# TGAC/KAT

Hardware: AMD Instinct MI355X
Metric: k-mers/sec (whole node) for kat comp reads-vs-assembly k=27 (higher is better)
Workload: dtype u64

## Files before the change

### kat_amd/csrc/kg_count.hip

```cpp
#include "kg_host.hpp"
#include "kg_ingest.hpp"
#include "kg_kernels.hpp"
#include "kg_partition.hpp"
#include "kg_partition_wide.hpp"

#include <condition_variable>
#include <deque>
#include <mutex>
#include <thread>


static const uint64_t g_test_sweep_thr = hook("KATGPU_TEST_SWEEP_THR") ? strtoull(hook("KATGPU_TEST_SWEEP_THR"), nullptr, 10) : 0;
static const uint64_t g_test_max_starts = hook("KATGPU_TEST_MAX_STARTS") ? strtoull(hook("KATGPU_TEST_MAX_STARTS"), nullptr, 10) : 0;

namespace kg {
static __global__ void __launch_bounds__(256)
k_sweep(DevTable t, uint32_t thr, unsigned long long* scratch) {
    uint32_t mx = 0;
    const uint64_t stride = (uint64_t)gridDim.x * blockDim.x;
    for (uint64_t i = (uint64_t)blockIdx.x * blockDim.x + threadIdx.x; i < t.cap; i += stride) {
        uint32_t c = t.counts[i];
        if (c >= thr) {
            uint64_t key = t.keys[i];
            uint32_t take = (c / thr) * thr;
            c -= take;
            t.counts[i] = c;
            ovf_add(t, key, take);
        }
        mx = c > mx ? c : mx;
    }
    for (int off = 32; off > 0; off >>= 1) { uint32_t o = __shfl_down(mx, off, 64); mx = o > mx ? o : mx; }
    if ((threadIdx.x & 63) == 0) atomicMax(scratch, (unsigned long long)mx);
}
}

static int maybe_sweep(katgpu_table* t, uint64_t next_starts) {
    katgpu_ctx* c = t->ctx;
    if (t->dev().cbits) return KATGPU_OK;
    const uint64_t limit = g_test_sweep_thr ? 2 * g_test_sweep_thr - 1 : 0xFFFFFFFFULL;
    if (t->count_bound + t->unchecked_adds + next_starts <= limit) return KATGPU_OK;
    const uint32_t thr = g_test_sweep_thr ? (uint32_t)g_test_sweep_thr : 0x80000000u;
    unsigned long long* scratch = (unsigned long long*)&t->dev().ctrs[CTR_SCRATCH];
    HIPCHK(c, hipMemsetAsync(scratch, 0, sizeof(uint64_t), c->stream));
    {
        ScopedTimer tm(c, KATGPU_K_REGROW, t->dev().cap);
        hipLaunchKernelGGL(k_sweep, dim3(grid_for(c, t->dev().cap, 256, 8)), dim3(256), 0, c->stream, t->dev(), thr, scratch);
    }
    uint64_t mx = 0;
    HIPCHK(c, hipMemcpyAsync(&mx, scratch, sizeof mx, hipMemcpyDeviceToHost, c->stream));
    HIPCHK(c, hipStreamSynchronize(c->stream));
    t->count_bound = mx;
    t->unchecked_adds = 0;
    return KATGPU_OK;
}

static int launch_count(katgpu_table* t, const uint8_t* dev_bases, size_t n) {
    katgpu_ctx* c = t->ctx;
    if (n < t->dev().k) return KATGPU_OK;
    if (t->dev().keys_b) {
        const uint64_t n_chunks = (n + WIDE_CHUNK_STARTS - 1) / WIDE_CHUNK_STARTS;
        const int grid = (int)std::min<uint64_t>(n_chunks, (uint64_t)c->n_cu * 4);
        ScopedTimer tm(c, KATGPU_K_COUNT, n);
        if ((reinterpret_cast<uintptr_t>(dev_bases) & 15) == 0)
            hipLaunchKernelGGL((k_count<true, true>), dim3(grid), dim3(COUNT_BLOCK), 0, c->stream, t->dev(), dev_bases, (uint64_t)n, n_chunks);
        else
            hipLaunchKernelGGL((k_count<false, true>), dim3(grid), dim3(COUNT_BLOCK), 0, c->stream, t->dev(), dev_bases, (uint64_t)n, n_chunks);
        HIPCHK(c, hipGetLastError());
        return KATGPU_OK;
    }
    int src = maybe_sweep(t, n);
    if (src) return src;
    t->unchecked_adds += n;
    const uint64_t n_chunks = (n + CHUNK_STARTS - 1) / CHUNK_STARTS;
    const int grid = (int)std::min<uint64_t>(n_chunks, (uint64_t)c->n_cu * c->count_blocks_per_cu);
    ScopedTimer tm(c, KATGPU_K_COUNT, n);
    if ((reinterpret_cast<uintptr_t>(dev_bases) & 15) == 0)
        hipLaunchKernelGGL(k_count<true>, dim3(grid), dim3(COUNT_BLOCK), 0, c->stream, t->dev(), dev_bases, (uint64_t)n, n_chunks);
    else
        hipLaunchKernelGGL(k_count<false>, dim3(grid), dim3(COUNT_BLOCK), 0, c->stream, t->dev(), dev_bases, (uint64_t)n, n_chunks);
    HIPCHK(c, hipGetLastError());
    return KATGPU_OK;
}



static const uint64_t g_part_min_starts = getenv("KATGPU_PART_MIN_STARTS") ? strtoull(getenv("KATGPU_PART_MIN_STARTS"), nullptr, 10) : (32ULL << 20);
static const uint64_t g_test_round_items = hook("KATGPU_TEST_ROUND_ITEMS") ? strtoull(hook("KATGPU_TEST_ROUND_ITEMS"), nullptr, 10) : 0;
static const double g_arena_fraction = getenv("KATGPU_ARENA_FRACTION") ? std::min(0.95, std::max(0.05, atof(getenv("KATGPU_ARENA_FRACTION")))) : 0.85;
static const uint32_t g_p1_wgs = hook("KATGPU_P1_WGS") ? std::max<uint32_t>(1, (uint32_t)strtoul(hook("KATGPU_P1_WGS"), nullptr, 10)) : 3;
static const bool g_l1_lean = hook_u64("KATGPU_L1_LEAN", 1) != 0;
static const uint32_t g_l1_fast = hook("KATGPU_L1_FAST") ? (uint32_t)strtoul(hook("KATGPU_L1_FAST"), nullptr, 10) : 1;
static const uint32_t g_test_l1_cpb = hook("KATGPU_TEST_L1_CPB") ? (uint32_t)strtoul(hook("KATGPU_TEST_L1_CPB"), nullptr, 10) : 0;
static const uint32_t g_p2_fast = hook("KATGPU_P2_FAST") ? (uint32_t)strtoul(hook("KATGPU_P2_FAST"), nullptr, 10) : 1;
static const uint64_t g_test_p2_ovf_cap = hook("KATGPU_TEST_P2_OVF_CAP") ? strtoull(hook("KATGPU_TEST_P2_OVF_CAP"), nullptr, 10) : 0;
static const uint32_t g_test_spill_mod = hook("KATGPU_TEST_SPILL_MOD") ? (uint32_t)strtoul(hook("KATGPU_TEST_SPILL_MOD"), nullptr, 10) : 0;
static const uint64_t g_test_ap_seg = hook_u64("KATGPU_TEST_AP_SEG", 0) & ~3ULL;
static const uint32_t g_apply_per_cu = (uint32_t)hook_u64("KATGPU_APPLY_PER_CU", 0);
static const uint64_t g_fresh_max_pct = hook_u64("KATGPU_FRESH_MAX_PCT", 100);
static const bool g_l1b_stamp = hook_u64("KATGPU_L1B_STAMP", 0) != 0;
static const bool g_p2x_stamp = hook_u64("KATGPU_P2X_STAMP", 0) != 0;
static const bool g_p2_stamp = hook_u64("KATGPU_P2_STAMP", 0) != 0;
static const bool g_apply_stamp = hook_u64("KATGPU_APPLY_STAMP", 0) != 0;

static bool part_geometry(const DevTable& d, PartGeom* g) {
    g->R = d.n_regions; g->S = d.region_slots; g->P1 = d.p1; g->P2 = d.p2; g->l2 = d.l2;
    g->b_lo = 0; g->b_hi = d.p1;
    g->pl = place_make(d.k, d.p1, d.n1, d.l2);
    g->hb = l2_hi_bytes(g->pl.rb);
    g->hb1 = l2_hi_bytes(g->pl.n1);
    g->cbits = d.cbits;
    if (d.cbits && g->hb > 2) g->hb = 2;
    return d.k <= 32 && g->pl.rb <= 63  && g->P1 <= MAX_PARTS && g->P2 <= MAX_PARTS && g->S % 4 == 0 && g->S >= 64 && g->S <= AP2_MAX_SLOTS;
}
static double l2_items_per_l1_item(uint32_t hb) { return 1 + 1.0 / 16 + 2.0 * MAX_PARTS / l2_tile_items(hb); }
static const uint32_t g_test_pass_buckets = hook("KATGPU_TEST_PASS_BUCKETS") ? (uint32_t)strtoul(hook("KATGPU_TEST_PASS_BUCKETS"), nullptr, 10) : 0;
static uint32_t pass_buckets(uint32_t p1, uint32_t n_cu) {
    if (g_test_pass_buckets) return std::max<uint32_t>(1, std::min(p1, g_test_pass_buckets));
    return n_cu && p1 > n_cu && p1 % n_cu == 0 ? n_cu : p1;
}
static double arena_bytes_per_item(uint32_t hb, uint32_t passes) { return 8.0 * (1 + 1.0 / 24) + l2_bytes_per_item(hb) * (1 + 1.0 / 24) * l2_items_per_l1_item(hb) / passes + 0.25 + 0.02; }

static const bool g_test_grow_nomem = hook("KATGPU_TEST_GROW_NOMEM") != nullptr;

static void insert_keys(katgpu_table* t, const void* keys, uint64_t n, size_t key_bytes) {
    katgpu_ctx* c = t->ctx;
    ScopedTimer tm(c, KATGPU_K_COUNT, n);
    if (key_bytes == 16) hipLaunchKernelGGL(k_insert_keys_w, dim3(grid_for(c, n, 256, 6)), dim3(256), 0, c->stream, t->dev(), (const u64x2*)keys, n);
    else hipLaunchKernelGGL(k_insert_keys, dim3(grid_for(c, n, 256, 6)), dim3(256), 0, c->stream, t->dev(), (const uint64_t*)keys, n);
}
typedef std::vector<std::pair<const void*, uint64_t>> KeyLists;
static int grow_beside_arena(katgpu_table* t, uint64_t incoming, uint64_t min_cap, const KeyLists& stash, size_t key_bytes, bool* arena_lost) {
    uint64_t n_stash = 0;
    for (auto& l : stash) n_stash += l.second;
    katgpu_ctx* c = t->ctx;
    auto grow = [&]() -> int {
        if (min_cap > t->dev().cap) {
            if (t->disable_grow) return fail(c, KATGPU_ERR_TABLE_FULL, "Hash full");
            uint64_t nc = t->dev().cap; while (nc < min_cap) nc *= 2;
            return regrow(t, nc);
        }
        return ensure_room(t, incoming);
    };
    *arena_lost = false;
    int rc = g_test_grow_nomem ? KATGPU_ERR_NOMEM : grow();
    if (rc != KATGPU_ERR_NOMEM) return rc;
    (void)hipGetLastError();
    std::vector<uint8_t> host;
    if (n_stash) {
        try { host.resize(n_stash * key_bytes); } catch (...) { return fail(c, KATGPU_ERR_NOMEM, "no host memory to park %llu spilled k-mers", (unsigned long long)n_stash); }
        uint64_t at = 0;
        for (auto& l : stash) { HIPCHK(c, hipMemcpy(host.data() + at * key_bytes, l.first, l.second * key_bytes, hipMemcpyDeviceToHost)); at += l.second; }
    }
    HIPCHK(c, hipStreamSynchronize(c->stream));
    release_arena(c);
    *arena_lost = true;
    if (g_trace) fprintf(stderr, "[katgpu] growth beside the partition arena failed: arena released, %llu keys parked on the host\n", (unsigned long long)n_stash);
    rc = grow();
    if (rc) return rc;
    if (n_stash) {
        const size_t chunk = std::min<size_t>(n_stash, ((size_t)256 << 20) / key_bytes);
        uint8_t* d = nullptr;
        HIPCHK(c, pool_alloc(c, (void**)&d, chunk * key_bytes));
        for (size_t i = 0; i < n_stash && rc == KATGPU_OK; i += chunk) {
            const size_t m = std::min(chunk, (size_t)n_stash - i);
            if (hipMemcpyAsync(d, host.data() + i * key_bytes, m * key_bytes, hipMemcpyHostToDevice, c->stream) != hipSuccess) { rc = fail(c, KATGPU_ERR_DEVICE, "spill upload"); break; }
            insert_keys(t, d, m, key_bytes);
            if (hipStreamSynchronize(c->stream) != hipSuccess) rc = fail(c, KATGPU_ERR_DEVICE, "spill insert");
        }
        pool_release(c, d);
    }
    return rc;
}

static int ensure_arena(katgpu_ctx* c, size_t small_bytes, size_t item_bytes, size_t want_items, size_t want_bytes, const char* note, bool* usable) {
    *usable = false;
    if (c->arena_limit) want_bytes = std::min(want_bytes, std::max(c->arena_limit, small_bytes + item_bytes * ((size_t)64 << 20)));
    if (c->arena_bytes < want_bytes) {
        size_t free_b = 0, total_b = 0;
        HIPCHK(c, hipMemGetInfo(&free_b, &total_b));
        free_b += c->arena_bytes;
        const size_t bytes = std::min<size_t>(want_bytes, (size_t)(g_arena_fraction * (double)free_b));
        if (bytes > c->arena_bytes + c->arena_bytes / 2 || c->arena_bytes < small_bytes + item_bytes * std::min<size_t>(want_items, (size_t)64 << 20)) {
            if (c->arena) { HIPCHK(c, hipFree(c->arena)); c->arena = nullptr; c->arena_bytes = 0; }
            if (!g_test_round_items && bytes < small_bytes + item_bytes * ((size_t)1 << 20)) return KATGPU_OK;
            const double t_ar = now_ms();
            if (hipMalloc((void**)&c->arena, bytes) != hipSuccess) { (void)hipGetLastError(); c->arena = nullptr; return KATGPU_OK; }
            c->arena_bytes = bytes;
            if (g_trace) fprintf(stderr, "[katgpu +%.0f ms] partition arena of %.1f GB%s: %.0f ms\n", since_load(), bytes / 1e9, note, now_ms() - t_ar);
        }
    }
    *usable = true;
    return KATGPU_OK;
}
struct ArenaBusy { katgpu_ctx* c; explicit ArenaBusy(katgpu_ctx* c_) : c(c_) { c->arena_busy = true; } ~ArenaBusy() { c->arena_busy = false; } };
template <typename T> static T* carve(uint8_t*& a, size_t bytes) { T* p = (T*)a; a += align_up(bytes, 256); return p; }

constexpr size_t LDS_BYTES = 160 * 1024, LDS_GRANULE = 1280;
template <typename K, typename... Args>
static int launch_lds(katgpu_ctx* c, K kern, dim3 grid, dim3 block, size_t lds, size_t ceiling, Args... args) {
    if (!c->lds_attr.count(reinterpret_cast<const void*>(kern))) {
        HIPCHK(c, hipFuncSetAttribute(reinterpret_cast<const void*>(kern), hipFuncAttributeMaxDynamicSharedMemorySize, (int)ceiling));
        c->lds_attr.insert(reinterpret_cast<const void*>(kern));
    }
    hipLaunchKernelGGL(kern, grid, block, lds, c->stream, args...);
    return KATGPU_OK;
}

struct StampLine { const char* head; int n_shown, n_sum; const char* phase[9];  int digits; };
static const StampLine STAMPS_L1B = {"[katgpu] level-1 (blocks) stamps (wave 0 of every workgroup, cycles summed):", 9, 9,
    {" codes %.*f %%", "  blocks out %.*f %%", " (+ barrier %.*f %%)", "  sweep %.*f %%", " (+ %.*f %%)", "  per bucket %.*f %%", " (+ %.*f %%)", "  placing %.*f %%", " (+ %.*f %%)"}, 1};
static const StampLine STAMPS_P2X = {"[katgpu] level-2 (blocks in, blocks out) stamps (wave 0 of every workgroup, cycles summed):", 7, 9,
    {" wait for the tile %.*f %%", " (+ barrier %.*f %%)", "  ranking + blocks out %.*f %%", " (+ %.*f %%)", "  per sub-bucket %.*f %%", " (+ %.*f %%)", "  placing %.*f %%"}, 1};
static const StampLine STAMPS_P2 = {"[katgpu] level-2 stamps (lane 0 of every workgroup, cycles summed):", 5, 5,
    {" wait for the tile %.*f %%", "  digit + rank %.*f %%", "  scan %.*f %%", "  staging %.*f %%", "  copy-out %.*f %%"}, 0};
constexpr int STAMP_AT_APPLY = 8, STAMP_AT = 18;
constexpr int STAMP_AREA = 256 / 8;
static_assert(2 <= STAMP_AT_APPLY && STAMP_AT_APPLY + 9 <= STAMP_AT && STAMP_AT + 10 <= STAMP_AREA, "the stamp counters lie behind spill_n and ovf_n, apart, inside spill_n's carve");
template <typename Launch>
static int with_stamps(katgpu_ctx* c, unsigned long long* dev, int n, const StampLine* line, Launch launch) {
    unsigned long long st[10];
    HIPCHK(c, hipMemsetAsync(dev, 0, n * sizeof(unsigned long long), c->stream));
    int rc = launch(dev);
    if (rc) return rc;
    HIPCHK(c, hipMemcpyAsync(st, dev, n * sizeof(unsigned long long), hipMemcpyDeviceToHost, c->stream));
    HIPCHK(c, hipStreamSynchronize(c->stream));
    double tot = line ? 0 : (double)(st[0] + st[1] + st[3] + st[4]);
    if (!line && st[5])
        fprintf(stderr, "[katgpu] apply stamps (wave 0 of every workgroup, cycles summed): fill %.3g (%.0f %%)  walk %.3g (%.0f %%; drains %.0f %% of the walk, %.2f iterations per pass)  barrier + sweep %.3g (%.0f %%)  write-back %.3g (%.0f %%); %llu regions, %.1f chunks per wave and region, %.0f cycles per region\n",
                (double)st[0], 100 * st[0] / tot, (double)st[1], 100 * st[1] / tot, 100.0 * st[2] / std::max(1.0, (double)st[1]), (double)st[8] / std::max(1.0, (double)st[7]), (double)st[3], 100 * st[3] / tot, (double)st[4], 100 * st[4] / tot, st[5], (double)st[6] / st[5], tot / st[5]);
    if (!line || !st[n - 1]) return KATGPU_OK;
    for (int i = 0; i < line->n_sum; ++i) tot += (double)st[i];
    char buf[768];
    int at = snprintf(buf, sizeof buf, "%s", line->head);
    for (int i = 0; i < line->n_shown; ++i) at += snprintf(buf + at, sizeof buf - at, line->phase[i], line->digits, 100 * st[i] / tot);
    fprintf(stderr, "%s; %llu tiles, %.0f cycles per tile\n", buf, st[n - 1], tot / st[n - 1]);
    return KATGPU_OK;
}

struct ApplyForm { bool packed; int block, kp; bool fresh , hooked; };
struct ApplyLaunch {
    katgpu_table* t; const PartGeom& g; const uint64_t* off2; const uint8_t* l2_buf; uint64_t* spill_buf; unsigned long long* spill_n; const uint32_t* run_len; const uint64_t* bucket_end;
    dim3 grid; size_t lds; uint32_t qcap; uint64_t seg_len; uint32_t zero_fill; ApplyForm* form;
};
template <int B, int KP, int HB, bool INL, bool HK, bool LATE , int NR, bool STAMP = false>
static int apply_pk(const ApplyLaunch& a) {
    if (a.form) *a.form = ApplyForm{true, B, KP, INL, HK};
    return launch_lds(a.t->ctx, k_p3_apply_pk<B, KP, HB, INL, HK, LATE, NR, STAMP>, a.grid, dim3(B), a.lds, LDS_BYTES - 256, a.t->dv, a.g, a.off2, a.l2_buf, a.spill_buf, a.spill_n, a.run_len, a.bucket_end,
                      a.qcap, a.seg_len, g_test_spill_mod, a.zero_fill);
}
template <int HB>
static int apply_pk_shape(const ApplyLaunch& a, uint32_t blk, bool fresh, bool hooked) {
    if (hooked) return apply_pk<1024, 5, HB, false, true, true, 3>(a);
    if (blk == 1024) return fresh ? apply_pk<1024, 5, HB, true, false, true, 3>(a) : apply_pk<1024, 5, HB, false, false, true, 2>(a);
    if (a.g.S <= 4096) {
        if (HB == 1 && g_apply_stamp && fresh)
            return with_stamps(a.t->ctx, a.spill_n + STAMP_AT_APPLY, 9, nullptr, [&](unsigned long long*) { return apply_pk<512, 4, 1, true, false, true, 3, true>(a); });
        return fresh ? apply_pk<512, 4, HB, true, false, true, 3>(a) : apply_pk<512, 4, HB, false, false, true, 2>(a);
    }
    if (HB == 1 && g_apply_stamp && !fresh)
        return with_stamps(a.t->ctx, a.spill_n + STAMP_AT_APPLY, 9, nullptr, [&](unsigned long long*) { return apply_pk<512, 10, 1, false, false, false, 2, true>(a); });
    return fresh ? apply_pk<512, 10, HB, true, false, false, 3>(a) : apply_pk<512, 10, HB, false, false, false, 2>(a);
}
template <int B, int KP, int HB, bool INL, int QC, bool HK>
static int apply_kv12(const ApplyLaunch& a) {
    if (a.form) *a.form = ApplyForm{false, B, KP, INL, HK};
    return launch_lds(a.t->ctx, k_p3_apply2<B, KP, 4, 3, HB, false, INL, true, QC, HK>, a.grid, dim3(B), a.lds, LDS_BYTES - 256, a.t->dev(), a.g, a.off2, a.l2_buf, a.spill_buf, a.spill_n, a.run_len, a.bucket_end,
                      (unsigned long long*)nullptr, g_test_spill_mod, a.seg_len);
}
template <int HB>
static int apply_kv12_shape(const ApplyLaunch& a, uint32_t blk, bool big, bool fresh, bool hooked) {
    if (hooked) return apply_kv12<1024, 5, HB, false, AP2_QCAP_BIG, true>(a);
    if (blk == 512 && a.g.S <= 2048) return fresh ? apply_kv12<512, 2, HB, true, AP2_QCAP, false>(a) : apply_kv12<512, 2, HB, false, AP2_QCAP, false>(a);
    if (blk == 512) return fresh ? apply_kv12<512, 4, HB, true, AP2_QCAP, false>(a) : apply_kv12<512, 4, HB, false, AP2_QCAP, false>(a);
    if (big) return fresh ? apply_kv12<1024, 5, HB, true, AP2_QCAP_BIG, false>(a) : apply_kv12<1024, 5, HB, false, AP2_QCAP_BIG, false>(a);
    return fresh ? apply_kv12<1024, 4, HB, true, AP2_QCAP, false>(a) : apply_kv12<1024, 4, HB, false, AP2_QCAP, false>(a);
}
static int launch_apply(katgpu_table* t, const PartGeom& g, const uint64_t* off2, const uint8_t* l2_buf, uint64_t* spill_buf, unsigned long long* spill_n,
                        const uint32_t* run_len, const uint64_t* bucket_end, uint64_t round_items, ApplyForm* form = nullptr) {
    katgpu_ctx* c = t->ctx;
    const uint32_t n_cu = (uint32_t)c->n_cu, regions = (g.b_hi - g.b_lo) * g.P2;
    bool fresh = t->distinct == 0;
    const bool hooked = g_test_spill_mod != 0;
    ApplyLaunch a{t, g, off2, l2_buf, spill_buf, spill_n, run_len, bucket_end, dim3(1), 0, 0, 0, 0, form};
    int rc = KATGPU_OK;
    if (g.cbits) {
        const size_t region_b = (size_t)g.S * 8;
        auto room = [&](uint32_t wgs) -> long { return (long)(LDS_BYTES / wgs / LDS_GRANULE * LDS_GRANULE) - 64 - (long)region_b; };
        uint32_t per_cu = 4;
        auto min_q = [&](uint32_t wgs) -> long { return 8L * 8 * (wgs == 2 ? 72 : 96); };
        while (per_cu > 1 && room(per_cu) < min_q(per_cu)) --per_cu;
        if (g_apply_per_cu) per_cu = std::min(per_cu, g_apply_per_cu);
        uint32_t blk = per_cu == 1 ? 1024 : 512;
        if (hooked) { blk = 1024; per_cu = 1; }
        per_cu = std::min<uint32_t>(per_cu, 2048 / blk);
        const uint32_t nw = blk / 64;
        while (per_cu > 1 && room(per_cu) < (long)(nw * 72 * 8)) --per_cu;
        a.qcap = (uint32_t)std::min<long>(256, room(per_cu) / (long)(nw * 8));
        if (a.qcap < 72) return fail(c, KATGPU_ERR_DEVICE, "a region of %u packed slots leaves no room for the apply kernel's queues", g.S);
        a.lds = region_b + (size_t)nw * a.qcap * 8;
        if (fresh && a.qcap >= 96 && (double)round_items * 100.0 >= (double)g_fresh_max_pct * (double)t->dv.cap) fresh = false;
        const uint64_t seg_cap = (pk_half(g.cbits) - 1) & ~3ULL;
        a.seg_len = g_test_ap_seg ? std::min<uint64_t>(g_test_ap_seg, seg_cap) : std::min<uint64_t>(AP2_SEGMENT, seg_cap);
        a.grid = dim3(std::min<uint32_t>(regions, n_cu * per_cu));
        const uint64_t r_lo = (uint64_t)g.b_lo * g.P2, r_hi = (uint64_t)g.b_hi * g.P2;
        if (t->zero_from != ~0ULL) { if (t->zero_from == r_lo) a.zero_fill = 1; else t->zero_rest(); }
        switch (g.hb) {
        case 0: rc = apply_pk_shape<0>(a, blk, fresh, hooked); break;
        case 1: rc = apply_pk_shape<1>(a, blk, fresh, hooked); break;
        case 2: rc = apply_pk_shape<2>(a, blk, fresh, hooked); break;
        default: return fail(c, KATGPU_ERR_DEVICE, "packed apply: item width %u", g.hb);
        }
        if (rc) return rc;
        HIPCHK(c, hipGetLastError());
        if (a.zero_fill) t->zero_from = r_hi >= t->dv.n_regions ? ~0ULL : r_hi;
        return KATGPU_OK;
    }
    const uint32_t blk = hooked ? 1024 : (g.S <= 4096 ? 512 : 1024);
    const bool big = g.S > 8192 || hooked;
    a.lds = (size_t)g.S * 12 + (size_t)(blk / 64) * (big ? AP2_QCAP_BIG : AP2_QCAP) * 12;
    const uint32_t per_cu = (uint32_t)std::max<size_t>(1, std::min<size_t>(LDS_BYTES / (a.lds + 512), 2048 / blk));
    a.grid = dim3(std::min<uint32_t>(regions, n_cu * per_cu));
    a.seg_len = g_test_ap_seg ? std::min<uint64_t>(g_test_ap_seg, AP2_SEGMENT) : AP2_SEGMENT;
    switch (g.hb) {
    case 0: rc = apply_kv12_shape<0>(a, blk, big, fresh, hooked); break;
    case 1: rc = apply_kv12_shape<1>(a, blk, big, fresh, hooked); break;
    case 2: rc = apply_kv12_shape<2>(a, blk, big, fresh, hooked); break;
    case 4: rc = apply_kv12_shape<4>(a, blk, big, fresh, hooked); break;
    }
    if (rc) return rc;
    HIPCHK(c, hipGetLastError());
    return KATGPU_OK;
}

constexpr size_t SEG_PAD = 64;
struct PartArena {
    uint32_t hb, passes; double per_item; size_t fixed_l1, small_bytes;
    uint32_t* hist1; uint64_t* offs; uint64_t* l1_off; uint64_t* off2; uint32_t* cnt2; uint64_t* bend; unsigned long long* spill_n; unsigned long long* ovf_n;
    uint8_t* l1_buf;
    uint8_t* l2_buf;
    uint64_t* ovf_buf; uint64_t ovf_cap;
    size_t round_items, l1_items, l2_items;
    PartArena(const PartGeom& g0, uint32_t W, uint32_t n_cu) : hb(g0.hb), passes(std::max<uint32_t>(1, g0.P1 / pass_buckets(g0.P1, n_cu))), per_item(arena_bytes_per_item(hb, passes)) {
        fixed_l1 = (size_t)W * MAX_PARTS * SEG_PAD;
        const size_t fixed_l2 = (size_t)((double)fixed_l1 * l2_items_per_l1_item(hb) / passes) + (size_t)MAX_PARTS * MAX_PARTS * P2_RUN_SLACK + 8192;
        small_bytes = align_up((size_t)W * MAX_PARTS * 4, 256) + align_up((size_t)W * MAX_PARTS * 8, 256) +
                      align_up((MAX_PARTS + 1) * 8, 256) + align_up(((size_t)MAX_PARTS * MAX_PARTS + 1) * 8, 256) +
                      align_up((size_t)MAX_PARTS * MAX_PARTS * 4, 256) + align_up((size_t)MAX_PARTS * 8, 256) + align_up((size_t)MAX_PARTS * 4, 256) + 256 +
                      (fixed_l1 + fixed_l2 + 4096) * 8 + 4096;
    }
    void carve_from(uint8_t* a, size_t arena_bytes, uint32_t W, size_t want_items) {
        hist1 = carve<uint32_t>(a, (size_t)W * MAX_PARTS * 4);
        offs = carve<uint64_t>(a, (size_t)W * MAX_PARTS * 8);
        l1_off = carve<uint64_t>(a, (MAX_PARTS + 1) * 8);
        off2 = carve<uint64_t>(a, ((size_t)MAX_PARTS * MAX_PARTS + 1) * 8);
        cnt2 = carve<uint32_t>(a, (size_t)MAX_PARTS * MAX_PARTS * 4);
        bend = carve<uint64_t>(a, (size_t)MAX_PARTS * 8);
        carve<uint32_t>(a, (size_t)MAX_PARTS * 4);
        spill_n = carve<unsigned long long>(a, STAMP_AREA * 8);
        ovf_n = spill_n + 1;
        round_items = std::min<size_t>(want_items, (size_t)((double)(arena_bytes - small_bytes) / per_item));
        l1_items = (round_items + round_items / 24 + fixed_l1 + 15) & ~(size_t)15;
        l2_items = ((size_t)((double)l1_items * l2_items_per_l1_item(hb) / passes) + (size_t)MAX_PARTS * MAX_PARTS * P2_RUN_SLACK + 4096 + 11) / 12 * 12;
        l1_buf = a;
        l2_buf = l1_buf + l1_items * 8;
        ovf_buf = (uint64_t*)(l2_buf + align_up(l2_buffer_bytes(hb, l2_items), 16));
        ovf_cap = g_test_p2_ovf_cap ? g_test_p2_ovf_cap : round_items / 32 + 1024;
    }
};
static int restore_ones(katgpu_table* t) { katgpu_ctx* c = t->ctx; HIPCHK(c, hipMemcpyAsync(&t->dv.ctrs[CTR_ONES], &t->ones, sizeof(uint64_t), hipMemcpyHostToDevice, c->stream)); return KATGPU_OK; }
static int probe_items_per_start(katgpu_table* t, const PartGeom& g, const PartArena& A, uint32_t W, const uint8_t* p, size_t left, double* items_per_start) {
    katgpu_ctx* c = t->ctx;
    const size_t probe_m = std::min<size_t>(left, (size_t)64 << 20) / P1_TILE_STARTS * P1_TILE_STARTS;
    const uint64_t pt = probe_m / P1_TILE_STARTS, ptw = (pt + W - 1) / W;
    hipLaunchKernelGGL(k_p1v2_count, dim3(W), dim3(P1_BLOCK), 0, c->stream, t->dv, g, p, (uint64_t)(probe_m + t->dv.k - 1), pt, ptw, A.hist1);
    hipLaunchKernelGGL(k_p1_scan, dim3(1), dim3(PART_BLOCK), 0, c->stream, g, W, A.hist1, A.offs, A.l1_off);
    uint64_t probe_items = 0;
    HIPCHK(c, hipMemcpyAsync(&probe_items, &A.l1_off[g.P1], sizeof probe_items, hipMemcpyDeviceToHost, c->stream));
    HIPCHK(c, hipStreamSynchronize(c->stream));
    *items_per_start = std::max(0.05, (double)probe_items / (double)probe_m);
    return t->dv.k == 32 && !t->dv.canonical ? restore_ones(t) : KATGPU_OK;
}
static size_t round_starts(size_t left, size_t round_items, double items_per_start) {
    size_t m = left;
    if (m > round_items) m = std::min(m, (size_t)((double)round_items / items_per_start * 0.98));
    if (m < left) {
        const size_t rounds_left = (left + m - 1) / m;
        m = (left + rounds_left - 1) / rounds_left;
        m += P1_TILE_STARTS - m % P1_TILE_STARTS;
        m = std::min(m, left);
    }
    return m;
}

enum class L1Edition { Blocks, SegLean512, SegLean1024, SegPlain512, SegPlain1024, ExactLean, ExactPlain };
static const char* const L1_EDITION_NAME[] = {"Blocks", "SegLean512", "SegLean1024", "SegPlain512", "SegPlain1024", "ExactLean", "ExactPlain"};
struct L1Plan {
    L1Edition edition; bool seg ; uint32_t wgs ; uint64_t n_tiles, tiles_per_wg;
    uint64_t seg_cap, cap_plain, stride64;
};
static L1Plan plan_level1(const PartGeom& g, uint32_t k, size_t m, uint64_t est_items, uint32_t W, uint32_t n_cu, size_t l1_items, bool seg_wanted) {
    const bool lean = g_l1_lean && lean_applies(k, g.pl.n1);
    const bool pb512 = g.P1 <= 512;
    const bool l1b = lean && pb512 && g.hb1 == 2;
    const uint64_t n_tiles = (m + P1_TILE_STARTS - 1) / P1_TILE_STARTS;
    L1Plan pl;
    pl.wgs = l1b ? n_cu : W;
    pl.n_tiles = l1b ? (m + L1B_TILE_STARTS - 1) / L1B_TILE_STARTS : n_tiles;
    uint64_t seg_cap = est_items / ((uint64_t)pl.wgs * g.P1);
    seg_cap += seg_cap / 24 + SEG_PAD;
    if (g_test_l1_cpb) seg_cap = std::min<uint64_t>(seg_cap, g_test_l1_cpb);
    if (l1b) seg_cap = (seg_cap + L1B_ITEMS - 1) / L1B_ITEMS * L1B_ITEMS;
    pl.cap_plain = seg_cap;
    if (!l1b && g.hb1 != 4 && !g_test_l1_cpb) seg_cap += std::min<uint64_t>(3 * seg_cap, 2 * ((pl.n_tiles + pl.wgs - 1) / pl.wgs));
    if (!l1b) seg_cap = (seg_cap + 3) & ~3ULL;
    pl.seg_cap = seg_cap;
    pl.stride64 = l1b ? align_up(8 * (uint64_t)pl.wgs * pl.cap_plain + 32, 64)
                      : std::max<uint64_t>(8 * (uint64_t)pl.wgs * pl.cap_plain, (uint64_t)(4 + g.hb1) * pl.wgs * seg_cap) + 32;
    pl.seg = seg_wanted && pl.stride64 * g.P1 <= (uint64_t)l1_items * 8 &&
             seg_cap < (1u << 24) && pl.stride64 <= 0xFFFFFFFFULL ;
    if (pl.seg) pl.edition = l1b ? L1Edition::Blocks : lean ? (pb512 ? L1Edition::SegLean512 : L1Edition::SegLean1024) : (pb512 ? L1Edition::SegPlain512 : L1Edition::SegPlain1024);
    else { pl.edition = lean ? L1Edition::ExactLean : L1Edition::ExactPlain; pl.wgs = W; pl.n_tiles = n_tiles; }
    pl.tiles_per_wg = (pl.n_tiles + pl.wgs - 1) / pl.wgs;
    return pl;
}
static int launch_l1_scatter(katgpu_table* t, const PartGeom& g, const L1Plan& l1, const PartArena& A, const uint8_t* p, uint64_t nb) {
    katgpu_ctx* c = t->ctx;
    auto blocks = [&](auto kern, unsigned long long* stamps) {
        return launch_lds(c, kern, dim3(l1.wgs), dim3(L1B_THREADS), sizeof(P1BLds), sizeof(P1BLds), t->dv, g, p, nb, l1.n_tiles, l1.tiles_per_wg,
                          A.l1_buf, (uint32_t)(l1.seg_cap / L1B_ITEMS), (uint32_t)l1.stride64, A.ovf_buf, A.ovf_n, A.ovf_cap, stamps);
    };
    auto segmented = [&](auto kern) {
        hipLaunchKernelGGL(kern, dim3(l1.wgs), dim3(P1_BLOCK), 0, c->stream, t->dv, g, p, nb, l1.n_tiles, l1.tiles_per_wg, (const uint64_t*)nullptr, (const uint64_t*)nullptr, A.l1_buf,
                           (uint32_t)l1.seg_cap, (uint32_t)l1.stride64, (uint32_t)l1.cap_plain, A.ovf_buf, A.ovf_n, A.ovf_cap);
        return KATGPU_OK;
    };
    auto exact = [&](auto kern) {
        hipLaunchKernelGGL(kern, dim3(l1.wgs), dim3(P1_BLOCK), 0, c->stream, t->dv, g, p, nb, l1.n_tiles, l1.tiles_per_wg, (const uint64_t*)A.offs, (const uint64_t*)A.l1_off, A.l1_buf,
                           0u, 0u, 0u, (uint64_t*)nullptr, (unsigned long long*)nullptr, (uint64_t)0);
        return KATGPU_OK;
    };
    switch (l1.edition) {
    case L1Edition::Blocks:
        if (!g_l1b_stamp) return blocks(k_p1b_scatter<false>, nullptr);
        return with_stamps(c, A.spill_n + STAMP_AT, 10, &STAMPS_L1B, [&](unsigned long long* st) { return blocks(k_p1b_scatter<true>, st); });
    case L1Edition::SegLean512:   return segmented(k_p1v2_scatter<true, true, 512>);
    case L1Edition::SegLean1024:  return segmented(k_p1v2_scatter<true, true, MAX_PARTS>);
    case L1Edition::SegPlain512:  return segmented(k_p1v2_scatter<true, false, 512>);
    case L1Edition::SegPlain1024: return segmented(k_p1v2_scatter<true, false, MAX_PARTS>);
    case L1Edition::ExactLean:    return exact(k_p1v2_scatter<false, true, MAX_PARTS>);
    case L1Edition::ExactPlain:   return exact(k_p1v2_scatter<false, false, MAX_PARTS>);
    }
    return KATGPU_OK;
}
static int level1(katgpu_table* t, const PartGeom& g, const L1Plan& l1, const PartArena& A, const uint8_t* p, size_t m, double items_per_start, uint64_t* items) {
    katgpu_ctx* c = t->ctx;
    const uint64_t nb = m + t->dv.k - 1;
    if (l1.seg) {
        int rc;
        { ScopedTimer tm(c, KATGPU_K_PART_L1S, *items); rc = launch_l1_scatter(t, g, l1, A, p, nb); }
        if (!rc && g_trace) fprintf(stderr, "[katgpu] partition round (segmented level 1%s): %zu starts, ~%llu items, %llu k-mers per segment (arena %.1f GB)\n", l1.edition == L1Edition::Blocks ? ", blocks of ten" : "", m,
                                    (unsigned long long)*items, (unsigned long long)l1.seg_cap, c->arena_bytes / 1e9);
        return rc;
    }
    {
        ScopedTimer tm(c, KATGPU_K_PART_L1, m);
        hipLaunchKernelGGL(k_p1v2_count, dim3(l1.wgs), dim3(P1_BLOCK), 0, c->stream, t->dv, g, p, nb, l1.n_tiles, l1.tiles_per_wg, A.hist1);
        hipLaunchKernelGGL(k_p1_scan, dim3(1), dim3(PART_BLOCK), 0, c->stream, g, l1.wgs, A.hist1, A.offs, A.l1_off);
    }
    HIPCHK(c, hipMemcpyAsync(items, &A.l1_off[g.P1], sizeof *items, hipMemcpyDeviceToHost, c->stream));
    HIPCHK(c, hipStreamSynchronize(c->stream));
    if (g_trace) fprintf(stderr, "[katgpu] partition round: %zu starts -> %llu items (buffer %zu items, arena %.1f GB, ratio %.3f)\n", m, (unsigned long long)*items, A.round_items, c->arena_bytes / 1e9, items_per_start);
    if (*items > A.round_items) return t->dv.k == 32 && !t->dv.canonical ? restore_ones(t) : KATGPU_OK;
    if (!*items) return KATGPU_OK;
    ScopedTimer tm(c, KATGPU_K_PART_L1S, *items);
    return launch_l1_scatter(t, g, l1, A, p, nb);
}

enum class L1Items { Groups , WideGroups , Blocks  };
static const char* const L1_ITEMS_NAME[] = {"Groups", "WideGroups", "Blocks"};
enum L2Family : uint32_t { L2_BLOCKS = 1 , L2_ONE_PASS = 2 , L2_EXACT = 4  };
struct L2Pass { katgpu_ctx* c; const PartGeom& g; const PartArena& A; uint32_t grid; L1Items src; uint64_t seg_slots; uint32_t* families ; };
template <typename K>
static int p2_one_pass(const L2Pass& x, K kern, size_t lds, unsigned long long* stamps = nullptr) {
    return launch_lds(x.c, kern, dim3(x.grid), dim3(PART_BLOCK), lds, lds, x.g, x.A.l1_off, x.A.l1_buf, x.A.l2_buf, x.A.off2, x.A.cnt2, x.A.ovf_buf, x.A.ovf_n, x.A.ovf_cap, x.seg_slots, stamps);
}
template <typename K>
static int p2_exact(const L2Pass& x, K kern, size_t lds) {
    return launch_lds(x.c, kern, dim3(x.grid), dim3(PART_BLOCK), lds, lds, x.g, x.A.l1_off, x.A.l1_buf, x.A.l2_buf, x.A.off2, x.seg_slots, x.A.bend);
}
template <int HB>
static int launch_l2_hb(const L2Pass& x, bool one_pass) {
    constexpr size_t lds_e = sizeof(P2Lds<HB>), lds_f = sizeof(typename P2FastLds<HB>::type);
    unsigned long long* const stamps = x.A.spill_n + STAMP_AT;
    if (x.families) *x.families |= !one_pass ? L2_EXACT : x.src == L1Items::Blocks && HB == 1 ? L2_BLOCKS : L2_ONE_PASS;
    switch (x.src) {
    case L1Items::Blocks:
        if constexpr (HB == 4) break;
        else if (!one_pass) return p2_exact(x, k_p2<HB, false, true>, lds_e);
        else if constexpr (HB != 1) return p2_one_pass(x, k_p2_fast<HB, false, false, true>, lds_f);
        else if (!g_p2x_stamp) return p2_one_pass(x, k_p2x_fast<false>, sizeof(P2XLds));
        else return with_stamps(x.c, stamps, 10, &STAMPS_P2X, [&](unsigned long long* st) { return p2_one_pass(x, k_p2x_fast<true>, sizeof(P2XLds), st); });
    case L1Items::WideGroups: return one_pass ? p2_one_pass(x, k_p2_fast<HB, true>, lds_f) : p2_exact(x, k_p2<HB, true>, lds_e);
    case L1Items::Groups:
        if constexpr (HB == 1) if (one_pass && g_p2_stamp) return with_stamps(x.c, stamps, 6, &STAMPS_P2, [&](unsigned long long* st) { return p2_one_pass(x, k_p2_fast<1, false, true>, lds_f, st); });
        return one_pass ? p2_one_pass(x, k_p2_fast<HB, false>, lds_f) : p2_exact(x, k_p2<HB, false>, lds_e);
    }
    return fail(x.c, KATGPU_ERR_DEVICE, "level 2 from blocked level-1 items: item width %u", x.g.hb);
}
static int launch_l2(const L2Pass& x, bool one_pass) {
    switch (x.g.hb) {
    case 0: return launch_l2_hb<0>(x, one_pass);
    case 1: return launch_l2_hb<1>(x, one_pass);
    case 2: return launch_l2_hb<2>(x, one_pass);
    case 4: return launch_l2_hb<4>(x, one_pass);
    }
    return fail(x.c, KATGPU_ERR_DEVICE, "level 2: item width %u", x.g.hb);
}
enum class L2Next { UseCnt2 , Exact , FallBackExact ,
                    RedoRound  };
static int read_overflow(katgpu_table* t, const PartArena& A, bool seg, bool tried_fast, unsigned long long ovf_l1, const unsigned long long* ovf_before, unsigned long long* overflowed, L2Next* next) {
    katgpu_ctx* c = t->ctx;
    HIPCHK(c, hipMemcpyAsync(overflowed, A.ovf_n, sizeof *overflowed, hipMemcpyDeviceToHost, c->stream));
    HIPCHK(c, hipStreamSynchronize(c->stream));
    if (seg && ovf_l1 > A.ovf_cap) {
        if (g_trace) fprintf(stderr, "[katgpu] segmented level 1: %llu k-mers beyond their segments (list holds %llu): exact level 1 from here on\n", ovf_l1, (unsigned long long)A.ovf_cap);
        *next = L2Next::RedoRound;
        return restore_ones(t);
    }
    *next = !tried_fast ? L2Next::Exact : *overflowed <= A.ovf_cap ? L2Next::UseCnt2 : L2Next::FallBackExact;
    if (*next == L2Next::FallBackExact) {
        if (g_trace) fprintf(stderr, "[katgpu] k_p2_fast: %llu k-mers beyond their runs (list holds %llu): exact level 2 from here on\n", *overflowed, (unsigned long long)A.ovf_cap);
        *overflowed = *ovf_before;
        HIPCHK(c, hipMemcpyAsync(A.ovf_n, ovf_before, sizeof *ovf_before, hipMemcpyHostToDevice, c->stream));
    }
    return KATGPU_OK;
}

enum class RoundEnd { Done, RedoExactL1 , DirectPath  };
static int level2_and_apply(katgpu_table* t, PartGeom& g, const L1Plan& l1, const PartArena& A, uint64_t items, bool* p2_fast_ok, KeyLists* lists, RoundEnd* end) {
    katgpu_ctx* c = t->ctx;
    const bool seg = l1.seg;
    const uint64_t seg_slots = seg ? (uint64_t)l1.wgs * l1.seg_cap : 0;
    const L1Items src = seg && l1.edition == L1Edition::Blocks ? L1Items::Blocks : g.hb1 == 4 ? L1Items::WideGroups : L1Items::Groups;
    *end = RoundEnd::Done;
    std::vector<uint64_t> h_l1_off;
    unsigned long long ovf_l1 = 0;
    if (!seg) {
        h_l1_off.resize(g.P1 + 1);
        HIPCHK(c, hipMemcpyAsync(h_l1_off.data(), A.l1_off, (g.P1 + 1) * sizeof(uint64_t), hipMemcpyDeviceToHost, c->stream));
    } else HIPCHK(c, hipMemcpyAsync(&ovf_l1, A.ovf_n, sizeof ovf_l1, hipMemcpyDeviceToHost, c->stream));
    HIPCHK(c, hipStreamSynchronize(c->stream));
    auto lbeg = [&](uint32_t b) -> uint64_t { return seg ? (uint64_t)b * g.l1_real : h_l1_off[b]; };
    const uint32_t tile2 = l2_tile_items(g.hb);
    auto pass_extent = [&](uint32_t b_lo, uint32_t b_hi) -> uint64_t {
        const uint64_t nn = lbeg(b_hi) - lbeg(b_lo);
        return nn + nn / 16 + 2ULL * g.P2 * (nn / tile2 + 1) + (uint64_t)(b_hi - b_lo) * g.P2 * P2_RUN_SLACK + 64;
    };
    uint32_t step = pass_buckets(g.P1, (uint32_t)c->n_cu);
    auto fits = [&](uint32_t st) { for (uint32_t b = 0; b < g.P1; b += st) if (pass_extent(b, std::min(g.P1, b + st)) > A.l2_items) return false; return true; };
    while (step > 1 && !fits(step)) step = (step + 1) / 2;
    if (!fits(step)) {
        *end = RoundEnd::DirectPath;
        return seg || (t->dv.k == 32 && !t->dv.canonical) ? restore_ones(t) : KATGPU_OK;
    }
    const bool try_fast0 = *p2_fast_ok && (g_p2_fast == 2 || items / g.R >= 1024);
    unsigned long long ovf_total = ovf_l1;
    uint32_t l2_families = 0;
    ApplyForm ap{};
    if (g_trace && g.P1 > step) fprintf(stderr, "[katgpu]   level 2 + apply in %u passes of %u buckets (level-2 buffer: %zu items)\n", (g.P1 + step - 1) / step, step, A.l2_items);
    for (uint32_t b_lo = 0; b_lo < g.P1; b_lo += step) {
        g.b_lo = b_lo; g.b_hi = std::min(g.P1, b_lo + step);
        const uint64_t pass_items = std::max<uint64_t>(1, (uint64_t)((double)items * (g.b_hi - g.b_lo) / g.P1));
        auto l1_at = [&](uint32_t b) -> uint64_t { return seg ? (uint64_t)b * g.l1_stride : l1_bucket_base(lbeg(b), b); };
        uint64_t* spill_buf = (uint64_t*)(A.l1_buf + l1_at(b_lo));
        g.spill_cap = (l1_at(g.b_hi) - l1_at(b_lo)) / 8;
        const bool try_fast = try_fast0 && *p2_fast_ok;
        const L2Pass x{c, g, A, std::min<uint32_t>(g.b_hi - g.b_lo, (uint32_t)c->n_cu), src, seg_slots, &l2_families};
        HIPCHK(c, hipMemsetAsync(A.spill_n, 0, sizeof(unsigned long long), c->stream));
        int rc = KATGPU_OK;
        if (try_fast) { ScopedTimer tm(c, KATGPU_K_PART_L2, pass_items); rc = launch_l2(x, true); }
        if (rc) return rc;
        L2Next next = L2Next::Exact;
        unsigned long long overflowed = ovf_total;
        if (try_fast || (seg && b_lo == 0)) {
            rc = read_overflow(t, A, seg, try_fast, ovf_l1, &ovf_total, &overflowed, &next);
            if (rc) return rc;
            if (next == L2Next::RedoRound) { *end = RoundEnd::RedoExactL1; return KATGPU_OK; }
            if (next == L2Next::FallBackExact) *p2_fast_ok = false;
        }
        const bool runs = next == L2Next::UseCnt2;
        if (!runs) { ScopedTimer tm(c, KATGPU_K_PART_L2, pass_items); rc = launch_l2(x, false); }
        if (rc) return rc;
        ovf_total = overflowed;
        {
            ScopedTimer tm(c, KATGPU_K_PART_APPLY, pass_items);
            rc = launch_apply(t, g, A.off2, A.l2_buf, spill_buf, A.spill_n, runs ? A.cnt2 : nullptr, runs ? nullptr : A.bend, items, &ap);
        }
        if (rc) return rc;
        HIPCHK(c, hipGetLastError());
        unsigned long long spilled = 0;
        HIPCHK(c, hipMemcpyAsync(&spilled, A.spill_n, sizeof spilled, hipMemcpyDeviceToHost, c->stream));
        HIPCHK(c, hipStreamSynchronize(c->stream));
        if (spilled > g.spill_cap)
            return fail(c, KATGPU_ERR_TABLE_FULL, "Hash full: %llu k-mers of a partition pass found no slot (the list holds %llu); raise the size hint", spilled, (unsigned long long)g.spill_cap);
        if (spilled) lists->push_back({spill_buf, spilled});
    }
    if (ovf_total) lists->push_back({A.ovf_buf, ovf_total});
    if (g_trace) {
        char l2[32];
        snprintf(l2, sizeof l2, "%s%s%s", l2_families & L2_BLOCKS ? "+blocks" : "", l2_families & L2_ONE_PASS ? "+one-pass" : "", l2_families & L2_EXACT ? "+exact" : "");
        fprintf(stderr, "[katgpu] partition forms: l1=%s items=%s hb1=%u hb=%u l2=%s apply=%s B=%d KP=%d fresh=%d%s\n", L1_EDITION_NAME[(int)l1.edition], L1_ITEMS_NAME[(int)src], g.hb1, g.hb,
                l2[0] ? l2 + 1 : "none", ap.packed ? "packed" : "KV12", ap.block, ap.kp, (int)ap.fresh, ap.hooked ? " hooked" : "");
    }
    return KATGPU_OK;
}
static int insert_spilled(katgpu_table* t, const KeyLists& lists, bool* arena_lost) {
    *arena_lost = false;
    if (lists.empty()) return KATGPU_OK;
    uint64_t total = 0;
    for (auto& l : lists) total += l.second;
    int rc = grow_beside_arena(t, total, 0, lists, 8, arena_lost);
    if (rc || *arena_lost) return rc;
    for (auto& l : lists) insert_keys(t, l.first, l.second, 8);
    return KATGPU_OK;
}

static int count_partitioned(katgpu_table* t, const uint8_t* dev_bases, size_t n, size_t* done) {
    katgpu_ctx* c = t->ctx;
    const uint32_t k = t->dv.k, n_cu = (uint32_t)c->n_cu;
    const size_t n_starts = n - k + 1;
    *done = 0;
    c->arena_borrowed = false;
    if (n < 64) return KATGPU_OK;
    if (!g_test_round_items && !t->disable_grow && t->dv.cap < n_starts / 16) {
        uint64_t nc = t->dv.cap; while (nc < n_starts / 16) nc *= 2;
        int grc = regrow(t, nc);
        if (grc) return grc;
    }
    const uint32_t W = n_cu * std::min<uint32_t>(g_p1_wgs, 4);
    PartGeom g0;
    if (!part_geometry(t->dv, &g0)) return KATGPU_OK;
    PartArena A(g0, W, n_cu);
    size_t want_items = n_starts;
    if (g_test_round_items) want_items = std::min<size_t>(want_items, g_test_round_items);
    bool usable = false;
    int rc = ensure_arena(c, A.small_bytes, 18, want_items, A.small_bytes + (size_t)((A.per_item + 0.5) * (double)want_items), "", &usable);
    if (rc || !usable) return rc;
    ArenaBusy busy(c);
    A.carve_from(c->arena, c->arena_bytes, W, want_items);
    if (!g_test_round_items && A.round_items < ((size_t)1 << 20) && A.round_items < n_starts) return KATGPU_OK;
    bool p2_fast_ok = g_p2_fast != 0, l1_fast_ok = g_l1_fast != 0;
    double items_per_start = 1.0;
    size_t pos = 0;
    bool ratio_known = false;
    while (pos < n_starts) {
        rc = refresh_counters(t);
        if (rc) return rc;
        if ((double)t->distinct > 0.6 * (double)t->dv.cap) {
            bool lost = false;
            rc = grow_beside_arena(t, 0, t->dv.cap * 2, KeyLists(), 8, &lost);
            if (rc) return rc;
            if (lost) break;
        }
        PartGeom g;
        if (!part_geometry(t->dv, &g)) break;
        if (g.hb > A.hb) break;
        const size_t left = n_starts - pos;
        const uint8_t* p = dev_bases + pos;
        if (!ratio_known && !g_test_round_items && (left > A.round_items || (l1_fast_ok && left >= ((size_t)64 << 20)))) {
            rc = probe_items_per_start(t, g, A, W, p, left, &items_per_start);
            if (rc) return rc;
            ratio_known = true;
        }
        const size_t m = round_starts(left, A.round_items, items_per_start);
        t->count_bound = 0xFFFFFFFFULL;
        const uint64_t est_items = (uint64_t)((double)m * items_per_start);
        const bool seg_wanted = l1_fast_ok && (g_l1_fast == 2 || (ratio_known && est_items >= ((uint64_t)64 << 20)));
        const L1Plan l1 = plan_level1(g, k, m, est_items, W, n_cu, A.l1_items, seg_wanted);
        g.l1_stride = l1.seg ? l1.stride64 : 0;
        g.l1_real = l1.seg ? (uint64_t)l1.wgs * l1.cap_plain : 0;
        HIPCHK(c, hipMemsetAsync(A.spill_n, 0, 2 * sizeof(unsigned long long), c->stream));
        uint64_t items = est_items;
        rc = level1(t, g, l1, A, p, m, items_per_start, &items);
        if (rc) return rc;
        if (!l1.seg && items > A.round_items) {
            items_per_start = std::min(1.0, (double)items / (double)m * 1.02);
            continue;
        }
        if (items) {
            KeyLists lists;
            RoundEnd end;
            rc = level2_and_apply(t, g, l1, A, items, &p2_fast_ok, &lists, &end);
            if (rc) return rc;
            if (end == RoundEnd::RedoExactL1) { l1_fast_ok = false; continue; }
            if (end == RoundEnd::DirectPath) break;
            bool lost = false;
            rc = insert_spilled(t, lists, &lost);
            if (rc) return rc;
            if (lost) { pos += m; break; }
        }
        pos += m;
    }
    *done = pos;
    return refresh_counters(t);
}

static bool wide_part_geometry(const DevTable& d) {
    return d.keys_b && d.p1 <= (uint32_t)MAX_PARTS && d.p2 <= (uint32_t)MAX_PARTS && d.region_slots % 4 == 0 && d.region_slots >= 64 && d.region_slots <= WIDE_AP_MAX_SLOTS &&
           (uint64_t)d.p1 * d.p2 == d.n_regions;
}
static int count_partitioned_w(katgpu_table* t, const uint8_t* dev_bases, size_t n, size_t* done) {
    katgpu_ctx* c = t->ctx;
    const uint32_t k = t->dev().k;
    const size_t n_starts = n - k + 1;
    *done = 0;
    c->arena_borrowed = false;
    if (n < 4096 || !wide_part_geometry(t->dev())) return KATGPU_OK;
    if (!g_test_round_items && !t->disable_grow && t->dev().cap < n_starts / 16) {
        uint64_t nc = t->dev().cap; while (nc < n_starts / 16) nc *= 2;
        int grc = regrow(t, nc);
        if (grc) return grc;
        if (!wide_part_geometry(t->dev())) return KATGPU_OK;
    }
    const uint32_t W = (uint32_t)c->n_cu * 3;
    const size_t tile_starts = W1_TILE_STARTS;
    const size_t small_bytes = align_up((size_t)W * MAX_PARTS * 4, 256) + align_up((size_t)W * MAX_PARTS * 8, 256) + align_up((MAX_PARTS + 1) * 8, 256) +
                               align_up(((size_t)MAX_PARTS * MAX_PARTS + 1) * 8, 256) + 256 + 4096;
    size_t want_items = n_starts;
    if (g_test_round_items) want_items = std::min<size_t>(want_items, g_test_round_items);
    bool usable = false;
    int rc = ensure_arena(c, small_bytes, 32, want_items + 64, small_bytes + 32 * (want_items + 64), " (wide k-mers)", &usable);
    if (rc || !usable) return rc;
    ArenaBusy busy(c);
    uint8_t* a = c->arena;
    uint32_t* hist1 = carve<uint32_t>(a, (size_t)W * MAX_PARTS * 4);
    uint64_t* offs = carve<uint64_t>(a, (size_t)W * MAX_PARTS * 8);
    uint64_t* l1_off = carve<uint64_t>(a, (MAX_PARTS + 1) * 8);
    uint64_t* off2 = carve<uint64_t>(a, ((size_t)MAX_PARTS * MAX_PARTS + 1) * 8);
    unsigned long long* spill_n = carve<unsigned long long>(a, 256);
    const size_t round_items = std::min<size_t>(want_items, (c->arena_bytes - small_bytes) / 32);
    u64x2* l1_buf = (u64x2*)a;
    u64x2* l2_buf = l1_buf + round_items;
    if (!g_test_round_items && round_items < ((size_t)1 << 20) && round_items < n_starts) return KATGPU_OK;
    if (round_items < tile_starts && round_items < n_starts) return KATGPU_OK;

    size_t pos = 0;
    while (pos < n_starts) {
        rc = refresh_counters(t);
        if (rc) return rc;
        if ((double)t->distinct > 0.6 * (double)t->dev().cap) {
            bool lost = false;
            rc = grow_beside_arena(t, 0, t->dev().cap * 2, KeyLists(), 16, &lost);
            if (rc) return rc;
            if (lost) break;
        }
        if (!wide_part_geometry(t->dev())) break;
        const DevTable d = t->dev();
        size_t m = std::min(n_starts - pos, round_items);
        if (m < n_starts - pos) {
            const size_t rounds_left = (n_starts - pos + m - 1) / m;
            m = std::min(m, (n_starts - pos + rounds_left - 1) / rounds_left + tile_starts);
            m -= m % tile_starts;
            if (!m) break;
        }
        const size_t nb = m + k - 1;
        const uint8_t* p = dev_bases + pos;
        const uint64_t n_tiles = (m + tile_starts - 1) / tile_starts;
        const uint64_t tiles_per_wg = (n_tiles + W - 1) / W;
        PartGeom g{};
        g.P1 = d.p1;
        HIPCHK(c, hipMemsetAsync(spill_n, 0, sizeof(unsigned long long), c->stream));
        {
            ScopedTimer tm(c, KATGPU_K_PART_L1, m);
            hipLaunchKernelGGL(k_w1<false>, dim3(W), dim3(W1_BLOCK), 0, c->stream, d, d.p1, p, (uint64_t)nb, n_tiles, tiles_per_wg, hist1, (const uint64_t*)nullptr, (u64x2*)nullptr);
            hipLaunchKernelGGL(k_p1_scan, dim3(1), dim3(PART_BLOCK), 0, c->stream, g, W, hist1, offs, l1_off);
        }
        uint64_t items = 0;
        HIPCHK(c, hipMemcpyAsync(&items, &l1_off[d.p1], sizeof items, hipMemcpyDeviceToHost, c->stream));
        HIPCHK(c, hipStreamSynchronize(c->stream));
        if (g_trace) fprintf(stderr, "[katgpu] partition round (wide k-mers): %zu starts -> %llu items (buffer %zu items, arena %.1f GB)\n", m, (unsigned long long)items, round_items, c->arena_bytes / 1e9);
        if (items > round_items) return fail(c, KATGPU_ERR_DEVICE, "wide partition round: %llu items from %zu starts", (unsigned long long)items, m);
        if (items) {
            {
                ScopedTimer tm(c, KATGPU_K_PART_L1S, items);
                hipLaunchKernelGGL(k_w1<true>, dim3(W), dim3(W1_BLOCK), 0, c->stream, d, d.p1, p, (uint64_t)nb, n_tiles, tiles_per_wg, (uint32_t*)nullptr, (const uint64_t*)offs, l1_buf);
            }
            {
                ScopedTimer tm(c, KATGPU_K_PART_L2, items);
                hipLaunchKernelGGL(k_w2, dim3(std::min<uint32_t>(d.p1, (uint32_t)c->n_cu)), dim3(PART_BLOCK), 0, c->stream, d.p1, d.p2, (const uint64_t*)l1_off, (const u64x2*)l1_buf, l2_buf, off2);
            }
            {
                ScopedTimer tm(c, KATGPU_K_PART_APPLY, items);
                rc = launch_lds(c, k_w3_apply, dim3(std::min<uint32_t>(d.n_regions, (uint32_t)c->n_cu)), dim3(W3_BLOCK), (size_t)d.region_slots * 20, LDS_BYTES - 256, d, (const uint64_t*)off2, (const u64x2*)l2_buf,
                                l1_buf , spill_n, g_test_spill_mod);
                if (rc) return rc;
            }
            HIPCHK(c, hipGetLastError());
            unsigned long long spilled = 0;
            HIPCHK(c, hipMemcpyAsync(&spilled, spill_n, sizeof spilled, hipMemcpyDeviceToHost, c->stream));
            HIPCHK(c, hipStreamSynchronize(c->stream));
            if (spilled) {
                if (g_trace) fprintf(stderr, "[katgpu]   %llu k-mers spilled by full regions\n", spilled);
                bool lost = false;
                rc = grow_beside_arena(t, spilled, 0, KeyLists(1, {l1_buf, spilled}), 16, &lost);
                if (rc) return rc;
                if (lost) { pos += m; break; }
                insert_keys(t, l1_buf, spilled, 16);
                HIPCHK(c, hipStreamSynchronize(c->stream));
            }
        }
        pos += m;
    }
    *done = pos;
    return refresh_counters(t);
}

int count_resident(katgpu_table* t, const uint8_t* dev_bases, size_t n) {
    const uint32_t k = t->dv.k;
    if (n < k) return KATGPU_OK;
    size_t pos = 0;
    const size_t n_starts = n - k + 1;
    while (!t->dv.keys_b && n_starts - pos >= std::max<uint64_t>(g_part_min_starts, 1) && (reinterpret_cast<uintptr_t>(dev_bases + pos) & 15) == 0) {
        size_t done = 0;
        int prc = count_partitioned(t, dev_bases + pos, n - pos, &done);
        if (prc) return prc;
        if (!done) break;
        pos += done;
    }
    while (t->dv.keys_b && n_starts - pos >= std::max<uint64_t>(g_part_min_starts, 1) && (reinterpret_cast<uintptr_t>(dev_bases + pos) & 15) == 0) {
        size_t done = 0;
        int prc = count_partitioned_w(t, dev_bases + pos, n - pos, &done);
        if (prc) return prc;
        if (!done) break;
        pos += done;
    }
    while (pos < n_starts) {
        int rc = refresh_counters(t);
        if (rc) return rc;
        uint64_t room = (uint64_t)(load_limit(t->dev()) * (double)t->dev().cap) > t->distinct ? (uint64_t)(load_limit(t->dev()) * (double)t->dev().cap) - t->distinct : 0;
        uint64_t want = std::min<uint64_t>(n_starts - pos, (uint64_t)CHUNK_STARTS * 65536);
        if (g_test_max_starts) want = std::min<uint64_t>(want, g_test_max_starts);
        if (room < std::min<uint64_t>(want, std::max<uint64_t>(t->dev().cap / 64, CHUNK_STARTS))) {
            rc = ensure_room(t, std::min<uint64_t>(want, std::max<uint64_t>(t->dev().cap / 2, CHUNK_STARTS)));
            if (rc) return rc;
            continue;
        }
        uint64_t starts = std::min(want, room);
        if (starts < n_starts - pos) starts -= starts % 16;
        if (starts == 0) starts = std::min<uint64_t>(16, n_starts - pos);
        rc = launch_count(t, dev_bases + pos, (size_t)(starts + k - 1));
        if (rc) return rc;
        pos += starts;
    }
    return refresh_counters(t);
}

extern "C" int katgpu_count_bases_device(katgpu_table* t, const uint8_t* dev_bases, size_t n) {
    if (!t || (!dev_bases && n)) return KATGPU_ERR_INVALID_ARG;
    HIPCHK(t->ctx, hipSetDevice(t->ctx->device));
    return count_resident(t, dev_bases, n);
}

static const size_t g_ring_bytes = (getenv("KATGPU_RING_MB") ? std::max<size_t>(1, strtoull(getenv("KATGPU_RING_MB"), nullptr, 10)) : 1024) << 20;

static int ensure_staging(katgpu_ctx* c, size_t want = 0) {
    int rc = ensure_pinned(c); if (rc) return rc;
    size_t ring_want = g_ring_bytes;
    if (want) ring_want = std::min(g_ring_bytes, std::max<size_t>((size_t)16 << 20, align_up(want + 4096, (size_t)16 << 20)));
    if (c->ring_bytes && c->ring_bytes < ring_want) {
        for (int i = 0; i < 2; ++i) { hipFree(c->ring[i]); c->ring[i] = nullptr; }
        c->ring_bytes = 0;
    }
    for (; !c->ring_bytes; ring_want /= 2) {
        if (ring_want < ((size_t)1 << 20)) return fail(c, KATGPU_ERR_NOMEM, "no device memory for the staging rings");
        bool ok = true;
        for (int i = 0; i < 2 && ok; ++i) {
            hipError_t e = hipMalloc((void**)&c->ring[i], ring_want);
            if (e != hipSuccess && c->arena && !c->arena_borrowed && !c->arena_busy) {
                (void)hipGetLastError();
                hipFree(c->arena); c->arena = nullptr; c->arena_bytes = 0;
                e = hipMalloc((void**)&c->ring[i], ring_want);
            }
            if (e != hipSuccess) { (void)hipGetLastError(); for (int j = 0; j < i; ++j) { hipFree(c->ring[j]); c->ring[j] = nullptr; } ok = false; }
        }
        if (ok) c->ring_bytes = ring_want;
    }
    return KATGPU_OK;
}

struct HostFeeder {
    katgpu_table* t; katgpu_ctx* c;
    int cur = 0; size_t fill = 0; bool pin_used[2] = {false, false};
    int ring_cur = 0; size_t ring_fill = 0;
    uint8_t tail[64]; uint32_t tail_n = 0;
    static constexpr size_t HEAD = 64;
    std::thread worker;
    std::mutex mu; std::condition_variable cv;
    struct Job { int ring; size_t n; };
    std::deque<Job> jobs;
    bool ring_busy[2] = {false, false};
    bool stop = false;
    int worker_rc = KATGPU_OK; std::string worker_err;

    explicit HostFeeder(katgpu_table* t_) : t(t_), c(t_->ctx) {}
    ~HostFeeder() { shutdown(); }

    void run() {
        hipSetDevice(c->device);
        for (;;) {
            Job j;
            {
                std::unique_lock<std::mutex> lk(mu);
                cv.wait(lk, [&] { return stop || !jobs.empty(); });
                if (jobs.empty()) return;
                j = jobs.front(); jobs.pop_front();
            }
            int rc = worker_rc ? worker_rc : count_resident(t, c->ring[j.ring], j.n);
            {
                std::lock_guard<std::mutex> lk(mu);
                if (rc && !worker_rc) { worker_rc = rc; worker_err = c->err; }
                ring_busy[j.ring] = false;
            }
            cv.notify_all();
        }
    }
    void shutdown() {
        if (!worker.joinable()) return;
        { std::lock_guard<std::mutex> lk(mu); stop = true; }
        cv.notify_all();
        worker.join();
    }
    int begin(size_t want = 0) {
        int rc = ensure_staging(c, want); if (rc) return rc;
        tail_n = 0;
        worker = std::thread([this] { run(); });
        return open_ring();
    }
    int open_ring() {
        uint8_t head[HEAD];
        memset(head, 'N', HEAD);
        memcpy(head + HEAD - tail_n, tail, tail_n);
        HIPCHK(c, hipMemcpyAsync(c->ring[ring_cur], head, HEAD, hipMemcpyHostToDevice, c->copy_stream));
        HIPCHK(c, hipStreamSynchronize(c->copy_stream));
        ring_fill = HEAD;
        return KATGPU_OK;
    }
    int submit_ring() {
        HIPCHK(c, hipStreamSynchronize(c->copy_stream));
        const int other = ring_cur ^ 1;
        {
            std::unique_lock<std::mutex> lk(mu);
            if (ring_fill > HEAD) { ring_busy[ring_cur] = true; jobs.push_back({ring_cur, ring_fill}); }
            cv.notify_all();
            cv.wait(lk, [&] { return !ring_busy[other]; });
            if (worker_rc) return fail(c, worker_rc, "%s", worker_err.c_str());
        }
        if (ring_fill > HEAD) ring_cur = other;
        return open_ring();
    }
    int push(const uint8_t* p, size_t n) {
        while (n) {
            if (fill == 0 && pin_used[cur]) { hipError_t e = hipEventSynchronize(c->pin_free[cur]); if (e != hipSuccess) return fail(c, KATGPU_ERR_DEVICE, "%s", hipGetErrorString(e)); }
            const size_t room = c->stage_bytes - fill, take = std::min(room, n);
            memcpy(c->pinned[cur] + fill, p, take);
            fill += take; p += take; n -= take;
            if (fill == c->stage_bytes) { int rc = flush(); if (rc) return rc; }
        }
        return KATGPU_OK;
    }
    int flush() {
        if (!fill) return KATGPU_OK;
        const uint32_t want = t->dv.k - 1;
        size_t off = 0;
        while (off < fill) {
            if (ring_fill == c->ring_bytes) { int rc = submit_ring(); if (rc) return rc; }
            const size_t take = std::min(fill - off, c->ring_bytes - ring_fill);
            const uint8_t* src = c->pinned[cur] + off;
            HIPCHK(c, hipMemcpyAsync(c->ring[ring_cur] + ring_fill, src, take, hipMemcpyHostToDevice, c->copy_stream));
            ring_fill += take; off += take;
            if (take >= want) { memcpy(tail, src + take - want, want); tail_n = want; }
            else {
                uint8_t tmp[128]; const uint32_t keep = (uint32_t)std::min<size_t>(tail_n, want - take);
                memcpy(tmp, tail + tail_n - keep, keep); memcpy(tmp + keep, src, take);
                tail_n = keep + (uint32_t)take; memcpy(tail, tmp, tail_n);
            }
        }
        HIPCHK(c, hipEventRecord(c->pin_free[cur], c->copy_stream));
        pin_used[cur] = true;
        cur ^= 1; fill = 0;
        return KATGPU_OK;
    }
    int end_of_file() {
        static const uint8_t sep = 'N';
        return push(&sep, 1);
    }
    int finish() {
        int rc = flush(); if (rc) { shutdown(); return rc; }
        HIPCHK(c, hipStreamSynchronize(c->copy_stream));
        {
            std::unique_lock<std::mutex> lk(mu);
            if (ring_fill > HEAD) { ring_busy[ring_cur] = true; jobs.push_back({ring_cur, ring_fill}); }
            cv.notify_all();
// ... 108 lines not shown
```

### kat_amd/csrc/kg_l2_blocks.hpp

```cpp
#pragma once

namespace kg {

constexpr int L2X_N = 14;
constexpr uint32_t L2X_TILE = L2X_N * PART_BLOCK;
constexpr uint32_t L2X_POOL = 1252;

struct P2XLds {
    uint32_t hist[MAX_PARTS + 64];
    uint2 gb[MAX_PARTS];
    uint32_t where[L2X_POOL];
    uint32_t wave_tot[32];
    __attribute__((aligned(64))) uint32_t img[(MAX_PARTS + L2X_POOL) * 16];
};
static_assert(sizeof(P2XLds) <= 160 * 1024 - 256 && offsetof(P2XLds, img) % 64 == 0, "LDS");
static_assert(PART_BLOCK == MAX_PARTS, "thread b is sub-bucket b");

template <bool STAMP = false >
__global__ void __launch_bounds__(PART_BLOCK)
k_p2x_fast(PartGeom g, const uint64_t* __restrict__ l1_off, const uint8_t* __restrict__ l1_buf, uint8_t* __restrict__ l2_buf,
           uint64_t* __restrict__ off2, uint32_t* __restrict__ cnt2, uint64_t* __restrict__ ovf_buf, unsigned long long* __restrict__ ovf_n,
           uint64_t ovf_cap, uint64_t seg_slots, unsigned long long* __restrict__ stamps) {
    constexpr int N = L2X_N;
    constexpr uint32_t PB = MAX_PARTS, TILE_CAP = L2Fmt<1>::TILE ;
    extern __shared__ __attribute__((aligned(64))) unsigned char lds_raw[];
    P2XLds& L = *reinterpret_cast<P2XLds*>(lds_raw);
    unsigned char* const img8 = reinterpret_cast<unsigned char*>(L.img);
    const uint32_t tid = threadIdx.x, P = g.P2;
    unsigned long long st[10] = {0, 0, 0, 0, 0, 0, 0, 0, 0, 0}, tq = 0;
    auto stamp = [&](int i) { if (STAMP) { const unsigned long long x = (unsigned long long)clock64(); st[i] += x - tq; tq = x; } };
    uint64_t beg0, n0, nr0;
    l1_bucket_range(g, l1_off, seg_slots, g.b_lo, beg0, n0, nr0);
    uint32_t tid_o = tid;
    for (uint32_t b1 = g.b_lo + blockIdx.x; b1 < g.b_hi; b1 += gridDim.x) {
        uint64_t beg, n_items, n_real;
        const uint8_t* bucket = l1_buf + l1_bucket_range(g, l1_off, seg_slots, b1, beg, n_items, n_real);
        const uint64_t cap = p2_region_cap(n_real, P, TILE_CAP, L2_BLOCK_ITEMS);
        const uint64_t obase = p2_out_base(beg, b1, P, TILE_CAP, L2_BLOCK_ITEMS) - p2_out_base(beg0, g.b_lo, P, TILE_CAP, L2_BLOCK_ITEMS);
        uint8_t* const runs = l2_buf + l2_lo_at<1>(obase >> 2);
        const uint32_t capb = (uint32_t)(cap / L2_BLOCK_ITEMS);
        lds_barrier();
        asm volatile("" : "+v"(tid_o));
        L.hist[tid_o] = 0; L.gb[tid_o] = uint2{0u, 0u};
        if (tid < 64) L.hist[PB + tid_o] = 0;
        L.img[tid_o * 16 + 15] = 0;
        if (tid < P) off2[(uint64_t)b1 * P + tid_o] = obase + (uint64_t)tid * cap;
        uint32_t n_out = 0;
        constexpr int OUT_STEPS = (L2X_POOL + PART_BLOCK / 4 - 1) / (PART_BLOCK / 4);
        static_assert(OUT_STEPS <= N / 2, "a step per pair of the ranking's items");
        struct OutStep { u32x4 v; uint32_t where; };
        auto out_read = [&](int it, OutStep& o) {
            asm volatile("" : "+v"(tid_o));
            const uint32_t s = min((tid_o >> 2) + (uint32_t)it * (PART_BLOCK / 4), L2X_POOL - 1);
            o.where = L.where[s];
            o.v = *reinterpret_cast<const u32x4*>(&L.img[(PB + s) * 16 + (tid_o & 3) * 4]);
        };
        auto out_store = [&](int it, const OutStep& o) {
            asm volatile("" : "+v"(tid_o));
            if ((tid_o >> 2) + (uint32_t)it * (PART_BLOCK / 4) < n_out)
                *reinterpret_cast<u32x4*>(runs + (((uint64_t)o.where << 6) | ((tid_o & 3) * 16))) = o.v;
        };
        RawTileB<N> raw;
        p2_tile_issue_l1b<N>(bucket, 0, raw);
        for (uint64_t tbeg = 0; tbeg < n_items; tbeg += L2X_TILE) {
            if (STAMP) tq = (unsigned long long)clock64();
            TileItems<N, false> key;
            const uint32_t valid = p2_tile_decode_l1b<N>(tbeg, n_items, raw, key);
            {
#pragma unroll
                for (int j = 0; j < N; ++j) asm volatile("" : "+v"(key.lo[j]));
#pragma unroll
                for (int j = 0; j < N / 2; ++j) asm volatile("" : "+v"(key.hi[j]));
            }
            p2_tile_issue_l1b<N>(bucket, tbeg + L2X_TILE, raw);
            stamp(0);
            lds_barrier();
            stamp(1);
            uint32_t br[N];
            {
                uint32_t rk[N];
                const uint32_t dump = PB + (tid & 63);
                OutStep o;
#pragma unroll
                for (int j = 0; j < N; ++j) {
                    if (j % 2 == 0 && j / 2 < OUT_STEPS) out_read(j / 2, o);
                    const uint32_t b = place_digit2_of(key.r1(j), g.pl) & (PB - 1);
                    rk[j] = atomicAdd(&L.hist[(valid >> j & 1) ? b : dump], 1u);
                    br[j] = b << 16;
                    if (j >= 2) br[j - 2] |= rk[j - 2];
                    if (j % 2 == 1 && j / 2 < OUT_STEPS) out_store(j / 2, o);
                }
#pragma unroll
                for (int j = N - 2; j < N; ++j) br[j] |= rk[j];
            }
            stamp(2);
            lds_barrier();
            stamp(3);
            asm volatile("" : "+v"(tid_o));
            {
                uint32_t want = 0, avail = 0, nblk = 0, cur = 0, cn_old = 0;
                if (tid < P) {
                    avail = L.hist[tid_o];
                    const uint32_t w15 = L.img[tid_o * 16 + 15];
                    cur = w15 & 0x0FFFFFFFu; cn_old = w15 >> 28;
                    nblk = __umulhi(avail, 0xAAAAAAABu) >> 3;
                    want = min(nblk, capb > cur ? capb - cur : 0u);
                }
                const uint32_t lane = tid_o & 63, wave = tid_o >> 6;
                const uint32_t inc = wave_inclusive_scan(want);
                if (lane == 63) L.wave_tot[wave] = inc;
                lds_barrier();
                const uint32_t sc = wave_inclusive_scan(lane < PART_BLOCK / 64 ? L.wave_tot[lane] : 0u);
                const uint32_t wv = (uint32_t)__builtin_amdgcn_readfirstlane((int)wave);
                const uint32_t excl = (wv ? lane_value(sc, (int)wv - 1) : 0u) + inc - want;
                { const uint32_t tot = lane_value(sc, PART_BLOCK / 64 - 1); n_out = tot < L2X_POOL ? tot : L2X_POOL; }
                if (tid < P) {
                    const uint32_t nst = excl < L2X_POOL ? min(want, L2X_POOL - excl) : 0u;
                    const bool stuck = nblk != 0 && nst == 0;
                    L.gb[tid_o] = uint2{(L2_BLOCK_ITEMS * nst) | ((stuck ? 0xFFFFu : L2_BLOCK_ITEMS * nblk) << 16), PB + excl};
                    if (nst) {
                        const uint32_t first = tid_o * capb + cur;
                        for (uint32_t q = 0; q < nst; ++q) L.where[excl + q] = first + q;
                    }
                    const uint32_t cn = stuck ? cn_old : avail - L2_BLOCK_ITEMS * nblk;
                    L.img[tid_o * 16 + 15] = (cur + nst) | (cn << 28);
                    L.hist[tid_o] = cn;
                } else L.hist[tid_o] = 0;
                if (tid < 64) L.hist[PB + tid_o] = 0;
                blk_move_waiting(L, tid_o);
            }
            stamp(4);
            lds_barrier();
            stamp(5);
            {
                uint32_t lostm = 0;
                constexpr int SB = 2;
#pragma unroll
                for (int j0 = 0; j0 < N; j0 += SB) {
                    uint2 G[SB];
#pragma unroll
                    for (int u = 0; u < SB; ++u) G[u] = L.gb[br[j0 + u] >> 16];
#pragma unroll
                    for (int u = 0; u < SB; ++u) asm volatile("" : "+v"(G[u].x), "+v"(G[u].y));
#pragma unroll
                    for (int u = 0; u < SB; ++u) {
                        const int j = j0 + u;
                        const bool ok = (valid >> j & 1) != 0;
                        const uint32_t v = br[j] & 0xFFFFu, lf = G[u].x >> 16;
                        const uint32_t q = __umulhi(v, 0xAAAAAAABu) >> 3;
                        uint32_t s = v - L2_BLOCK_ITEMS * q, B_p = G[u].y + q;
                        asm volatile("" : "+v"(s), "+v"(B_p));
                        const bool placed = v < (G[u].x & 0xFFFFu), later = v >= lf;
                        const uint32_t B = later ? br[j] >> 16 : B_p;
                        const uint64_t rem = key.r1(j) & g.pl.mr;
                        if (ok && (placed || later)) { L.img[B * 16 + s] = (uint32_t)rem; img8[B * 64 + 48 + s] = (uint8_t)(rem >> 32); }
                        lostm |= (ok && !placed && !later) ? 1u << j : 0u;
                    }
                }
                if (__any(lostm != 0)) {
#pragma unroll
                    for (int j = 0; j < N; ++j)
                        if (lostm >> j & 1) {
                            const unsigned long long at = atomicAdd(ovf_n, 1ULL);
                            if (at < ovf_cap) ovf_buf[at] = place_key_d(b1, br[j] >> 16, key.r1(j) & g.pl.mr, g.pl);
                        }
                }
            }
            stamp(6);
            if (STAMP) st[9] += 1;
        }
        lds_barrier();
#pragma unroll
        for (int it = 0; it < OUT_STEPS; ++it) { OutStep o; out_read(it, o); out_store(it, o); }
        lds_barrier();
        asm volatile("" : "+v"(tid_o));
        uint32_t blocks = 0;
        {
            const uint32_t w15 = L.img[tid_o * 16 + 15], cur = w15 & 0x0FFFFFFFu, cn = tid < P ? w15 >> 28 : 0u;
            const bool room = cur < capb;
            if (cn && room) for (uint32_t q = cn; q < L2_BLOCK_ITEMS; ++q) { L.img[tid_o * 16 + q] = 0xFFFFFFFFu; img8[tid_o * 64 + 48 + q] = 0xFF; }
            if (cn && !room)
                for (uint32_t q = 0; q < cn; ++q) {
                    const unsigned long long at = atomicAdd(ovf_n, 1ULL);
                    if (at < ovf_cap) ovf_buf[at] = place_key_d(b1, tid, ((uint64_t)img8[tid_o * 64 + 48 + q] << 32) | L.img[tid_o * 16 + q], g.pl);
                }
            L.gb[tid_o].x = cn && room ? 1u : 0u;
            blocks = cur + (cn && room ? 1u : 0u);
        }
        lds_barrier();
        for (uint32_t qi = tid_o; qi < 4 * P; qi += PART_BLOCK) {
            const uint32_t b = qi >> 2, w = qi & 3;
            const uint32_t cur = L.img[b * 16 + 15] & 0x0FFFFFFFu;
            const u32x4 v = *reinterpret_cast<const u32x4*>(&L.img[b * 16 + 4 * w]);
            if (L.gb[b].x) *reinterpret_cast<u32x4*>(runs + (((uint64_t)b * capb + cur) << 6) + 16 * w) = v;
        }
        asm volatile("" : "+v"(tid_o));
        if (tid < P) cnt2[(uint64_t)b1 * P + tid_o] = blocks * L2_BLOCK_ITEMS;
    }
    if (STAMP && tid == 0 && stamps) for (int i = 0; i < 10; ++i) atomicAdd(&stamps[i], st[i]);
}

}
```

### kat_amd/csrc/kg_partition.hpp

```cpp
#pragma once
#include "kg_kernels.hpp"
#include "kg_l1_lean.hpp"
#include "kg_apply_lean.hpp"

#include <cstddef>
#include <type_traits>

namespace kg {

constexpr int PART_BLOCK = 1024;
constexpr int PART_ITEMS = BASES_PER_LANE;
constexpr int TILE_ITEMS = PART_BLOCK * PART_ITEMS;
constexpr int L1_TILE_BYTES = TILE_ITEMS;
constexpr int L1_TILE_STARTS = L1_TILE_BYTES - CHUNK_OVERLAP;
constexpr int L1_LANES_WITH_STARTS = L1_TILE_STARTS / PART_ITEMS;

__device__ __forceinline__ void lds_barrier() { asm volatile("s_waitcnt lgkmcnt(0)\n\ts_barrier" ::: "memory"); }
__device__ __forceinline__ void spill_put(uint64_t* __restrict__ spill, unsigned long long* __restrict__ spill_n, uint64_t cap, uint64_t key) {
    const unsigned long long at = atomicAdd(spill_n, 1ULL);
    if (at < cap) spill[at] = key;
}

struct PartGeom {
    uint32_t R, S;
    uint32_t P1, P2;
    uint32_t b_lo, b_hi;
    uint32_t l2;
    uint32_t hb;
    uint32_t hb1;
    uint64_t l1_stride;
    uint64_t l1_real;
    uint64_t spill_cap;
    uint32_t cbits;
    Place pl;
};
__device__ __host__ __forceinline__ uint32_t l2_hi_bytes(uint32_t rb) { return rb <= 31 ? 0u : rb <= 39 ? 1u : rb <= 47 ? 2u : 4u; }
template <int HB> struct L2Fmt {
    static constexpr int N = HB == 4 ? 12 : 16;
    static constexpr int TILE = N * 1024;
    static constexpr int NS = TILE + 3 * 1024;
    static constexpr uint32_t GS = 16 + 4 * HB;
    static constexpr uint64_t NONE = HB == 4 ? ~0ULL : (1ULL << (32 + 8 * HB)) - 1;
};
__device__ __host__ __forceinline__ uint32_t l2_tile_items(uint32_t hb) { return hb == 4 ? 12 * 1024 : 16 * 1024; }
__device__ __host__ __forceinline__ constexpr bool l2_blocked(uint32_t hb) { return hb == 1; }
constexpr uint32_t L2_BLOCK_ITEMS = 12, L2_BLOCK_BYTES = 64;
template <int HB> __device__ __host__ __forceinline__ uint64_t l2_lo_at(uint64_t grp) {
    if (l2_blocked(HB)) { const uint64_t b = grp / 3; return b * L2_BLOCK_BYTES + (grp - 3 * b) * 16; }
    return grp * L2Fmt<HB>::GS;
}
template <int HB> __device__ __host__ __forceinline__ uint64_t l2_hi_at(uint64_t grp) {
    if (l2_blocked(HB)) { const uint64_t b = grp / 3; return b * L2_BLOCK_BYTES + 48 + (grp - 3 * b) * 4; }
    return grp * L2Fmt<HB>::GS + 16;
}
__device__ __host__ __forceinline__ uint64_t l2_buffer_bytes(uint32_t hb, uint64_t items) { return l2_blocked(hb) ? (items / L2_BLOCK_ITEMS + 2) * L2_BLOCK_BYTES : items / 4 * (16 + 4 * hb); }
__device__ __host__ __forceinline__ double l2_bytes_per_item(uint32_t hb) { return l2_blocked(hb) ? (double)L2_BLOCK_BYTES / L2_BLOCK_ITEMS : 4.0 + hb; }
__device__ __host__ __forceinline__ uint32_t l2_run_align(uint32_t hb) { return l2_blocked(hb) ? L2_BLOCK_ITEMS : 4u; }
template <int HB> struct HiWord { typedef uint32_t type; };
template <> struct HiWord<1> { typedef uint8_t type; };
template <> struct HiWord<2> { typedef uint16_t type; };
template <int HB>
__device__ __forceinline__ void l2_put(uint8_t* __restrict__ buf, uint64_t i, uint64_t rem) {
    reinterpret_cast<uint32_t*>(buf + l2_lo_at<HB>(i >> 2))[i & 3] = (uint32_t)rem;
    if (HB) reinterpret_cast<typename HiWord<HB>::type*>(buf + l2_hi_at<HB>(i >> 2))[i & 3] = (typename HiWord<HB>::type)(rem >> 32);
}
template <int HB>
__device__ __forceinline__ uint64_t l2_get(const uint8_t* __restrict__ buf, uint64_t i) {
    const uint32_t l = reinterpret_cast<const uint32_t*>(buf + l2_lo_at<HB>(i >> 2))[i & 3];
    const uint32_t h = HB ? (uint32_t)reinterpret_cast<const typename HiWord<HB>::type*>(buf + l2_hi_at<HB>(i >> 2))[i & 3] : 0u;
    return ((uint64_t)h << 32) | l;
}
typedef uint32_t u32x4 __attribute__((ext_vector_type(4)));
typedef uint32_t u32x2 __attribute__((ext_vector_type(2)));
typedef u32x4 u32x4_a4 __attribute__((aligned(4)));
typedef u32x2 u32x2_a4 __attribute__((aligned(4)));
template <int HB> struct HiGroup { typedef uint32_t type; typedef uint32_t mem; };
template <> struct HiGroup<2> { typedef u32x2 type; typedef u32x2_a4 mem; };
template <> struct HiGroup<4> { typedef u32x4 type; typedef u32x4_a4 mem; };
template <int HB>
__device__ __forceinline__ uint32_t hi_of_group(const typename HiGroup<HB>::type& h, int q);
template <> __device__ __forceinline__ uint32_t hi_of_group<0>(const uint32_t&, int) { return 0; }
template <> __device__ __forceinline__ uint32_t hi_of_group<1>(const uint32_t& h, int q) { return (h >> (8 * q)) & 0xFF; }
template <> __device__ __forceinline__ uint32_t hi_of_group<2>(const u32x2& h, int q) { return ((q < 2 ? h.x : h.y) >> (16 * (q & 1))) & 0xFFFF; }
template <> __device__ __forceinline__ uint32_t hi_of_group<4>(const u32x4& h, int q) { return q == 0 ? h.x : q == 1 ? h.y : q == 2 ? h.z : h.w; }
template <int HB>
__device__ __forceinline__ void l2_store_group(uint8_t* __restrict__ buf, uint64_t grp, const u32x4& lo, const typename HiGroup<HB>::type& hi) {
    uint8_t* p = buf + grp * L2Fmt<HB>::GS;
    *reinterpret_cast<u32x4_a4*>(p) = lo;
    if (HB) *reinterpret_cast<typename HiGroup<HB>::mem*>(p + 16) = hi;
}
template <int HB>
struct L2Run {
    const uint8_t* p;
    uint32_t r0;
    __device__ __forceinline__ L2Run(const uint8_t* __restrict__ buf, uint64_t g0) {
        if constexpr (l2_blocked(HB)) { const uint64_t q0 = g0 / 3; r0 = (uint32_t)(g0 - 3 * q0); p = buf + q0 * L2_BLOCK_BYTES; }
        else { r0 = 0; p = buf + g0 * L2Fmt<HB>::GS; }
    }
    __device__ __forceinline__ void load(uint32_t gi, u32x4& lo, typename HiGroup<HB>::type& hi) const {
        if constexpr (l2_blocked(HB)) {
            const uint32_t x = r0 + gi, blk = __umulhi(x, 0xAAAAAAABu) >> 1, part = x - 3 * blk;
            const uint8_t* q = p + ((uint64_t)blk << 6);
            lo = *reinterpret_cast<const u32x4*>(q + 16 * part);
            hi = *reinterpret_cast<const uint32_t*>(q + 48 + 4 * part);
        } else {
            const uint8_t* q = p + (uint64_t)gi * L2Fmt<HB>::GS;
            lo = *reinterpret_cast<const u32x4_a4*>(q);
            if (HB) hi = *reinterpret_cast<const typename HiGroup<HB>::mem*>(q + 16);
        }
    }
};

template <int HB>
struct P2Lds {
    uint64_t cursor[MAX_PARTS];
    uint32_t hist[MAX_PARTS];
    uint32_t goff[MAX_PARTS];
    uint32_t wave_tot[32];
    uint32_t pad_[32];
    uint32_t st_lo[L2Fmt<HB>::TILE];
    typename HiWord<HB>::type st_hi[HB ? L2Fmt<HB>::TILE : 4];
};
static_assert(sizeof(P2Lds<0>) <= 160 * 1024 && sizeof(P2Lds<1>) <= 160 * 1024 && sizeof(P2Lds<2>) <= 160 * 1024 && sizeof(P2Lds<4>) <= 160 * 1024, "LDS");

__device__ __forceinline__ uint32_t block_exclusive_scan(uint32_t v, uint32_t* wave_tot, uint32_t* total) {
    const uint32_t lane = threadIdx.x & 63, wave = threadIdx.x >> 6;
    const uint32_t inc = wave_inclusive_scan(v);
    if (lane == 63) wave_tot[wave] = inc;
    lds_barrier();
    const uint32_t sc = wave_inclusive_scan(lane < PART_BLOCK / 64 ? wave_tot[lane] : 0u);
    const uint32_t wv = (uint32_t)__builtin_amdgcn_readfirstlane((int)wave);
    *total = lane_value(sc, PART_BLOCK / 64 - 1);
    const uint32_t prefix = wv ? lane_value(sc, (int)wv - 1) : 0u;
    lds_barrier();
    return prefix + inc - v;
}

__device__ __forceinline__ uint64_t block_exclusive_scan64(uint64_t v, uint64_t* wave_tot) {
    const uint32_t lane = threadIdx.x & 63, wave = threadIdx.x >> 6;
    uint64_t inc = v;
#pragma unroll
    for (int d = 1; d < 64; d <<= 1) { uint64_t o = __shfl_up(inc, d, 64); if (lane >= (uint32_t)d) inc += o; }
    lds_barrier();
    if (lane == 63) wave_tot[wave] = inc;
    lds_barrier();
    uint64_t prefix = 0;
#pragma unroll
    for (int w = 0; w < PART_BLOCK / 64; ++w) { uint64_t x = wave_tot[w]; if ((uint32_t)w < wave) prefix += x; }
    lds_barrier();
    return prefix + inc - v;
}

static __global__ void __launch_bounds__(PART_BLOCK)
k_p1_scan(PartGeom g, uint32_t n_wg, const uint32_t* __restrict__ hist1, uint64_t* __restrict__ offs, uint64_t* __restrict__ l1_off) {
    __shared__ uint64_t s_base[MAX_PARTS + 1];
    const uint32_t b = threadIdx.x;
    uint64_t tot = 0;
    if (b < g.P1) for (uint32_t w = 0; w < n_wg; ++w) tot += hist1[(uint64_t)w * g.P1 + b];
    if (b < g.P1) s_base[b] = tot;
    lds_barrier();
    if (b == 0) {
        uint64_t run = 0;
        for (uint32_t i = 0; i < g.P1; ++i) { uint64_t v = s_base[i]; s_base[i] = run; run += v; }
        s_base[g.P1] = run;
    }
    lds_barrier();
    if (b < g.P1) l1_off[b] = s_base[b];
    if (b == 0) l1_off[g.P1] = s_base[g.P1];
    if (b < g.P1) {
        uint64_t run = s_base[b];
        for (uint32_t w = 0; w < n_wg; ++w) { offs[(uint64_t)w * g.P1 + b] = run; run += hist1[(uint64_t)w * g.P1 + b]; }
    }
}

constexpr int P1_BLOCK = 512;
constexpr int P1_TILE_BYTES = P1_BLOCK * PART_ITEMS;
constexpr int P1_TILE_STARTS = P1_TILE_BYTES - CHUNK_OVERLAP;
constexpr int P1_LANES_WITH_STARTS = P1_TILE_STARTS / PART_ITEMS;

__device__ __host__ __forceinline__ uint64_t l1_bucket_base(uint64_t first_item, uint32_t b) { return 8 * first_item + 32ULL * b; }
template <uint32_t HB1>
__device__ __forceinline__ void l1_put(uint8_t* __restrict__ bucket, uint64_t group_byte, uint32_t q, uint32_t lo, uint32_t hi) {
    uint8_t* grp = bucket + group_byte;
    if (HB1 == 4) { reinterpret_cast<uint64_t*>(grp)[q] = ((uint64_t)hi << 32) | lo; return; }
    reinterpret_cast<uint32_t*>(grp)[q] = lo;
    if (HB1 == 1) grp[16 + q] = (uint8_t)hi;
    else if (HB1 == 2) reinterpret_cast<uint16_t*>(grp + 16)[q] = (uint16_t)hi;
}
__device__ __forceinline__ void l1_put_any(uint8_t* __restrict__ bucket, uint64_t group_byte, uint32_t q, uint32_t hb1, uint32_t lo, uint32_t hi) {
    if (hb1 == 0) l1_put<0>(bucket, group_byte, q, lo, hi);
    else if (hb1 == 1) l1_put<1>(bucket, group_byte, q, lo, hi);
    else if (hb1 == 2) l1_put<2>(bucket, group_byte, q, lo, hi);
    else l1_put<4>(bucket, group_byte, q, lo, hi);
}

template <bool LEAN = false, bool SEG = false, int PB = MAX_PARTS>
struct P1LdsT {
    typedef typename std::conditional<SEG, uint32_t, uint64_t>::type cursor_t;
    cursor_t cursor[PB];
    uint32_t hist[PB + (LEAN ? 64 : 0)];
    uint32_t real[SEG ? PB : 1];
    uint32_t off[PB + (LEAN ? 64 : 0)];
    uint32_t wave_tot[16];
    uint32_t code[P1_BLOCK + 2];
    uint16_t bad[P1_BLOCK + 2];
    uint32_t rcode[LEAN ? P1_BLOCK + 2 : 1];
    uint32_t pad_[2];
    uint32_t pos[P1_TILE_BYTES + (SEG ? 3 * PB : 0) + (LEAN ? 128 : 0)];
};
static_assert(P1_BLOCK == (int)LEAN_BLOCK, "kg_l1_lean.hpp: the staged entries' arithmetic is written for this tile");
constexpr uint32_t P1_RCW = LEAN_RCW;
constexpr uint32_t P1_PAD = 0xFFFF0000u;

__device__ __forceinline__ uint64_t kmer_at(const uint32_t* code, uint32_t p, uint32_t k, bool canonical) {
    const uint32_t w = p >> 4, o = p & 15;
    const uint32_t c0 = code[w], c1 = code[w + 1], c2 = code[w + 2];
    const uint32_t sh = (32 - 2 * o) & 31;
    const uint32_t h1 = o ? __builtin_amdgcn_alignbit(c0, c1, sh) : c0, h0 = o ? __builtin_amdgcn_alignbit(c1, c2, sh) : c1;
    const uint64_t hi = ((uint64_t)h1 << 32) | h0;
    return canon_if(hi >> (64 - 2 * k), k, canonical);
}

__device__ __forceinline__ u32x4 p1_tile_issue(const uint8_t* __restrict__ bases, uint64_t n, uint64_t tile_off) {
    const uint64_t off = tile_off + (uint64_t)threadIdx.x * PART_ITEMS;
    return *reinterpret_cast<const u32x4*>(bases + (off + PART_ITEMS <= n ? off : 0));
}
__device__ __forceinline__ void p1_tile_fix(const uint8_t* __restrict__ bases, uint64_t n, uint64_t tile_off, const u32x4& v, uint32_t (&w)[4]) {
    const uint64_t off = tile_off + (uint64_t)threadIdx.x * PART_ITEMS;
    w[0] = v.x; w[1] = v.y; w[2] = v.z; w[3] = v.w;
    if (off + PART_ITEMS > n) {
#pragma unroll
        for (int q = 0; q < 4; ++q) {
            uint32_t x = 0;
#pragma unroll
            for (int b = 0; b < 4; ++b) { uint64_t i = off + q * 4 + b; x |= (i < n ? (uint32_t)bases[i] : (uint32_t)'N') << (8 * b); }
            w[q] = x;
        }
    }
}

__device__ __forceinline__ void p1_tile_load(const uint8_t* __restrict__ bases, uint64_t n, uint64_t tile_off, uint32_t (&w)[4]) {
    load16<true>(bases, n, tile_off + (uint64_t)threadIdx.x * PART_ITEMS, w);
}

template <bool LEAN, bool SEG, int PB>
__device__ __forceinline__ void p1_tile_stage(P1LdsT<LEAN, SEG, PB>& L, const uint32_t (&w)[4]) {
    const uint32_t tid = threadIdx.x;
    uint32_t code, bad;
    encode16(w, code, bad);
    L.code[tid] = code;
    L.bad[tid] = (uint16_t)bad;
    if (LEAN) L.rcode[P1_BLOCK - 1 - tid] = lean_revcomp16(code);
    if (tid < 2) { L.code[P1_BLOCK + tid] = 0; L.bad[P1_BLOCK + tid] = 0xFFFF; if (LEAN) L.rcode[P1_BLOCK + tid] = 0; }
    lds_barrier();
}

__device__ __forceinline__ void p1_scan_pair(uint32_t v0, uint32_t v1, uint32_t* wave_tot, uint32_t& e0, uint32_t& e1) {
    const uint32_t lane = threadIdx.x & 63, wave = threadIdx.x >> 6;
    const uint32_t i0 = wave_inclusive_scan(v0), i1 = wave_inclusive_scan(v1);
    lds_barrier();
    if (lane == 63) { wave_tot[wave] = i0; wave_tot[8 + wave] = i1; }
    lds_barrier();
    const uint32_t sc = wave_inclusive_scan(lane < 16 ? wave_tot[lane] : 0u);
    const uint32_t wv = (uint32_t)__builtin_amdgcn_readfirstlane((int)wave);
    const uint32_t p0 = wv ? lane_value(sc, (int)wv - 1) : 0u;
    const uint32_t p1 = lane_value(sc, 7 + (int)wv);
    e0 = p0 + i0 - v0;
    e1 = p1 + i1 - v1;
}

static __global__ void __launch_bounds__(P1_BLOCK)
k_p1v2_count(DevTable t, PartGeom g, const uint8_t* __restrict__ bases, uint64_t n, uint64_t n_tiles, uint64_t tiles_per_wg,
             uint32_t* __restrict__ hist1) {
    __shared__ uint32_t s_hist[MAX_PARTS];
    __shared__ StagedTile<P1_BLOCK, 2> s;
    const uint32_t tid = threadIdx.x;
    const bool canonical = t.canonical != 0;
    for (uint32_t b = tid; b < MAX_PARTS; b += P1_BLOCK) s_hist[b] = 0;
    uint32_t ones = 0;
    const uint64_t t0 = (uint64_t)blockIdx.x * tiles_per_wg, t1 = min(t0 + tiles_per_wg, n_tiles);
    u32x4 raw = p1_tile_issue(bases, n, (t0 < t1 ? t0 : 0) * P1_TILE_STARTS);
    for (uint64_t tile = t0; tile < t1; ++tile) {
        uint32_t w[4];
        p1_tile_fix(bases, n, tile * P1_TILE_STARTS, raw, w);
        raw = p1_tile_issue(bases, n, (tile + 1 < t1 ? tile + 1 : tile) * P1_TILE_STARTS);
        lds_barrier();
        uint32_t code, bad;
        encode16(w, code, bad);
        s.stage(code, bad); s.pad();
        lds_barrier();
        if (tid < P1_LANES_WITH_STARTS) {
            LaneWindow lw;
            lw.init(s.code, s.bad, tid, t.k);
#pragma unroll 4
            for (int j = 0; j < PART_ITEMS; ++j, lw.step()) {
                if (!lw.valid()) continue;
                const uint64_t key = canon_if(lw.fwd(), t.k, canonical);
                if (key == EMPTY) { ++ones; continue; }
                atomicAdd(&s_hist[place_digit1_of(key, g.pl)], 1u);
            }
        }
    }
    lds_barrier();
    for (uint32_t b = tid; b < g.P1; b += P1_BLOCK) hist1[(uint64_t)blockIdx.x * g.P1 + b] = s_hist[b];
    for (int off = 32; off > 0; off >>= 1) ones += __shfl_down(ones, off, 64);
    if ((tid & 63) == 0 && ones) atomicAdd((unsigned long long*)&t.ctrs[CTR_ONES], (unsigned long long)ones);
}

template <bool SEG, bool LEAN = false, int PB = MAX_PARTS>
__global__ void __launch_bounds__(P1_BLOCK, SEG && PB == 512 ? 6 : 4)
k_p1v2_scatter(DevTable t, PartGeom g, const uint8_t* __restrict__ bases, uint64_t n, uint64_t n_tiles, uint64_t tiles_per_wg,
               const uint64_t* __restrict__ offs, const uint64_t* __restrict__ l1_off, uint8_t* __restrict__ l1_buf, uint32_t seg_cap ,
               uint32_t bucket_stride ,
               uint32_t seg_real ,
               uint64_t* __restrict__ ovf_buf, unsigned long long* __restrict__ ovf_n, uint64_t ovf_cap) {
    __shared__ __attribute__((aligned(16))) P1LdsT<LEAN, SEG, PB> L;
    typedef typename P1LdsT<LEAN, SEG, PB>::cursor_t cursor_t;
    typedef P1LdsT<LEAN, SEG, PB> P1Lds_t;
    static_assert(!LEAN || offsetof(P1Lds_t, rcode) - offsetof(P1Lds_t, code) == 4 * P1_RCW, "the copy-out reads code | bad | rcode as one array");
    const uint32_t tid = threadIdx.x, P = g.P1, k = t.k;
    const bool canonical = t.canonical != 0;
    const uint32_t hb1 = g.hb1, gs1 = 16 + 4 * hb1;
    const bool grouped = SEG && hb1 != 4;
    uint32_t ones = 0;
    const uint64_t seg_off = SEG ? (uint64_t)blockIdx.x * (seg_cap >> 2) * gs1 : 0;
    for (uint32_t b = tid; b < P; b += P1_BLOCK) { L.cursor[b] = SEG ? (cursor_t)0 : (cursor_t)(offs[(uint64_t)blockIdx.x * P + b] - l1_off[b]); if (SEG) L.real[b] = 0; }
    constexpr uint32_t DUMP0 = LEAN ? sizeof(L.pos) / 4 - 128 : 0;
    static_assert(DUMP0 % 4 == 0, "dump slots");
    if (LEAN && tid < 64) L.off[PB + tid] = grouped ? DUMP0 / 4 : DUMP0;
    const uint64_t t0 = (uint64_t)blockIdx.x * tiles_per_wg, t1 = min(t0 + tiles_per_wg, n_tiles);
    u32x4 raw = p1_tile_issue(bases, n, (t0 < t1 ? t0 : 0) * P1_TILE_STARTS);
    for (uint64_t tile = t0; tile < t1; ++tile) {
        uint32_t w[4];
        p1_tile_fix(bases, n, tile * P1_TILE_STARTS, raw, w);
        lds_barrier();
        for (uint32_t b = tid; b < PB + (LEAN ? 64 : 0); b += P1_BLOCK) L.hist[b] = 0;
        p1_tile_stage(L, w);
        uint32_t br[PART_ITEMS];
        uint32_t valid = 0;
        if (LEAN) {
            const LeanGeom lg = lean_geom(k, canonical, g.pl.n1);
            const uint32_t v16 = tid < P1_LANES_WITH_STARTS ? lean_valid16(L.bad[tid], L.bad[tid + 1], L.bad[tid + 2], k) : 0u;
            LeanWin w{L.code[tid], L.code[tid + 1], L.code[tid + 2], 0, 0};
            uint32_t f_hi, f_lo;
            lean_fwd(w, lg, f_hi, f_lo);
            { const uint64_t rc0 = kmer_revcomp(((uint64_t)f_hi << 32) | f_lo, k); w.rc_hi = (uint32_t)(rc0 >> 32); w.rc_lo = (uint32_t)rc0; }
            valid = v16;
            const uint32_t dump = PB + (tid & 63);
            uint32_t rk[PART_ITEMS];
#pragma unroll
            for (int j = 0; j < PART_ITEMS; ++j) {
                if (j) { lean_step(w); lean_fwd(w, lg, f_hi, f_lo); lean_rc_roll(w, lg, f_lo); }
                uint32_t key_hi, key_lo;
                bool took_rc;
                const uint32_t b = lean_digit1(w, lg, g.pl, f_hi, f_lo, key_hi, key_lo, took_rc);
                const bool ok = (v16 & (0x8000u >> j)) != 0;
                const uint32_t sel = ok ? b : dump;
                rk[j] = atomicAdd(&L.hist[sel], 1u);
                br[j] = (sel << 16) | (took_rc ? 0x8000u : 0u);
                if (j >= 2) br[j - 2] |= rk[j - 2];
            }
#pragma unroll
            for (int j = PART_ITEMS - 2; j < PART_ITEMS; ++j) br[j] |= rk[j];
        }
        if (!LEAN && tid < P1_LANES_WITH_STARTS) {
            LaneWindow lw;
            lw.init(L.code, L.bad, tid, k);
            uint64_t rc = kmer_revcomp(lw.fwd(), k);
            const uint32_t top = 2 * k - 2;
#pragma unroll
            for (int j = 0; j < PART_ITEMS; ++j) {
                if (j) { lw.step(); rc = (rc >> 2) | ((uint64_t)(3u ^ ((uint32_t)lw.fwd() & 3u)) << top); }
                br[j] = 0;
                if (!lw.valid()) continue;
                const uint64_t fw = lw.fwd();
                const uint64_t key = canonical ? (rc < fw ? rc : fw) : fw;
                if (key == EMPTY) { if (SEG) ++ones; continue; }
                const uint32_t b = place_digit1_of(key, g.pl);
                br[j] = (b << 16) | atomicAdd(&L.hist[b], 1u);
                valid |= 1u << j;
            }
        }
        raw = p1_tile_issue(bases, n, (tile + 1 < t1 ? tile + 1 : tile) * P1_TILE_STARTS);
        lds_barrier();
        uint32_t e0, e1;
        {
            const uint32_t h0 = tid < P ? L.hist[tid] : 0, h1 = PB > P1_BLOCK && tid + P1_BLOCK < P ? L.hist[tid + P1_BLOCK] : 0;
            p1_scan_pair(grouped ? (h0 + 3) >> 2 : h0, grouped ? (h1 + 3) >> 2 : h1, L.wave_tot, e0, e1);
            L.off[tid] = e0;
            if (PB > P1_BLOCK) L.off[tid + P1_BLOCK] = e1;
            if (grouped) {
                for (uint32_t q = h0; q & 3; ++q) L.pos[4 * e0 + q] = P1_PAD;
                if (PB > P1_BLOCK) for (uint32_t q = h1; q & 3; ++q) L.pos[4 * e1 + q] = P1_PAD;
            }
        }
        lds_barrier();
        if (LEAN) {
            uint32_t run0[PART_ITEMS];
#pragma unroll
            for (int j = 0; j < PART_ITEMS; ++j) run0[j] = L.off[br[j] >> 16];
            const uint32_t gshift = grouped ? 2u : 0u;
            uint32_t base_f = tid * 32u;
            asm volatile("" : "+v"(base_f));
            const uint32_t Q = (uint32_t)P1_TILE_BYTES - 1u - k;
#pragma unroll
            for (int j = 0; j < PART_ITEMS; ++j) {
                asm volatile("" : "+v"(run0[j]));
                const uint32_t cj = lean_entry_fwd(j), sj = lean_entry_rc(Q - (uint32_t)j);
                uint32_t on_rc = (uint32_t)((int32_t)(br[j] << 16) >> 31);
                asm volatile("" : "+v"(on_rc));
                const uint32_t e = ((sj - base_f) & on_rc) | ((base_f + cj) & ~on_rc);
                L.pos[(run0[j] << gshift) + (br[j] & 0x7FFFu)] = (br[j] & 0xFFFF0000u) | (e & 0xFFFFu);
            }
        } else {
#pragma unroll
            for (int j = 0; j < PART_ITEMS; ++j)
                if (valid >> j & 1) {
                    const uint32_t run0 = L.off[br[j] >> 16];
                    L.pos[(grouped ? 4 * run0 : run0) + (br[j] & 0xFFFFu)] = (br[j] & 0xFFFF0000u) | (tid * PART_ITEMS + j);
                }
        }
        lds_barrier();
        auto entry_src = [&](uint32_t v, const uint32_t*& src, int32_t& wd, uint32_t& sh) {
            if (LEAN) {
                src = L.code - 1;
                wd = (int32_t)((v >> 5) & 0x7FFu); sh = v;
                return;
            }
            const uint32_t p = v & 0xFFFFu;
            const int32_t q = (int32_t)p - 1;
            src = L.code;
            wd = q >> 4; sh = 2u * (~(uint32_t)q & 15u);
        };
        auto entry_key = [&](uint32_t c0, uint32_t c1, uint32_t c2, uint32_t sh) -> uint64_t {
            const uint32_t h1 = __builtin_amdgcn_alignbit(c0, c1, sh), h0 = __builtin_amdgcn_alignbit(c1, c2, sh);
            uint64_t key1 = (((uint64_t)h1 << 32) | h0) >> (64 - 2 * k);
            if (!LEAN) key1 = canon_if(key1, k, canonical);
            return key1;
        };
        const uint32_t lastb = P - 1;
        const uint32_t total = L.off[lastb] + (grouped ? (L.hist[lastb] + 3) >> 2 : L.hist[lastb]);
        auto copy_out_groups = [&](auto hb1_tag) {
            constexpr int HB1 = decltype(hb1_tag)::value;
            const uint32_t seg_groups = seg_cap >> 2;
            for (uint32_t gi = tid; gi < total; gi += P1_BLOCK) {
                const u32x4 e = *reinterpret_cast<const u32x4*>(&L.pos[4 * gi]);
                const uint32_t ev[4] = {e.x, e.y, e.z, e.w};
                const uint32_t b = e.x >> 16;
                uint32_t c0[4], c1[4], c2[4], o[4];
#pragma unroll
                for (int q = 0; q < 4; ++q) {
                    const uint32_t* src; int32_t wd;
                    entry_src(ev[q], src, wd, o[q]);
                    c0[q] = src[wd]; c1[q] = src[wd + 1]; c2[q] = src[wd + 2];
                }
                const uint32_t gahead = gi - L.off[b];
                const uint32_t grel = ((uint32_t)L.cursor[b] >> 2) + gahead;
                uint32_t re = L.real[b];
                asm volatile("" : "+v"(re));
                const bool room = (grel < seg_groups) & (re + 4 * gahead + 4 <= seg_real);
                uint32_t lo[4], hi[4];
#pragma unroll
                for (int q = 0; q < 4; ++q) {
                    const uint32_t pad = (uint32_t)((int32_t)ev[q] >> 31);
                    if (LEAN) {
                        const uint32_t h1 = __builtin_amdgcn_alignbit(c0[q], c1[q], o[q]), h0 = __builtin_amdgcn_alignbit(c1[q], c2[q], o[q]);
                        lo[q] = __builtin_amdgcn_alignbit(h1, h0, 64 - 2 * k) | pad;
                        hi[q] = __builtin_amdgcn_ubfe(h1, 64 - 2 * k, g.pl.n1 - 32) | pad;
                    } else {
                        const uint64_t r1 = entry_key(c0[q], c1[q], c2[q], o[q]) & g.pl.m1;
                        lo[q] = (uint32_t)r1 | pad;
                        hi[q] = (uint32_t)(r1 >> 32) | pad;
                    }
                }
                if (room) {
                    const u32x4 glo = {lo[0], lo[1], lo[2], lo[3]};
                    typename HiGroup<HB1>::type ghi{};
                    if constexpr (HB1 == 1) ghi = (hi[0] & 0xFFu) | ((hi[1] & 0xFFu) << 8) | ((hi[2] & 0xFFu) << 16) | (hi[3] << 24);
                    if constexpr (HB1 == 2) { ghi.x = (hi[0] & 0xFFFFu) | (hi[1] << 16); ghi.y = (hi[2] & 0xFFFFu) | (hi[3] << 16); }
                    uint8_t* segp = l1_buf + ((uint64_t)b * bucket_stride + seg_off);
                    l2_store_group<HB1>(segp, grel, glo, ghi);
                } else {
#pragma unroll
// ... 232 lines not shown
        const uint64_t rem = ((uint64_t)(HB ? (uint32_t)L.st_hi[idx] : 0u) << 32) | L.st_lo[idx];
        l2_put<HB>(out, L.cursor[lo_b] + (idx - L.goff[lo_b]), rem);
    }
    lds_barrier();
    if (tid < P) L.cursor[tid] += mine;
}

template <int HB>
struct P2FLds {
    static constexpr bool CARRY = HB != 4;
    uint32_t cur[MAX_PARTS];
    uint32_t hist[MAX_PARTS + 64];
    uint32_t goff[MAX_PARTS];
    uint32_t wave_tot[32];
    uint32_t pad_[32];
    static constexpr uint32_t CBASE = L2Fmt<HB>::NS;
    uint32_t st_lo[L2Fmt<HB>::NS + (CARRY ? 3 * MAX_PARTS : 0)];
    typename HiWord<HB>::type st_hi[HB ? L2Fmt<HB>::NS + (CARRY ? 3 * MAX_PARTS : 0) : 4];
    uint16_t grp_b[L2Fmt<HB>::NS / 4];
};
static_assert(sizeof(P2FLds<0>) <= 160 * 1024 - 256 && sizeof(P2FLds<1>) <= 160 * 1024 - 256 && sizeof(P2FLds<2>) <= 160 * 1024 - 256 && sizeof(P2FLds<4>) <= 160 * 1024 - 256, "LDS");

template <int HB, bool W1, bool STAMP = false>
__device__ __forceinline__ void scatter_tile2_fast(P2FLds<HB>& L, const PartGeom g, const uint32_t b1, const TileItems<L2Fmt<HB>::N, W1>& key, uint32_t valid,
                                                   uint8_t* __restrict__ out , uint32_t capg ,
                                                   uint64_t* __restrict__ ovf_buf, unsigned long long* __restrict__ ovf_n, uint64_t ovf_cap, uint32_t& carry_n,
                                                   unsigned long long* st = nullptr ) {
    constexpr int N = L2Fmt<HB>::N;
    constexpr bool CARRY = P2FLds<HB>::CARRY;
    auto now = [&]() -> unsigned long long { return STAMP ? (unsigned long long)clock64() : 0ULL; };
    const unsigned long long t0 = now();
    typedef typename HiWord<HB>::type hi_t;
    const uint32_t tid = threadIdx.x;
    const uint32_t P = g.P2;
    if (tid < MAX_PARTS) L.hist[tid] = CARRY ? carry_n : 0u;
    lds_barrier();
    uint32_t br[N];
    {
        uint32_t rk[N];
        const uint32_t dump = MAX_PARTS + (tid & 63);
#pragma unroll
        for (int j = 0; j < N; ++j) {
            const uint32_t b = place_digit2_of(key.r1(j), g.pl) & (MAX_PARTS - 1);
            rk[j] = atomicAdd(&L.hist[(valid >> j & 1) ? b : dump], 1u);
            br[j] = b << 16;
            if (j >= 2) br[j - 2] |= rk[j - 2];
        }
#pragma unroll
        for (int j = N - 2; j < N; ++j) br[j] |= rk[j];
    }
    lds_barrier();
    const unsigned long long t1 = now();
    uint32_t total;
    const uint32_t mine = tid < P ? L.hist[tid] : 0;
    const uint32_t mygroups = CARRY ? mine >> 2 : (mine + 3) >> 2;
    const uint32_t excl = block_exclusive_scan(mygroups, L.wave_tot, &total);
    if (tid < MAX_PARTS) L.goff[tid] = CARRY ? excl | (mygroups << 16) : excl;
    if (tid < P) {
        if (CARRY) {
            if (mygroups) for (uint32_t q = 0; q < carry_n; ++q) { L.st_lo[excl * 4 + q] = L.st_lo[P2FLds<HB>::CBASE + 3 * tid + q]; if (HB) L.st_hi[excl * 4 + q] = L.st_hi[P2FLds<HB>::CBASE + 3 * tid + q]; }
        } else {
            for (uint32_t q = mine; q & 3; ++q) { L.st_lo[excl * 4 + q] = 0xFFFFFFFFu; if (HB) L.st_hi[excl * 4 + q] = (hi_t)~(hi_t)0; }
        }
        for (uint32_t gq = 0; gq < mygroups; ++gq) L.grp_b[excl + gq] = (uint16_t)tid;
    }
    lds_barrier();
    const unsigned long long t2 = now();
    constexpr int SB = N % 8 == 0 && !W1 ? 8 : 4;
    static_assert(N % SB == 0, "batches");
    uint32_t go[SB];
#pragma unroll
    for (int j = 0; j < N; ++j) {
        if (j % SB == 0) {
#pragma unroll
            for (int q = 0; q < SB; ++q) go[q] = L.goff[br[j + q] >> 16];
#pragma unroll
            for (int q = 0; q < SB; ++q) asm volatile("" : "+v"(go[q]));
        }
        if (valid >> j & 1) {
            const uint32_t b = br[j] >> 16, r = br[j] & 0xFFFF, gf = go[j % SB];
            const uint64_t rem = key.r1(j) & g.pl.mr;
            if (CARRY) {
                const uint32_t whole = (gf >> 16) * 4u;
                const uint32_t slot = r < whole ? (gf & 0xFFFFu) * 4u + r : P2FLds<HB>::CBASE + 3 * b + (r - whole);
                L.st_lo[slot] = (uint32_t)rem;
                if (HB) L.st_hi[slot] = (hi_t)(rem >> 32);
            } else {
                const uint32_t slot = gf * 4u + r;
                L.st_lo[slot] = (uint32_t)rem;
                if (HB) L.st_hi[slot] = (hi_t)(rem >> 32);
            }
        }
    }
    lds_barrier();
    const unsigned long long t3 = now();
    for (uint32_t gi0 = tid; gi0 < total; gi0 += 2 * PART_BLOCK) {
        uint32_t b[2], ahead[2];
        u32x4 lo[2];
        typename HiGroup<HB>::type hi[2];
        bool in[2];
#pragma unroll
        for (int u = 0; u < 2; ++u) { const uint32_t gi = gi0 + u * PART_BLOCK; in[u] = gi < total; b[u] = L.grp_b[in[u] ? gi : gi0]; }
#pragma unroll
        for (int u = 0; u < 2; ++u) {
            const uint32_t gi = in[u] ? gi0 + u * PART_BLOCK : gi0;
            ahead[u] = L.cur[b[u]] + (gi - (CARRY ? L.goff[b[u]] & 0xFFFFu : L.goff[b[u]]));
            lo[u] = *reinterpret_cast<const u32x4*>(&L.st_lo[gi * 4]);
            hi[u] = typename HiGroup<HB>::type{};
            if (HB) hi[u] = *reinterpret_cast<const typename HiGroup<HB>::type*>(&L.st_hi[gi * 4]);
        }
#pragma unroll
        for (int u = 0; u < 2; ++u) {
            if (!in[u]) continue;
            if (ahead[u] < capg) l2_store_group<HB>(out, (uint64_t)b[u] * capg + ahead[u], lo[u], hi[u]);
            else {
#pragma unroll
                for (int q = 0; q < 4; ++q) {
                    const uint64_t rem = ((uint64_t)hi_of_group<HB>(hi[u], q) << 32) | (q == 0 ? lo[u].x : q == 1 ? lo[u].y : q == 2 ? lo[u].z : lo[u].w);
                    if (rem == L2Fmt<HB>::NONE) continue;
                    const unsigned long long at = atomicAdd(ovf_n, 1ULL);
                    if (at < ovf_cap) ovf_buf[at] = place_key_d(b1, b[u], rem, g.pl);
                }
            }
        }
    }
    lds_barrier();
    if (STAMP && st) { const unsigned long long t4 = now(); st[1] += t1 - t0; st[2] += t2 - t1; st[3] += t3 - t2; st[4] += t4 - t3; }
    if (tid < P) { const uint32_t c = L.cur[tid] + mygroups; L.cur[tid] = c < capg ? c : capg; }
    if (CARRY) carry_n = mine & 3;
}

template <int HB>
__device__ __forceinline__ void flush_carry2(P2FLds<HB>& L, const PartGeom g, const uint32_t b1, uint8_t* __restrict__ out, uint32_t capg,
                                             uint64_t* __restrict__ ovf_buf, unsigned long long* __restrict__ ovf_n, uint64_t ovf_cap, uint32_t carry_n) {
    const uint32_t tid = threadIdx.x;
    if (tid >= g.P2 || !carry_n) return;
    uint32_t lo[4], hi[4];
#pragma unroll
    for (int q = 0; q < 4; ++q) {
        const bool have = (uint32_t)q < carry_n;
        lo[q] = have ? L.st_lo[P2FLds<HB>::CBASE + 3 * tid + (q < 3 ? q : 0)] : 0xFFFFFFFFu;
        hi[q] = have && HB ? (uint32_t)L.st_hi[HB ? P2FLds<HB>::CBASE + 3 * tid + (q < 3 ? q : 0) : 0] : 0xFFFFFFFFu;
    }
    const uint32_t c = L.cur[tid];
    if (c < capg) {
        const u32x4 glo = {lo[0], lo[1], lo[2], lo[3]};
        typename HiGroup<HB>::type ghi{};
        if constexpr (HB == 1) ghi = (hi[0] & 0xFFu) | ((hi[1] & 0xFFu) << 8) | ((hi[2] & 0xFFu) << 16) | (hi[3] << 24);
        if constexpr (HB == 2) { ghi.x = (hi[0] & 0xFFFFu) | (hi[1] << 16); ghi.y = (hi[2] & 0xFFFFu) | (hi[3] << 16); }
        l2_store_group<HB>(out, (uint64_t)tid * capg + c, glo, ghi);
        L.cur[tid] = c + 1;
    } else {
        for (uint32_t q = 0; q < carry_n; ++q) {
            const uint64_t rem = ((uint64_t)(HB ? hi[q] & (HB == 1 ? 0xFFu : 0xFFFFu) : 0u) << 32) | lo[q];
            const unsigned long long at = atomicAdd(ovf_n, 1ULL);
            if (at < ovf_cap) ovf_buf[at] = place_key_d(b1, tid, rem, g.pl);
        }
    }
}

struct P2BLds {
    static constexpr int TILE = L2Fmt<1>::TILE;
    uint32_t hist[MAX_PARTS + 64];
    uint32_t goff[MAX_PARTS];
    uint32_t wave_tot[32];
    uint32_t pad_[32];
    uint32_t cb[MAX_PARTS * 16];
    uint32_t st_lo[TILE];
    uint8_t st_hi[TILE + 16];
    uint16_t blk_b[TILE / 12 + 2];
};
static_assert(sizeof(P2BLds) <= 160 * 1024 - 256 && offsetof(P2BLds, cb) % 64 == 0 && offsetof(P2BLds, st_lo) % 16 == 0 && offsetof(P2BLds, st_hi) % 4 == 0, "LDS");
template <int HB> struct P2FastLds { typedef P2FLds<HB> type; };
template <> struct P2FastLds<1> { typedef P2BLds type; };

template <typename HiFn>
__device__ __forceinline__ void blk_overflow(const PartGeom& g, uint32_t b1, uint32_t b, const u32x4& lo, HiFn hi8, uint64_t* __restrict__ ovf_buf, unsigned long long* __restrict__ ovf_n, uint64_t ovf_cap) {
#pragma unroll
    for (int q = 0; q < 4; ++q) {
        const uint64_t rem = ((uint64_t)hi8(q) << 32) | (q == 0 ? lo.x : q == 1 ? lo.y : q == 2 ? lo.z : lo.w);
        if (rem == L2Fmt<1>::NONE) continue;
        const unsigned long long at = atomicAdd(ovf_n, 1ULL);
        if (at < ovf_cap) ovf_buf[at] = place_key_d(b1, b, rem, g.pl);
    }
}

template <bool W1, bool STAMP = false, typename Prefetch>
__device__ __forceinline__ void scatter_tile2_blk(P2BLds& L, const PartGeom g, const uint32_t b1, const TileItems<16, W1>& key, uint32_t valid,
                                                  uint8_t* __restrict__ out, uint32_t capb, uint64_t* __restrict__ ovf_buf, unsigned long long* __restrict__ ovf_n, uint64_t ovf_cap,
                                                  uint32_t& carry_n, unsigned long long* st, Prefetch prefetch ) {
    constexpr int N = 16;
    auto now = [&]() -> unsigned long long { return STAMP ? (unsigned long long)clock64() : 0ULL; };
    const unsigned long long t0 = now();
    const uint32_t tid = threadIdx.x, P = g.P2;
    uint8_t* const cb8 = reinterpret_cast<uint8_t*>(L.cb);
    L.hist[tid] = carry_n;
    lds_barrier();
    uint32_t br[N];
    {
        uint32_t rk[N];
        const uint32_t dump = MAX_PARTS + (tid & 63);
#pragma unroll
        for (int j = 0; j < N; ++j) {
            const uint32_t b = place_digit2_of(key.r1(j), g.pl) & (MAX_PARTS - 1);
            rk[j] = atomicAdd(&L.hist[(valid >> j & 1) ? b : dump], 1u);
            br[j] = b << 16;
            if (j >= 2) br[j - 2] |= rk[j - 2];
        }
#pragma unroll
        for (int j = N - 2; j < N; ++j) br[j] |= rk[j];
    }
    lds_barrier();
    const unsigned long long t1 = now();
    prefetch();
    const uint32_t avail = tid < P ? L.hist[tid] : 0;
    const uint32_t nblk = __umulhi(avail, 0xAAAAAAABu) >> 3;
    const uint32_t nstg = nblk ? nblk - 1 : 0;
    uint32_t total;
    const uint32_t excl = block_exclusive_scan(nstg, L.wave_tot, &total);
    L.goff[tid] = excl | (nblk << 16);
    for (uint32_t q = 0; q < nstg; ++q) L.blk_b[excl + q] = (uint16_t)tid;
    lds_barrier();
    const unsigned long long t2 = now();
    {
        constexpr int SB = 4;
        uint32_t go[SB];
#pragma unroll
        for (int j = 0; j < N; ++j) {
            if (j % SB == 0) {
#pragma unroll
                for (int q = 0; q < SB; ++q) go[q] = L.goff[br[j + q] >> 16];
#pragma unroll
                for (int q = 0; q < SB; ++q) asm volatile("" : "+v"(go[q]));
            }
            uint32_t later = 0;
            if (valid >> j & 1) {
                const uint32_t b = br[j] >> 16, v = br[j] & 0xFFFF, gf = go[j % SB], whole = (gf >> 16) * 12u;
                const uint64_t rem = key.r1(j) & g.pl.mr;
                if (v < 12) { L.cb[b * 16 + v] = (uint32_t)rem; cb8[b * 64 + 48 + v] = (uint8_t)(rem >> 32); }
                else if (v < whole) { const uint32_t slot = (gf & 0xFFFFu) * 12u + (v - 12); L.st_lo[slot] = (uint32_t)rem; L.st_hi[slot] = (uint8_t)(rem >> 32); }
                else later = 0x80000000u | (b << 4) | (v - whole);
            }
            br[j] = later;
        }
    }
    lds_barrier();
    const unsigned long long t3 = now();
    for (uint32_t qi = tid; qi < 4 * P; qi += PART_BLOCK) {
        const uint32_t b = qi >> 2, w = qi & 3;
        const uint32_t nb = L.goff[b] >> 16, cur = L.cb[b * 16 + 15];
        const u32x4 v = *reinterpret_cast<const u32x4*>(&L.cb[b * 16 + 4 * w]);
        if (nb) {
            if (cur < capb) *reinterpret_cast<u32x4*>(out + (((uint64_t)b * capb + cur) << 6) + 16 * w) = v;
            else if (w < 3) blk_overflow(g, b1, b, v, [&](int q) -> uint32_t { return cb8[b * 64 + 48 + 4 * w + q]; }, ovf_buf, ovf_n, ovf_cap);
        }
    }
    for (uint32_t qi = tid; qi < 4 * total; qi += PART_BLOCK) {
        const uint32_t s = qi >> 2, w = qi & 3;
        const uint32_t b = L.blk_b[s];
        const uint32_t gf = L.goff[b], cur = L.cb[b * 16 + 15];
        const u32x4 lo = *reinterpret_cast<const u32x4*>(&L.st_lo[12 * s + 4 * (w < 3 ? w : 0)]);
        const uint32_t* h = reinterpret_cast<const uint32_t*>(&L.st_hi[12 * s]);
        const u32x4 hv = {h[0], h[1], h[2], 0xFFFFFFFFu};
        const uint32_t dst = cur + 1 + (s - (gf & 0xFFFFu));
        if (dst < capb) *reinterpret_cast<u32x4*>(out + (((uint64_t)b * capb + dst) << 6) + 16 * w) = w < 3 ? lo : hv;
        else if (w < 3) blk_overflow(g, b1, b, lo, [&](int q) -> uint32_t { return L.st_hi[12 * s + 4 * w + q]; }, ovf_buf, ovf_n, ovf_cap);
    }
    lds_barrier();
#pragma unroll
    for (int j = 0; j < N; ++j)
        if (br[j] & 0x80000000u) {
            const uint32_t b = (br[j] >> 4) & (MAX_PARTS - 1), v = br[j] & 15u;
            const uint64_t rem = key.r1(j) & g.pl.mr;
            L.cb[b * 16 + v] = (uint32_t)rem; cb8[b * 64 + 48 + v] = (uint8_t)(rem >> 32);
        }
    if (tid < P) { const uint32_t c = L.cb[tid * 16 + 15] + nblk; L.cb[tid * 16 + 15] = c < capb ? c : capb; }
    carry_n = avail - 12 * nblk;
    if (STAMP && st) { const unsigned long long t4 = now(); st[1] += t1 - t0; st[2] += t2 - t1; st[3] += t3 - t2; st[4] += t4 - t3; }
}

__device__ __forceinline__ uint32_t flush_carry_blk(P2BLds& L, const PartGeom g, const uint32_t b1, uint8_t* __restrict__ out, uint32_t capb,
                                                    uint64_t* __restrict__ ovf_buf, unsigned long long* __restrict__ ovf_n, uint64_t ovf_cap, uint32_t carry_n) {
    const uint32_t tid = threadIdx.x, P = g.P2;
    uint8_t* const cb8 = reinterpret_cast<uint8_t*>(L.cb);
    lds_barrier();
    if (tid < P && carry_n) for (uint32_t q = carry_n; q < 12; ++q) { L.cb[tid * 16 + q] = 0xFFFFFFFFu; cb8[tid * 64 + 48 + q] = 0xFF; }
    L.goff[tid] = carry_n;
    lds_barrier();
    for (uint32_t qi = tid; qi < 4 * P; qi += PART_BLOCK) {
        const uint32_t b = qi >> 2, w = qi & 3;
        const uint32_t cn = L.goff[b], cur = L.cb[b * 16 + 15];
        const u32x4 v = *reinterpret_cast<const u32x4*>(&L.cb[b * 16 + 4 * w]);
        if (cn) {
            if (cur < capb) *reinterpret_cast<u32x4*>(out + (((uint64_t)b * capb + cur) << 6) + 16 * w) = v;
            else if (w < 3) blk_overflow(g, b1, b, v, [&](int q) -> uint32_t { return cb8[b * 64 + 48 + 4 * w + q]; }, ovf_buf, ovf_n, ovf_cap);
        }
    }
    lds_barrier();
    uint32_t blocks = 0;
    if (tid < P) { const uint32_t c = L.cb[tid * 16 + 15]; blocks = carry_n && c < capb ? c + 1 : c; }
    return blocks;
}

__device__ __host__ __forceinline__ uint64_t p2_exact_base(uint64_t beg, uint32_t b1, uint32_t P2) { return (beg + 4 * ((uint64_t)P2 + 1) * b1 + 3) & ~3ULL; }

template <int HB, bool W1 , bool L1B = false >
__global__ void __launch_bounds__(PART_BLOCK)
k_p2(PartGeom g, const uint64_t* __restrict__ l1_off, const uint8_t* __restrict__ l1_buf, uint8_t* __restrict__ l2_buf,
     uint64_t* __restrict__ off2, uint64_t seg_slots, uint64_t* __restrict__ bend ) {
    extern __shared__ __attribute__((aligned(16))) unsigned char lds_raw[];
    P2Lds<HB>& L = *reinterpret_cast<P2Lds<HB>*>(lds_raw);
    constexpr int N = L2Fmt<HB>::N;
    const uint32_t tid = threadIdx.x;
    uint64_t beg0, n0, nr0;
    l1_bucket_range(g, l1_off, seg_slots, g.b_lo, beg0, n0, nr0);
    for (uint32_t b1 = g.b_lo + blockIdx.x; b1 < g.b_hi; b1 += gridDim.x) {
        uint64_t beg, n_items, n_real;
        const uint8_t* bucket = l1_buf + l1_bucket_range(g, l1_off, seg_slots, b1, beg, n_items, n_real);
        const uint64_t obeg = p2_exact_base(beg, b1, g.P2) - p2_exact_base(beg0, g.b_lo, g.P2);
        lds_barrier();
        unsigned long long* h64 = reinterpret_cast<unsigned long long*>(L.cursor);
        if (tid < MAX_PARTS) h64[tid] = 0;
        lds_barrier();
        for (uint64_t tbeg = 0; tbeg < n_items; tbeg += L2Fmt<HB>::TILE) {
            TileItems<N, W1> key;
            const uint32_t valid = p2_tile_load<N, W1, L1B>(g.hb1, bucket, tbeg, n_items, key);
#pragma unroll
            for (int j = 0; j < N; ++j)
                if (valid >> j & 1) atomicAdd(&h64[place_digit2_of(key.r1(j), g.pl)], 1ULL);
        }
        lds_barrier();
        const uint64_t mine = tid < g.P2 ? h64[tid] : 0;
        const uint64_t excl = block_exclusive_scan64((mine + 3) & ~3ULL, reinterpret_cast<uint64_t*>(L.st_lo));
        if (tid < g.P2) {
            const uint64_t start = obeg + excl;
            L.cursor[tid] = start;
            off2[(uint64_t)b1 * g.P2 + tid] = start;
            for (uint64_t q = mine; q & 3; ++q) l2_put<HB>(l2_buf, start + q, L2Fmt<HB>::NONE);
        }
        if (b1 == g.b_hi - 1 && tid == g.P2 - 1) off2[(uint64_t)g.b_hi * g.P2] = obeg + excl + ((mine + 3) & ~3ULL);
        if (bend && tid == g.P2 - 1) bend[b1] = obeg + excl + ((mine + 3) & ~3ULL);
        for (uint64_t tbeg = 0; tbeg < n_items; tbeg += L2Fmt<HB>::TILE) {
            TileItems<N, W1> key;
            const uint32_t valid = p2_tile_load<N, W1, L1B>(g.hb1, bucket, tbeg, n_items, key);
            lds_barrier();
            scatter_tile2<HB, W1>(L, g, key, valid, l2_buf);
        }
    }
}

constexpr uint32_t P2_RUN_SLACK = 48;
__device__ __host__ __forceinline__ uint64_t p2_region_cap(uint64_t n_b, uint32_t P2, uint32_t tile, uint32_t al = 4) {
    const uint64_t c = ((n_b + (n_b >> 4)) >> (31 - __builtin_clz(P2))) + 2 * (n_b / tile + 1) + 16;
    return (c + al - 1) / al * al;
}
__device__ __host__ __forceinline__ uint64_t p2_out_base(uint64_t beg, uint32_t b1, uint32_t P2, uint32_t tile, uint32_t al = 4) {
    const uint64_t o = beg + (beg >> 4) + 2 * (uint64_t)P2 * (beg / tile) + (uint64_t)b1 * P2 * P2_RUN_SLACK;
    return (o + al - 1) / al * al;
}

template <int HB, bool W1, bool STAMP = false, bool L1B = false >
__global__ void __launch_bounds__(PART_BLOCK)
k_p2_fast(PartGeom g, const uint64_t* __restrict__ l1_off, const uint8_t* __restrict__ l1_buf, uint8_t* __restrict__ l2_buf,
          uint64_t* __restrict__ off2, uint32_t* __restrict__ cnt2, uint64_t* __restrict__ ovf_buf, unsigned long long* __restrict__ ovf_n,
          uint64_t ovf_cap, uint64_t seg_slots, unsigned long long* __restrict__ stamps = nullptr) {
    unsigned long long st[6] = {0, 0, 0, 0, 0, 0};
    extern __shared__ __attribute__((aligned(16))) unsigned char lds_raw[];
    typedef typename P2FastLds<HB>::type Lds;
    Lds& L = *reinterpret_cast<Lds*>(lds_raw);
    constexpr int N = L2Fmt<HB>::N;
    constexpr bool BLK = l2_blocked(HB);
    constexpr uint32_t AL = BLK ? L2_BLOCK_ITEMS : 4;
    const uint32_t tid = threadIdx.x;
    uint64_t beg0, n0, nr0;
    l1_bucket_range(g, l1_off, seg_slots, g.b_lo, beg0, n0, nr0);
    for (uint32_t b1 = g.b_lo + blockIdx.x; b1 < g.b_hi; b1 += gridDim.x) {
        uint64_t beg, n_items, n_real;
        const uint8_t* bucket = l1_buf + l1_bucket_range(g, l1_off, seg_slots, b1, beg, n_items, n_real);
        const uint64_t cap = p2_region_cap(n_real, g.P2, L2Fmt<HB>::TILE, AL);
        const uint64_t obase = p2_out_base(beg, b1, g.P2, L2Fmt<HB>::TILE, AL) - p2_out_base(beg0, g.b_lo, g.P2, L2Fmt<HB>::TILE, AL);
        uint8_t* runs = l2_buf + l2_lo_at<HB>(obase >> 2);
        const uint32_t capg = (uint32_t)(cap / AL);
        lds_barrier();
        uint32_t carry_n = 0;
        uint32_t tid_b = tid;
        asm volatile("" : "+v"(tid_b));
        if (tid < g.P2) {
            if constexpr (BLK) L.cb[tid * 16 + 15] = 0; else L.cur[tid] = 0;
            off2[(uint64_t)b1 * g.P2 + tid_b] = obase + (uint64_t)tid * cap;
        }
        if constexpr (BLK && !W1) {
            typename std::conditional<L1B, RawTileB<N>, RawTile<N>>::type raw;
            auto issue = [&](uint64_t at) { if constexpr (L1B) p2_tile_issue_l1b<N>(bucket, at, raw); else p2_tile_issue_narrow<N>(g.hb1, bucket, at, raw); };
            issue(0);
            for (uint64_t tbeg = 0; tbeg < n_items; tbeg += L2Fmt<HB>::TILE) {
                const unsigned long long ta = STAMP ? (unsigned long long)clock64() : 0ULL;
                TileItems<N, W1> key;
                uint32_t valid;
                if constexpr (L1B) valid = p2_tile_decode_l1b<N>(tbeg, n_items, raw, key); else valid = p2_tile_decode_narrow<N>(g.hb1, tbeg, n_items, raw, key);
                if (STAMP) { __builtin_amdgcn_s_waitcnt(0); }
                lds_barrier();
                if (STAMP) { st[0] += (unsigned long long)clock64() - ta; st[5] += 1; }
                scatter_tile2_blk<W1, STAMP>(L, g, b1, key, valid, runs, capg, ovf_buf, ovf_n, ovf_cap, carry_n, st,
                                             [&]() { issue(tbeg + L2Fmt<HB>::TILE); });
            }
        } else
        for (uint64_t tbeg = 0; tbeg < n_items; tbeg += L2Fmt<HB>::TILE) {
            const unsigned long long ta = STAMP ? (unsigned long long)clock64() : 0ULL;
            TileItems<N, W1> key;
            const uint32_t valid = p2_tile_load<N, W1, L1B>(g.hb1, bucket, tbeg, n_items, key);
            if (STAMP) { __builtin_amdgcn_s_waitcnt(0); }
            lds_barrier();
            if (STAMP) { st[0] += (unsigned long long)clock64() - ta; st[5] += 1; }
            if constexpr (BLK) scatter_tile2_blk<W1, STAMP>(L, g, b1, key, valid, runs, capg, ovf_buf, ovf_n, ovf_cap, carry_n, st, []() {});
            else scatter_tile2_fast<HB, W1, STAMP>(L, g, b1, key, valid, runs, capg, ovf_buf, ovf_n, ovf_cap, carry_n, st);
        }
        if constexpr (BLK) {
            const uint32_t blocks = flush_carry_blk(L, g, b1, runs, capg, ovf_buf, ovf_n, ovf_cap, carry_n);
            asm volatile("" : "+v"(tid_b));
            if (tid < g.P2) cnt2[(uint64_t)b1 * g.P2 + tid_b] = blocks * L2_BLOCK_ITEMS;
        } else {
            lds_barrier();
            if constexpr (P2FLds<HB>::CARRY) { flush_carry2<HB>(L, g, b1, runs, capg, ovf_buf, ovf_n, ovf_cap, carry_n); lds_barrier(); }
            if (tid < g.P2) cnt2[(uint64_t)b1 * g.P2 + tid] = L.cur[tid] << 2;
        }
    }
    if (STAMP && tid == 0 && stamps) for (int i = 0; i < 6; ++i) atomicAdd(&stamps[i], st[i]);
}

}
#include "kg_l2_blocks.hpp"
namespace kg {

constexpr int AP2_QCAP = 256;
constexpr int AP2_LANE_PROBES = 12;
constexpr uint64_t AP2_SEGMENT = 0x7FF00000ULL;

template <int BLOCK, int KP , int U, int NR, int HB , bool STAMP = false, bool INLINE_CLAIM = false, bool DYN = true,
          int QCAP = AP2_QCAP ,
          bool TEST_SPILL = false >
__global__ void __launch_bounds__(BLOCK)
k_p3_apply2(DevTable t, PartGeom g, const uint64_t* __restrict__ off2, const uint8_t* __restrict__ l2_buf,
            uint64_t* __restrict__ spill, unsigned long long* __restrict__ spill_n,
            const uint32_t* __restrict__ cnt2, const uint64_t* __restrict__ bend, unsigned long long* __restrict__ stamps = nullptr, uint32_t spill_mod = 0,
            uint64_t seg_len = AP2_SEGMENT ) {
    unsigned long long st[7] = {0, 0, 0, 0, 0, 0, 0};
    auto now = [&]() -> unsigned long long { return STAMP ? (unsigned long long)clock64() : 0ULL; };
    extern __shared__ __attribute__((aligned(16))) unsigned char lds_raw[];
    constexpr int NW = BLOCK / 64, CP = (KP + 1) / 2;
    constexpr uint32_t CH = 64 * U;
    static_assert(U == 4, "a lane takes one group of the level-2 buffer: four items");
    const uint32_t S = g.S;
    unsigned long long* rk = reinterpret_cast<unsigned long long*>(lds_raw);
    uint32_t* rc = reinterpret_cast<uint32_t*>(lds_raw + (size_t)S * 8);
    const uint32_t tid = threadIdx.x, lane = tid & 63, wave = tid >> 6;
    unsigned long long* wqk = reinterpret_cast<unsigned long long*>(lds_raw + (size_t)S * 12) + (size_t)wave * QCAP;
    uint32_t* wqs = reinterpret_cast<uint32_t*>(lds_raw + (size_t)S * 12 + (size_t)NW * QCAP * 8) + (size_t)wave * QCAP;
    uint32_t new_distinct = 0;
    u32x4 kq[KP], cq[CP];
    __shared__ unsigned long long s_next_chunk;

    const uint32_t r_hi = g.b_hi * g.P2;
    auto run_end = [&](uint32_t r) -> uint64_t {
        if (bend && (r + 1) % g.P2 == 0) return bend[r / g.P2];
        return off2[r + 1];
    };
    auto next_region = [&](uint32_t from) {
        uint32_t r = from;
        while (r < r_hi && (cnt2 ? cnt2[r] == 0 : off2[r] == run_end(r))) r += gridDim.x;
        return r;
    };
    auto prefetch = [&](uint32_t r) {
        const uint64_t base = (uint64_t)r * S;
#pragma unroll
        for (int u = 0; u < KP; ++u) { const uint32_t i = (u * BLOCK + tid) * 2; kq[u] = *reinterpret_cast<const u32x4*>(t.keys + base + (i < S ? i : 0)); }
#pragma unroll
        for (int u = 0; u < CP; ++u) { const uint32_t i = (u * BLOCK + tid) * 4; cq[u] = *reinterpret_cast<const u32x4*>(t.counts + base + (i < S ? i : 0)); }
    };

    uint32_t r = next_region(g.b_lo * g.P2 + blockIdx.x);
    if (r < r_hi) prefetch(r);
    while (r < r_hi) {
        const uint64_t beg = off2[r], end = cnt2 ? beg + cnt2[r] : run_end(r);
        const uint64_t base = (uint64_t)r * S;
        const unsigned long long t_top = now();
#pragma unroll
        for (int u = 0; u < KP; ++u) { const uint32_t i = (u * BLOCK + tid) * 2; if (i < S) *reinterpret_cast<u32x4*>(rk + i) = kq[u]; }
#pragma unroll
        for (int u = 0; u < CP; ++u) { const uint32_t i = (u * BLOCK + tid) * 4; if (i < S) *reinterpret_cast<u32x4*>(rc + i) = cq[u]; }
        const uint32_t rn = next_region(r + gridDim.x);
        const uint32_t rd1 = r >> g.l2, rd2 = r & (g.P2 - 1);

        for (uint64_t sbeg = beg; sbeg < end; sbeg += seg_len) {
            const uint64_t n_run = (end - sbeg < seg_len ? end - sbeg : seg_len);
            if (tid == 0) s_next_chunk = NW;
            lds_barrier();
#pragma unroll 1
            for (int u = 0; u < CP; ++u) {
                const uint32_t i = (u * BLOCK + tid) * 4;
                if (i >= S) break;
                const u32x4 c = *reinterpret_cast<const u32x4*>(rc + i);
                if (!((c.x | c.y | c.z | c.w) & 0x80000000u)) continue;
#pragma unroll 1
                for (uint32_t j = 0; j < 4; ++j)
                    if (rc[i + j] & 0x80000000u) { rc[i + j] -= 0x80000000u; ovf_add(t, rk[i + j], 0x80000000ULL); }
            }
            lds_barrier();
            st[0] += now() - t_top;

            uint32_t q_n = 0;
            auto add1 = [&](uint32_t slot) { (void)__hip_atomic_fetch_add(&rc[slot], 1u, __ATOMIC_RELAXED, __HIP_MEMORY_SCOPE_WORKGROUP); };
            auto drain_pass = [&](bool fin ) {
                const uint32_t take = q_n < 64 ? q_n : 64;
                q_n -= take;
                bool live = lane < take;
                unsigned long long key = EMPTY; uint32_t slot = 0, budget = 0;
                if (live) { key = wqk[q_n + lane]; const uint32_t s = wqs[q_n + lane]; slot = s & 0xFFFF; budget = s >> 16; }
#pragma unroll 1
                for (int rr = 0; rr < AP2_LANE_PROBES; ++rr) {
                    const int busy = __popcll(__ballot(live));
                    if (busy == 0 || (busy < 8 && (fin || rr >= 4))) break;
                    if (live) {
                        unsigned long long c0 = rk[slot];
                        if (c0 == EMPTY) {
                            c0 = atomicCAS(&rk[slot], (unsigned long long)EMPTY, key);
                            if (c0 == EMPTY) { ++new_distinct; c0 = key; }
                        }
                        if (c0 == key) { add1(slot); live = false; }
                        else {
                            slot = slot + 1 == S ? 0 : slot + 1;
                            if (--budget == 0) { spill_put(spill, spill_n, g.spill_cap, key); live = false; }
                        }
                    }
                }
                const bool lng = live && (fin || S - budget >= (uint32_t)(AP2_LANE_PROBES + NR));
                {
                    const bool back = live && !lng;
                    const unsigned long long m = __ballot(back);
                    if (m) {
                        const uint32_t at = q_n + __builtin_amdgcn_mbcnt_hi((uint32_t)(m >> 32), __builtin_amdgcn_mbcnt_lo((uint32_t)m, 0));
                        if (back) { wqk[at] = key; wqs[at] = slot | (budget << 16); }
                        q_n += (uint32_t)__popcll(m);
                    }
                }
                unsigned long long todo = __ballot(lng);
#pragma unroll 1
                while (todo) {
                    const int src = __ffsll((long long)todo) - 1;
                    todo &= todo - 1;
                    const unsigned long long ck = lane_value((uint64_t)key, src);
                    uint32_t cs = lane_value(slot, src);
                    int cb = (int)lane_value(budget, src);
#pragma unroll 1
                    for (;;) {
                        uint32_t idx = cs + lane; if (idx >= S) idx -= S;
                        const unsigned long long c0 = rk[idx];
                        const unsigned long long mk = __ballot(c0 == ck), me = __ballot(c0 == EMPTY);
                        if (!(mk | me)) {
                            cb -= 64; cs = cs + 64 >= S ? cs + 64 - S : cs + 64;
                            if (cb <= 0) { if (lane == 0) spill_put(spill, spill_n, g.spill_cap, ck); break; }
                            continue;
                        }
                        const int first = __ffsll((long long)(mk | me)) - 1;
                        if (first >= cb) { if (lane == 0) spill_put(spill, spill_n, g.spill_cap, ck); break; }
                        unsigned long long got = ck;
                        if (!((mk >> first) & 1)) {
                            unsigned long long old = EMPTY;
                            if ((int)lane == first) old = atomicCAS(&rk[idx], (unsigned long long)EMPTY, ck);
                            old = lane_value((uint64_t)old, first);
                            if (old == EMPTY) { if ((int)lane == first) ++new_distinct; }
                            else got = old;
                        }
                        if (got == ck) { if ((int)lane == first) add1(idx); break; }
                        cb -= first; cs = cs + first >= S ? cs + first - S : cs + first;
                    }
                }
            };

            const uint64_t n_chunks = (n_run + CH - 1) / CH;
            const uint64_t n_grp = (n_run + 3) >> 2, g0 = sbeg >> 2;
            unsigned long long cur[U];
            u32x4 c_lo, n_lo;
            typename HiGroup<HB>::type c_hi{}, n_hi{};
            bool c_in, n_in;
            const L2Run<HB> run(l2_buf, g0);
            { const uint64_t gi = (uint64_t)wave * 64 + lane; c_in = gi < n_grp; run.load(c_in ? (uint32_t)gi : 0u, c_lo, c_hi); }
            auto grab = [&]() -> uint64_t {
                unsigned long long v = 0;
                if (lane == 0) v = atomicAdd(&s_next_chunk, 1ULL);
                return lane_value((uint64_t)v, 0);
            };
            for (uint64_t c = wave; c < n_chunks;) {
                const unsigned long long t_a = now();
                const uint64_t c_next = DYN ? grab() : c + NW;
                {
                    const uint64_t gi = c_next * 64 + lane;
                    n_in = gi < n_grp;
                    run.load(n_in ? (uint32_t)gi : 0u, n_lo, n_hi);
                }
                uint32_t slot[U];
                bool pend[U];
#pragma unroll
                for (int u = 0; u < U; ++u) {
                    const uint64_t rem = ((uint64_t)hi_of_group<HB>(c_hi, u) << 32) | (u == 0 ? c_lo.x : u == 1 ? c_lo.y : u == 2 ? c_lo.z : c_lo.w);
                    pend[u] = c_in && rem != L2Fmt<HB>::NONE;
                    slot[u] = place_offset(rem, g.pl, S);
                    cur[u] = place_key_d(rd1, rd2, rem, g.pl);
                    if (TEST_SPILL && spill_mod && pend[u] && __umulhi((uint32_t)(mix64(cur[u]) >> 32), spill_mod) == 0) { spill_put(spill, spill_n, g.spill_cap, cur[u]); pend[u] = false; }
                }
                const unsigned long long t_b = now();
#pragma unroll
                for (int rr = 0; rr < NR; ++rr) {
                    unsigned long long seen[U];
#pragma unroll
                    for (int u = 0; u < U; ++u) { seen[u] = EMPTY; if (pend[u]) seen[u] = rk[slot[u]]; }
                    bool claim[U];
#pragma unroll
                    for (int u = 0; u < U; ++u) {
                        const bool hit = pend[u] && seen[u] == cur[u];
                        if (hit) add1(slot[u]);
                        pend[u] = pend[u] && !hit;
                        claim[u] = pend[u] && seen[u] == EMPTY;
                        const uint32_t nx = slot[u] + 1 == S ? 0 : slot[u] + 1;
                        slot[u] = (pend[u] && !claim[u]) ? nx : slot[u];
                    }
                    bool any_claim = false;
#pragma unroll
                    for (int u = 0; u < U; ++u) any_claim = any_claim || claim[u];
                    if (INLINE_CLAIM && __any(any_claim)) {
                        unsigned long long got[U];
#pragma unroll
                        for (int u = 0; u < U; ++u) { got[u] = 0; if (claim[u]) got[u] = atomicCAS(&rk[slot[u]], (unsigned long long)EMPTY, cur[u]); }
#pragma unroll
                        for (int u = 0; u < U; ++u) {
                            if (claim[u]) {
                                if (got[u] == EMPTY) ++new_distinct;
                                const bool mine = got[u] == EMPTY || got[u] == cur[u];
                                if (mine) add1(slot[u]);
                                pend[u] = !mine;
                                if (!mine) slot[u] = slot[u] + 1 == S ? 0 : slot[u] + 1;
                            }
                        }
                    }
                }
                if (STAMP) { __builtin_amdgcn_s_waitcnt(0); }
                const unsigned long long t_c = now();
                unsigned long long pm_u[U];
                uint32_t total = 0;
#pragma unroll
                for (int u = 0; u < U; ++u) { pm_u[u] = __ballot(pend[u]); total += (uint32_t)__popcll(pm_u[u]); }
                if (total <= QCAP - 64) {
                    uint32_t at = q_n;
#pragma unroll
                    for (int u = 0; u < U; ++u) {
                        if (pend[u]) {
                            const uint32_t i = at + __builtin_amdgcn_mbcnt_hi((uint32_t)(pm_u[u] >> 32), __builtin_amdgcn_mbcnt_lo((uint32_t)pm_u[u], 0));
                            wqk[i] = cur[u]; wqs[i] = slot[u] | ((S - NR) << 16);
                        }
                        at += (uint32_t)__popcll(pm_u[u]);
                    }
                    q_n += total;
                } else {
                    uint32_t pm = 0;
#pragma unroll
                    for (int u = 0; u < U; ++u) pm |= pend[u] ? 1u << u : 0u;
#pragma unroll 1
                    for (int it = 0; it < U; ++it) {
                        const bool p = pm & 1;
                        const unsigned long long m = __ballot(p);
                        if (m) {
                            while (q_n > QCAP - 64) drain_pass(false);
                            const uint32_t at = q_n + __builtin_amdgcn_mbcnt_hi((uint32_t)(m >> 32), __builtin_amdgcn_mbcnt_lo((uint32_t)m, 0));
                            if (p) { wqk[at] = cur[0]; wqs[at] = slot[0] | ((S - NR) << 16); }
                            q_n += (uint32_t)__popcll(m);
                        }
                        pm >>= 1;
#pragma unroll
                        for (int u = 0; u + 1 < U; ++u) { cur[u] = cur[u + 1]; slot[u] = slot[u + 1]; }
                    }
                }
                const bool last = c_next >= n_chunks;
                while (q_n > (last ? 0u : 64u)) drain_pass(last);
                c_lo = n_lo; c_hi = n_hi; c_in = n_in;
// ... 373 lines not shown
```

Measured before the change: 111.3 billion.

## Plan partition arena by dense L1 layout and trim level-2 slack for long runs

Moves the arena sizing maths into a shared planning header and carves the arena according to the actual level-1 format (dense 64-byte blocks vs 8-byte items), so more items fit per round. When per-region runs are long, it also trims the level-2 region capacity slack, shrinking the level-2 buffer. Fewer, larger rounds reduce per-round launch and probe overhead. Guard regions are added and checked in test mode, and rounds fall back to exact sizing if the dense path cannot run.

New measurement: 115.5 billion (median of 6 runs). +3.7%, better.

```diff
diff --git a/kat_amd/csrc/kg_arena_plan.hpp b/kat_amd/csrc/kg_arena_plan.hpp
--- /dev/null
+++ b/kat_amd/csrc/kg_arena_plan.hpp
@@ -0,0 +1,140 @@
+#pragma once
+#include <stddef.h>
+#include <stdint.h>
+
+#if defined(__HIPCC__)
+#define KG_PLAN_FN __host__ __device__ __forceinline__
+#else
+#define KG_PLAN_FN inline
+#endif
+
+namespace kg {
+
+constexpr uint32_t PLAN_MAX_PARTS = 1024, PLAN_L1_TILE_STARTS = 8160, PLAN_L1B_TILE_STARTS = 16352, PLAN_L1B_ITEMS = 10, PLAN_L1B_BYTES = 64;
+
+KG_PLAN_FN uint32_t l2_tile_items(uint32_t hb) { return hb == 4 ? 12 * 1024 : 16 * 1024; }
+KG_PLAN_FN constexpr bool l2_blocked(uint32_t hb) { return hb == 1; }
+constexpr uint32_t L2_BLOCK_ITEMS = 12, L2_BLOCK_BYTES = 64;
+KG_PLAN_FN uint64_t l2_buffer_bytes(uint32_t hb, uint64_t items) { return l2_blocked(hb) ? (items / L2_BLOCK_ITEMS + 2) * L2_BLOCK_BYTES : items / 4 * (16 + 4 * hb); }
+KG_PLAN_FN double l2_bytes_per_item(uint32_t hb) { return l2_blocked(hb) ? (double)L2_BLOCK_BYTES / L2_BLOCK_ITEMS : 4.0 + hb; }
+KG_PLAN_FN uint32_t l2_run_align(uint32_t hb) { return l2_blocked(hb) ? L2_BLOCK_ITEMS : 4u; }
+
+KG_PLAN_FN uint64_t l1_bucket_base(uint64_t first_item, uint32_t b) { return 8 * first_item + 32ULL * b; }
+KG_PLAN_FN uint64_t p2_exact_base(uint64_t beg, uint32_t b1, uint32_t P2) { return (beg + 4 * ((uint64_t)P2 + 1) * b1 + 3) & ~3ULL; }
+
+constexpr uint32_t P2_RUN_SLACK = 48;
+constexpr uint64_t P2_LONG_RUN = 16384;
+KG_PLAN_FN bool l2_trims(uint32_t hb, uint64_t round_items, uint64_t regions) { return l2_blocked(hb) && regions && round_items / regions >= P2_LONG_RUN; }
+KG_PLAN_FN uint64_t p2_region_cap(uint64_t n_b, uint32_t P2, uint32_t tile, uint32_t al = 4, bool trim = false) {
+    const uint32_t sh = 31 - __builtin_clz(P2);
+    const uint64_t c = trim ? ((n_b + (n_b >> 5) + (n_b >> 6)) >> sh) + 16 : ((n_b + (n_b >> 4)) >> sh) + 2 * (n_b / tile + 1) + 16;
+    return (c + al - 1) / al * al;
+}
+KG_PLAN_FN uint64_t p2_out_base(uint64_t beg, uint32_t b1, uint32_t P2, uint32_t tile, uint32_t al = 4, bool trim = false) {
+    const uint64_t o = beg + (trim ? (beg >> 5) + (beg >> 6) : (beg >> 4) + 2 * (uint64_t)P2 * (beg / tile)) + (uint64_t)b1 * P2 * P2_RUN_SLACK;
+    return (o + al - 1) / al * al;
+}
+KG_PLAN_FN uint64_t p2_pass_extent(uint64_t nn, uint32_t nb, uint32_t P2, uint32_t tile, bool trim) {
+    const uint64_t fast = nn + (trim ? nn / 32 + nn / 64 : nn / 16 + 2ULL * P2 * (nn / tile + 1)) + (uint64_t)nb * P2 * P2_RUN_SLACK + 64;
+    const uint64_t exact = nn + 4 * ((uint64_t)P2 + 1) * nb + 8;
+    return fast > exact ? fast : exact;
+}
+
+constexpr uint64_t SEG_PAD = 64;
+struct L1Segments {
+    uint64_t seg_cap, cap_plain, stride;
+    bool fits;
+};
+KG_PLAN_FN L1Segments l1_segments(bool blocks, uint32_t P1, uint32_t hb1, uint32_t wgs, uint64_t est_items, uint64_t tiles_per_wg, uint32_t test_cpb, uint64_t l1_bytes) {
+    L1Segments s;
+    uint64_t seg_cap = est_items / ((uint64_t)wgs * P1);
+    seg_cap += seg_cap / 24 + SEG_PAD;
+    if (test_cpb && seg_cap > test_cpb) seg_cap = test_cpb;
+    if (blocks) seg_cap = (seg_cap + PLAN_L1B_ITEMS - 1) / PLAN_L1B_ITEMS * PLAN_L1B_ITEMS;
+    s.cap_plain = seg_cap;
+    if (!blocks && hb1 != 4 && !test_cpb) { const uint64_t pad = 2 * tiles_per_wg; seg_cap += pad < 3 * seg_cap ? pad : 3 * seg_cap; }
+    if (!blocks) seg_cap = (seg_cap + 3) & ~3ULL;
+    s.seg_cap = seg_cap;
+    if (blocks) s.stride = ((uint64_t)wgs * (seg_cap / PLAN_L1B_ITEMS) * PLAN_L1B_BYTES + 32 + 63) & ~63ULL;
+    else { const uint64_t a = 8 * (uint64_t)wgs * s.cap_plain, b = (uint64_t)(4 + hb1) * wgs * seg_cap; s.stride = (a > b ? a : b) + 32; }
+    s.fits = s.stride * P1 <= l1_bytes && seg_cap < (1u << 24) && s.stride <= 0xFFFFFFFFULL;
+    return s;
+}
+
+constexpr size_t ARENA_GUARD = 4096;
+constexpr uint64_t L1_FAST_MIN_ITEMS = (uint64_t)64 << 20;
+KG_PLAN_FN double l1_bytes_per_item(bool dense) { return dense ? (double)PLAN_L1B_BYTES / PLAN_L1B_ITEMS : 8.0; }
+KG_PLAN_FN double l2_items_per_l1_item(uint32_t hb, bool big) { return big && l2_blocked(hb) ? 1 + 3.0 / 64 : 1 + 1.0 / 16 + 2.0 * PLAN_MAX_PARTS / l2_tile_items(hb); }
+KG_PLAN_FN uint64_t ovf_share(bool big) { return big ? 64 : 32; }
+KG_PLAN_FN double arena_bytes_per_item(uint32_t hb, uint32_t passes, bool dense, bool big) {
+    return l1_bytes_per_item(dense) * (1 + 1.0 / 24) + l2_bytes_per_item(hb) * (1 + 1.0 / 24) * l2_items_per_l1_item(hb, big) / passes + 8.0 / ovf_share(big) + 0.002;
+}
+struct ArenaCarve {
+    bool dense, big;
+    double per_item;
+    uint64_t round_items;
+    uint64_t exact_items;
+    uint64_t l1_count, l1_bytes, l2_items, l2_bytes, ovf_cap;
+    uint64_t total_bytes;
+};
+KG_PLAN_FN uint64_t arena_fixed_l1(uint32_t W, uint32_t n_cu, bool dense) { return dense ? (uint64_t)n_cu * 512 * (SEG_PAD + 2 * PLAN_L1B_ITEMS) : (uint64_t)W * PLAN_MAX_PARTS * SEG_PAD; }
+KG_PLAN_FN uint64_t arena_l2_items(uint64_t l1_count, uint32_t hb, uint32_t passes, bool big) {
+    return ((uint64_t)((double)l1_count * l2_items_per_l1_item(hb, big) / passes) + (uint64_t)PLAN_MAX_PARTS * PLAN_MAX_PARTS * P2_RUN_SLACK + 4096 + 11) / 12 * 12;
+}
+KG_PLAN_FN uint64_t arena_fixed_bytes(uint32_t hb, uint32_t passes, uint32_t W, uint32_t n_cu, bool dense, bool big) {
+    const uint64_t f1 = arena_fixed_l1(W, n_cu, dense) + 16;
+    return (uint64_t)((double)f1 * l1_bytes_per_item(dense)) + 256 + l2_buffer_bytes(hb, arena_l2_items(f1, hb, passes, big) + 12) + 16 + 1024 * 8 + 3 * ARENA_GUARD + 4096;
+}
+KG_PLAN_FN ArenaCarve arena_carve_as(uint64_t buf_bytes, uint64_t want_items, uint32_t hb, uint32_t passes, uint32_t W, uint32_t n_cu, bool dense, bool big, uint64_t test_ovf_cap) {
+    ArenaCarve c;
+    c.dense = dense; c.big = big;
+    c.per_item = arena_bytes_per_item(hb, passes, dense, big);
+    const uint64_t fixed = arena_fixed_bytes(hb, passes, W, n_cu, dense, big);
+    const uint64_t by_bytes = buf_bytes > fixed ? (uint64_t)((double)(buf_bytes - fixed) / c.per_item) : 0;
+    c.round_items = want_items < by_bytes ? want_items : by_bytes;
+    c.l1_count = (c.round_items + c.round_items / 24 + arena_fixed_l1(W, n_cu, dense) + 15) & ~(uint64_t)15;
+    c.l1_bytes = dense ? (((c.l1_count / PLAN_L1B_ITEMS + 1) * PLAN_L1B_BYTES + 127) & ~(uint64_t)127) : c.l1_count * 8;
+    c.l2_items = arena_l2_items(c.l1_count, hb, passes, big);
+    c.l2_bytes = (l2_buffer_bytes(hb, c.l2_items) + 15) & ~(uint64_t)15;
+    c.ovf_cap = test_ovf_cap ? test_ovf_cap : c.round_items / ovf_share(big) + 1024;
+    const uint64_t exact = (c.l1_bytes - 32 * ((uint64_t)PLAN_MAX_PARTS + 1)) / 8;
+    c.exact_items = exact < c.round_items ? exact : c.round_items;
+    c.total_bytes = c.l1_bytes + ARENA_GUARD + c.l2_bytes + ARENA_GUARD + c.ovf_cap * 8 + ARENA_GUARD;
+    return c;
+}
+KG_PLAN_FN ArenaCarve arena_carve(uint64_t buf_bytes, uint64_t want_items, uint32_t hb, uint32_t passes, uint32_t W, uint32_t n_cu, uint64_t regions, bool blocks_shape, uint32_t l1_fast, uint64_t test_ovf_cap) {
+    bool dense = blocks_shape && l1_fast != 0;
+    for (;;) {
+        ArenaCarve c = arena_carve_as(buf_bytes, want_items, hb, passes, W, n_cu, dense, false, test_ovf_cap);
+        if (c.round_items < want_items) {
+            const ArenaCarve t = arena_carve_as(buf_bytes, want_items, hb, passes, W, n_cu, dense, true, test_ovf_cap);
+            if (regions && t.round_items / regions >= P2_LONG_RUN) c = t;
+        }
+        if (!dense || l1_fast == 2 || c.round_items >= L1_FAST_MIN_ITEMS) return c;
+        dense = false;
+    }
+}
+KG_PLAN_FN bool round_trims(const ArenaCarve& c, uint32_t hb, uint64_t est_items, uint64_t regions, uint64_t nn, uint32_t nb, uint32_t P2) {
+    return c.big && l2_trims(hb, est_items, regions) && p2_pass_extent(nn, nb, P2, l2_tile_items(hb), false) > c.l2_items;
+}
+
+struct RoundCaps {
+    bool dense_ok = true;
+    KG_PLAN_FN uint64_t cap(const ArenaCarve& c, bool blocks_can_run) const { return dense_ok && blocks_can_run && c.dense ? c.round_items : c.exact_items; }
+    KG_PLAN_FN void exact_from_here() { dense_ok = false; }
+};
+
+KG_PLAN_FN size_t round_starts(size_t left, size_t round_items, double items_per_start) {
+    size_t m = left;
+    if (m > round_items) { const size_t by = (size_t)((double)round_items / items_per_start * 0.98); if (by < m) m = by; }
+    if (m < left) {
+        if (!m) m = 1;
+        const size_t rounds_left = (left + m - 1) / m;
+        m = (left + rounds_left - 1) / rounds_left;
+        m += PLAN_L1_TILE_STARTS - m % PLAN_L1_TILE_STARTS;
+        if (m > left) m = left;
+    }
+    return m;
+}
+
+}
diff --git a/kat_amd/csrc/kg_count.hip b/kat_amd/csrc/kg_count.hip
--- a/kat_amd/csrc/kg_count.hip
+++ b/kat_amd/csrc/kg_count.hip
@@ -88,7 +88,6 @@
 static const uint64_t g_test_round_items = hook("KATGPU_TEST_ROUND_ITEMS") ? strtoull(hook("KATGPU_TEST_ROUND_ITEMS"), nullptr, 10) : 0;
 static const double g_arena_fraction = getenv("KATGPU_ARENA_FRACTION") ? std::min(0.95, std::max(0.05, atof(getenv("KATGPU_ARENA_FRACTION")))) : 0.85;
 static const uint32_t g_p1_wgs = hook("KATGPU_P1_WGS") ? std::max<uint32_t>(1, (uint32_t)strtoul(hook("KATGPU_P1_WGS"), nullptr, 10)) : 3;
-static const bool g_l1_lean = hook_u64("KATGPU_L1_LEAN", 1) != 0;
 static const uint32_t g_l1_fast = hook("KATGPU_L1_FAST") ? (uint32_t)strtoul(hook("KATGPU_L1_FAST"), nullptr, 10) : 1;
 static const uint32_t g_test_l1_cpb = hook("KATGPU_TEST_L1_CPB") ? (uint32_t)strtoul(hook("KATGPU_TEST_L1_CPB"), nullptr, 10) : 0;
 static const uint32_t g_p2_fast = hook("KATGPU_P2_FAST") ? (uint32_t)strtoul(hook("KATGPU_P2_FAST"), nullptr, 10) : 1;
@@ -105,6 +104,7 @@
 static bool part_geometry(const DevTable& d, PartGeom* g) {
     g->R = d.n_regions; g->S = d.region_slots; g->P1 = d.p1; g->P2 = d.p2; g->l2 = d.l2;
     g->b_lo = 0; g->b_hi = d.p1;
+    g->l1_stride = 0; g->l1_real = 0; g->spill_cap = 0; g->l2_trim = 0;
     g->pl = place_make(d.k, d.p1, d.n1, d.l2);
     g->hb = l2_hi_bytes(g->pl.rb);
     g->hb1 = l2_hi_bytes(g->pl.n1);
@@ -112,13 +112,15 @@
     if (d.cbits && g->hb > 2) g->hb = 2;
     return d.k <= 32 && g->pl.rb <= 63  && g->P1 <= MAX_PARTS && g->P2 <= MAX_PARTS && g->S % 4 == 0 && g->S >= 64 && g->S <= AP2_MAX_SLOTS;
 }
-static double l2_items_per_l1_item(uint32_t hb) { return 1 + 1.0 / 16 + 2.0 * MAX_PARTS / l2_tile_items(hb); }
+static_assert(PLAN_MAX_PARTS == MAX_PARTS && PLAN_L1_TILE_STARTS == P1_TILE_STARTS && PLAN_L1B_TILE_STARTS == L1B_TILE_STARTS && PLAN_L1B_ITEMS == L1B_ITEMS && PLAN_L1B_BYTES == L1B_BYTES,
+              "kg_arena_plan.hpp's copies of the kernels' constants");
 static const uint32_t g_test_pass_buckets = hook("KATGPU_TEST_PASS_BUCKETS") ? (uint32_t)strtoul(hook("KATGPU_TEST_PASS_BUCKETS"), nullptr, 10) : 0;
 static uint32_t pass_buckets(uint32_t p1, uint32_t n_cu) {
     if (g_test_pass_buckets) return std::max<uint32_t>(1, std::min(p1, g_test_pass_buckets));
     return n_cu && p1 > n_cu && p1 % n_cu == 0 ? n_cu : p1;
 }
-static double arena_bytes_per_item(uint32_t hb, uint32_t passes) { return 8.0 * (1 + 1.0 / 24) + l2_bytes_per_item(hb) * (1 + 1.0 / 24) * l2_items_per_l1_item(hb) / passes + 0.25 + 0.02; }
+static const bool g_l1_lean = hook_u64("KATGPU_L1_LEAN", 1) != 0;
+static bool l1_blocks_shape(const PartGeom& g, uint32_t k) { return g_l1_lean && lean_applies(k, g.pl.n1) && g.P1 <= 512 && g.hb1 == 2; }
 
 static const bool g_test_grow_nomem = hook("KATGPU_TEST_GROW_NOMEM") != nullptr;
 
@@ -332,23 +334,24 @@
     return KATGPU_OK;
 }
 
-constexpr size_t SEG_PAD = 64;
+constexpr uint8_t GUARD_BYTE = 0xA5;
 struct PartArena {
-    uint32_t hb, passes; double per_item; size_t fixed_l1, small_bytes;
+    uint32_t hb, passes, n_cu; uint64_t regions; bool blocks_shape; double per_item_max; size_t small_bytes;
     uint32_t* hist1; uint64_t* offs; uint64_t* l1_off; uint64_t* off2; uint32_t* cnt2; uint64_t* bend; unsigned long long* spill_n; unsigned long long* ovf_n;
     uint8_t* l1_buf;
     uint8_t* l2_buf;
     uint64_t* ovf_buf; uint64_t ovf_cap;
-    size_t round_items, l1_items, l2_items;
-    PartArena(const PartGeom& g0, uint32_t W, uint32_t n_cu) : hb(g0.hb), passes(std::max<uint32_t>(1, g0.P1 / pass_buckets(g0.P1, n_cu))), per_item(arena_bytes_per_item(hb, passes)) {
-        fixed_l1 = (size_t)W * MAX_PARTS * SEG_PAD;
-        const size_t fixed_l2 = (size_t)((double)fixed_l1 * l2_items_per_l1_item(hb) / passes) + (size_t)MAX_PARTS * MAX_PARTS * P2_RUN_SLACK + 8192;
+    ArenaCarve cv;
+    size_t round_items, l1_bytes, l2_items;
+    PartArena(const PartGeom& g0, uint32_t k, uint32_t W, uint32_t n_cu_) : hb(g0.hb), passes(std::max<uint32_t>(1, g0.P1 / pass_buckets(g0.P1, n_cu_))), n_cu(n_cu_), regions(g0.R), blocks_shape(l1_blocks_shape(g0, k)) {
+        per_item_max = arena_bytes_per_item(hb, passes, false, false);
         small_bytes = align_up((size_t)W * MAX_PARTS * 4, 256) + align_up((size_t)W * MAX_PARTS * 8, 256) +
                       align_up((MAX_PARTS + 1) * 8, 256) + align_up(((size_t)MAX_PARTS * MAX_PARTS + 1) * 8, 256) +
-                      align_up((size_t)MAX_PARTS * MAX_PARTS * 4, 256) + align_up((size_t)MAX_PARTS * 8, 256) + align_up((size_t)MAX_PARTS * 4, 256) + 256 +
-                      (fixed_l1 + fixed_l2 + 4096) * 8 + 4096;
-    }
-    void carve_from(uint8_t* a, size_t arena_bytes, uint32_t W, size_t want_items) {
+                      align_up((size_t)MAX_PARTS * MAX_PARTS * 4, 256) + align_up((size_t)MAX_PARTS * 8, 256) + align_up((size_t)MAX_PARTS * 4, 256) + 256;
+    }
+    size_t fixed_bytes(uint32_t W) const { return small_bytes + (size_t)arena_fixed_bytes(hb, passes, W, n_cu, false, false); }
+    bool carve_from(uint8_t* a, size_t arena_bytes, uint32_t W, size_t want_items) {
+        uint8_t* const a0 = a;
         hist1 = carve<uint32_t>(a, (size_t)W * MAX_PARTS * 4);
         offs = carve<uint64_t>(a, (size_t)W * MAX_PARTS * 8);
         l1_off = carve<uint64_t>(a, (MAX_PARTS + 1) * 8);
@@ -358,15 +361,33 @@
         carve<uint32_t>(a, (size_t)MAX_PARTS * 4);
         spill_n = carve<unsigned long long>(a, STAMP_AREA * 8);
         ovf_n = spill_n + 1;
-        round_items = std::min<size_t>(want_items, (size_t)((double)(arena_bytes - small_bytes) / per_item));
-        l1_items = (round_items + round_items / 24 + fixed_l1 + 15) & ~(size_t)15;
-        l2_items = ((size_t)((double)l1_items * l2_items_per_l1_item(hb) / passes) + (size_t)MAX_PARTS * MAX_PARTS * P2_RUN_SLACK + 4096 + 11) / 12 * 12;
+        if ((size_t)(a - a0) > small_bytes || arena_bytes <= small_bytes) return false;
+        cv = arena_carve(arena_bytes - small_bytes, want_items, hb, passes, W, n_cu, regions, blocks_shape, g_l1_fast, g_test_p2_ovf_cap);
+        round_items = cv.round_items; l1_bytes = cv.l1_bytes; l2_items = cv.l2_items; ovf_cap = cv.ovf_cap;
         l1_buf = a;
-        l2_buf = l1_buf + l1_items * 8;
-        ovf_buf = (uint64_t*)(l2_buf + align_up(l2_buffer_bytes(hb, l2_items), 16));
-        ovf_cap = g_test_p2_ovf_cap ? g_test_p2_ovf_cap : round_items / 32 + 1024;
-    }
+        l2_buf = l1_buf + cv.l1_bytes + ARENA_GUARD;
+        ovf_buf = (uint64_t*)(l2_buf + cv.l2_bytes + ARENA_GUARD);
+        return (size_t)((uint8_t*)(ovf_buf + ovf_cap) + ARENA_GUARD - a0) <= arena_bytes;
+    }
+    uint8_t* guard(int i) const { return i == 0 ? l1_buf + cv.l1_bytes : i == 1 ? l2_buf + cv.l2_bytes : (uint8_t*)(ovf_buf + ovf_cap); }
 };
+static const char* const GUARD_NAME[3] = {"level-1 buffer", "level-2 buffer", "overflow list"};
+static int guards_set(katgpu_ctx* c, const PartArena& A) {
+    if (!g_testing) return KATGPU_OK;
+    for (int i = 0; i < 3; ++i) HIPCHK(c, hipMemsetAsync(A.guard(i), GUARD_BYTE, ARENA_GUARD, c->stream));
+    return KATGPU_OK;
+}
+static int guards_check(katgpu_ctx* c, const PartArena& A) {
+    if (!g_testing) return KATGPU_OK;
+    std::vector<uint8_t> h(3 * ARENA_GUARD);
+    for (int i = 0; i < 3; ++i) HIPCHK(c, hipMemcpyAsync(h.data() + i * ARENA_GUARD, A.guard(i), ARENA_GUARD, hipMemcpyDeviceToHost, c->stream));
+    HIPCHK(c, hipStreamSynchronize(c->stream));
+    for (int i = 0; i < 3; ++i)
+        for (size_t j = 0; j < ARENA_GUARD; ++j)
+            if (h[i * ARENA_GUARD + j] != GUARD_BYTE)
+                return fail(c, KATGPU_ERR_DEVICE, "partition arena: the guard behind the %s was written (byte %zu)", GUARD_NAME[i], j);
+    return KATGPU_OK;
+}
 static int restore_ones(katgpu_table* t) { katgpu_ctx* c = t->ctx; HIPCHK(c, hipMemcpyAsync(&t->dv.ctrs[CTR_ONES], &t->ones, sizeof(uint64_t), hipMemcpyHostToDevice, c->stream)); return KATGPU_OK; }
 static int probe_items_per_start(katgpu_table* t, const PartGeom& g, const PartArena& A, uint32_t W, const uint8_t* p, size_t left, double* items_per_start) {
     katgpu_ctx* c = t->ctx;
@@ -380,17 +401,6 @@
     *items_per_start = std::max(0.05, (double)probe_items / (double)probe_m);
     return t->dv.k == 32 && !t->dv.canonical ? restore_ones(t) : KATGPU_OK;
 }
-static size_t round_starts(size_t left, size_t round_items, double items_per_start) {
-    size_t m = left;
-    if (m > round_items) m = std::min(m, (size_t)((double)round_items / items_per_start * 0.98));
-    if (m < left) {
-        const size_t rounds_left = (left + m - 1) / m;
-        m = (left + rounds_left - 1) / rounds_left;
-        m += P1_TILE_STARTS - m % P1_TILE_STARTS;
-        m = std::min(m, left);
-    }
-    return m;
-}
 
 enum class L1Edition { Blocks, SegLean512, SegLean1024, SegPlain512, SegPlain1024, ExactLean, ExactPlain };
 static const char* const L1_EDITION_NAME[] = {"Blocks", "SegLean512", "SegLean1024", "SegPlain512", "SegPlain1024", "ExactLean", "ExactPlain"};
@@ -398,26 +408,17 @@
     L1Edition edition; bool seg ; uint32_t wgs ; uint64_t n_tiles, tiles_per_wg;
     uint64_t seg_cap, cap_plain, stride64;
 };
-static L1Plan plan_level1(const PartGeom& g, uint32_t k, size_t m, uint64_t est_items, uint32_t W, uint32_t n_cu, size_t l1_items, bool seg_wanted) {
+static L1Plan plan_level1(const PartGeom& g, uint32_t k, size_t m, uint64_t est_items, uint32_t W, uint32_t n_cu, size_t l1_bytes, bool seg_wanted) {
     const bool lean = g_l1_lean && lean_applies(k, g.pl.n1);
     const bool pb512 = g.P1 <= 512;
-    const bool l1b = lean && pb512 && g.hb1 == 2;
+    const bool l1b = l1_blocks_shape(g, k);
     const uint64_t n_tiles = (m + P1_TILE_STARTS - 1) / P1_TILE_STARTS;
     L1Plan pl;
     pl.wgs = l1b ? n_cu : W;
     pl.n_tiles = l1b ? (m + L1B_TILE_STARTS - 1) / L1B_TILE_STARTS : n_tiles;
-    uint64_t seg_cap = est_items / ((uint64_t)pl.wgs * g.P1);
-    seg_cap += seg_cap / 24 + SEG_PAD;
-    if (g_test_l1_cpb) seg_cap = std::min<uint64_t>(seg_cap, g_test_l1_cpb);
-    if (l1b) seg_cap = (seg_cap + L1B_ITEMS - 1) / L1B_ITEMS * L1B_ITEMS;
-    pl.cap_plain = seg_cap;
-    if (!l1b && g.hb1 != 4 && !g_test_l1_cpb) seg_cap += std::min<uint64_t>(3 * seg_cap, 2 * ((pl.n_tiles + pl.wgs - 1) / pl.wgs));
-    if (!l1b) seg_cap = (seg_cap + 3) & ~3ULL;
-    pl.seg_cap = seg_cap;
-    pl.stride64 = l1b ? align_up(8 * (uint64_t)pl.wgs * pl.cap_plain + 32, 64)
-                      : std::max<uint64_t>(8 * (uint64_t)pl.wgs * pl.cap_plain, (uint64_t)(4 + g.hb1) * pl.wgs * seg_cap) + 32;
-    pl.seg = seg_wanted && pl.stride64 * g.P1 <= (uint64_t)l1_items * 8 &&
-             seg_cap < (1u << 24) && pl.stride64 <= 0xFFFFFFFFULL ;
+    const L1Segments sg = l1_segments(l1b, g.P1, g.hb1, pl.wgs, est_items, (pl.n_tiles + pl.wgs - 1) / pl.wgs, g_test_l1_cpb, l1_bytes);
+    pl.cap_plain = sg.cap_plain; pl.seg_cap = sg.seg_cap; pl.stride64 = sg.stride;
+    pl.seg = seg_wanted && sg.fits;
     if (pl.seg) pl.edition = l1b ? L1Edition::Blocks : lean ? (pb512 ? L1Edition::SegLean512 : L1Edition::SegLean1024) : (pb512 ? L1Edition::SegPlain512 : L1Edition::SegPlain1024);
     else { pl.edition = lean ? L1Edition::ExactLean : L1Edition::ExactPlain; pl.wgs = W; pl.n_tiles = n_tiles; }
     pl.tiles_per_wg = (pl.n_tiles + pl.wgs - 1) / pl.wgs;
@@ -452,14 +453,16 @@
     }
     return KATGPU_OK;
 }
-static int level1(katgpu_table* t, const PartGeom& g, const L1Plan& l1, const PartArena& A, const uint8_t* p, size_t m, double items_per_start, uint64_t* items) {
+static int level1(katgpu_table* t, const PartGeom& g, const L1Plan& l1, const PartArena& A, size_t cap_items, const uint8_t* p, size_t m, double items_per_start, uint64_t* items) {
     katgpu_ctx* c = t->ctx;
     const uint64_t nb = m + t->dv.k - 1;
     if (l1.seg) {
         int rc;
+        if (l1.stride64 * g.P1 > A.l1_bytes || (uint64_t)l1.wgs * (l1.edition == L1Edition::Blocks ? l1.seg_cap / L1B_ITEMS * L1B_BYTES : (4 + g.hb1) * l1.seg_cap) > l1.stride64)
+            return fail(c, KATGPU_ERR_DEVICE, "partition round: %u buckets of %llu bytes end beyond the level-1 buffer of %zu bytes", g.P1, (unsigned long long)l1.stride64, A.l1_bytes);
         { ScopedTimer tm(c, KATGPU_K_PART_L1S, *items); rc = launch_l1_scatter(t, g, l1, A, p, nb); }
-        if (!rc && g_trace) fprintf(stderr, "[katgpu] partition round (segmented level 1%s): %zu starts, ~%llu items, %llu k-mers per segment (arena %.1f GB)\n", l1.edition == L1Edition::Blocks ? ", blocks of ten" : "", m,
-                                    (unsigned long long)*items, (unsigned long long)l1.seg_cap, c->arena_bytes / 1e9);
+        if (!rc && g_trace) fprintf(stderr, "[katgpu] partition round (segmented level 1%s): %zu starts, ~%llu items, %llu k-mers per segment (arena %.1f GB; capacity %zu items, %s, stride %llu)\n", l1.edition == L1Edition::Blocks ? ", blocks of ten" : "", m,
+                                    (unsigned long long)*items, (unsigned long long)l1.seg_cap, c->arena_bytes / 1e9, cap_items, L1_EDITION_NAME[(int)l1.edition], (unsigned long long)l1.stride64);
         return rc;
     }
     {
@@ -469,9 +472,12 @@
     }
     HIPCHK(c, hipMemcpyAsync(items, &A.l1_off[g.P1], sizeof *items, hipMemcpyDeviceToHost, c->stream));
     HIPCHK(c, hipStreamSynchronize(c->stream));
-    if (g_trace) fprintf(stderr, "[katgpu] partition round: %zu starts -> %llu items (buffer %zu items, arena %.1f GB, ratio %.3f)\n", m, (unsigned long long)*items, A.round_items, c->arena_bytes / 1e9, items_per_start);
-    if (*items > A.round_items) return t->dv.k == 32 && !t->dv.canonical ? restore_ones(t) : KATGPU_OK;
+    if (g_trace) fprintf(stderr, "[katgpu] partition round: %zu starts -> %llu items (buffer %zu items, arena %.1f GB, ratio %.3f; capacity %zu items, %s, stride 0)\n", m, (unsigned long long)*items, A.round_items, c->arena_bytes / 1e9, items_per_start,
+                         cap_items, L1_EDITION_NAME[(int)l1.edition]);
+    if (*items > cap_items) return t->dv.k == 32 && !t->dv.canonical ? restore_ones(t) : KATGPU_OK;
     if (!*items) return KATGPU_OK;
+    if (l1_bucket_base(*items, g.P1) + 32 > A.l1_bytes)
+        return fail(c, KATGPU_ERR_DEVICE, "partition round: %llu items of an exact level 1 end beyond the level-1 buffer of %zu bytes", (unsigned long long)*items, A.l1_bytes);
     ScopedTimer tm(c, KATGPU_K_PART_L1S, *items);
     return launch_l1_scatter(t, g, l1, A, p, nb);
 }
@@ -553,11 +559,14 @@
     auto lbeg = [&](uint32_t b) -> uint64_t { return seg ? (uint64_t)b * g.l1_real : h_l1_off[b]; };
     const uint32_t tile2 = l2_tile_items(g.hb);
     auto pass_extent = [&](uint32_t b_lo, uint32_t b_hi) -> uint64_t {
-        const uint64_t nn = lbeg(b_hi) - lbeg(b_lo);
-        return nn + nn / 16 + 2ULL * g.P2 * (nn / tile2 + 1) + (uint64_t)(b_hi - b_lo) * g.P2 * P2_RUN_SLACK + 64;
+        return p2_pass_extent(lbeg(b_hi) - lbeg(b_lo), b_hi - b_lo, g.P2, tile2, g.l2_trim != 0);
     };
     uint32_t step = pass_buckets(g.P1, (uint32_t)c->n_cu);
     auto fits = [&](uint32_t st) { for (uint32_t b = 0; b < g.P1; b += st) if (pass_extent(b, std::min(g.P1, b + st)) > A.l2_items) return false; return true; };
+    if (!seg && A.cv.big) {
+        g.l2_trim = 0;
+        if (!fits(step) && l2_trims(g.hb, items, g.R)) g.l2_trim = 1;
+    }
     while (step > 1 && !fits(step)) step = (step + 1) / 2;
     if (!fits(step)) {
         *end = RoundEnd::DirectPath;
@@ -640,16 +649,19 @@
     const uint32_t W = n_cu * std::min<uint32_t>(g_p1_wgs, 4);
     PartGeom g0;
     if (!part_geometry(t->dv, &g0)) return KATGPU_OK;
-    PartArena A(g0, W, n_cu);
+    PartArena A(g0, k, W, n_cu);
     size_t want_items = n_starts;
     if (g_test_round_items) want_items = std::min<size_t>(want_items, g_test_round_items);
     bool usable = false;
-    int rc = ensure_arena(c, A.small_bytes, 18, want_items, A.small_bytes + (size_t)((A.per_item + 0.5) * (double)want_items), "", &usable);
+    int rc = ensure_arena(c, A.fixed_bytes(W), 18, want_items, A.fixed_bytes(W) + (size_t)((A.per_item_max + 0.5) * (double)want_items), "", &usable);
     if (rc || !usable) return rc;
     ArenaBusy busy(c);
-    A.carve_from(c->arena, c->arena_bytes, W, want_items);
+    if (!A.carve_from(c->arena, c->arena_bytes, W, want_items)) return fail(c, KATGPU_ERR_DEVICE, "partition arena: the carve of %zu bytes ends beyond the arena", c->arena_bytes);
+    rc = guards_set(c, A);
+    if (rc) return rc;
     if (!g_test_round_items && A.round_items < ((size_t)1 << 20) && A.round_items < n_starts) return KATGPU_OK;
     bool p2_fast_ok = g_p2_fast != 0, l1_fast_ok = g_l1_fast != 0;
+    RoundCaps caps;
     double items_per_start = 1.0;
     size_t pos = 0;
     bool ratio_known = false;
@@ -667,24 +679,32 @@
         if (g.hb > A.hb) break;
         const size_t left = n_starts - pos;
         const uint8_t* p = dev_bases + pos;
-        if (!ratio_known && !g_test_round_items && (left > A.round_items || (l1_fast_ok && left >= ((size_t)64 << 20)))) {
+        const size_t cap_items = caps.cap(A.cv, l1_fast_ok && l1_blocks_shape(g, k));
+        if (!ratio_known && !g_test_round_items && (left > cap_items || (l1_fast_ok && left >= ((size_t)64 << 20)))) {
             rc = probe_items_per_start(t, g, A, W, p, left, &items_per_start);
             if (rc) return rc;
             ratio_known = true;
         }
-        const size_t m = round_starts(left, A.round_items, items_per_start);
+        const size_t m = round_starts(left, cap_items, items_per_start);
         t->count_bound = 0xFFFFFFFFULL;
         const uint64_t est_items = (uint64_t)((double)m * items_per_start);
         const bool seg_wanted = l1_fast_ok && (g_l1_fast == 2 || (ratio_known && est_items >= ((uint64_t)64 << 20)));
-        const L1Plan l1 = plan_level1(g, k, m, est_items, W, n_cu, A.l1_items, seg_wanted);
+        const L1Plan l1 = plan_level1(g, k, m, est_items, W, n_cu, A.l1_bytes, seg_wanted);
+        if (l1.edition != L1Edition::Blocks && cap_items > caps.cap(A.cv, false)) { caps.exact_from_here(); continue; }
         g.l1_stride = l1.seg ? l1.stride64 : 0;
         g.l1_real = l1.seg ? (uint64_t)l1.wgs * l1.cap_plain : 0;
+        {
+            const uint32_t nb = std::min(g.P1, pass_buckets(g.P1, n_cu));
+            const uint64_t nn = l1.seg ? nb * g.l1_real : (uint64_t)((double)est_items * nb / g.P1 * (1 + 1.0 / 64)) + 1024;
+            g.l2_trim = round_trims(A.cv, g.hb, est_items, g.R, nn, nb, g.P2) ? 1u : 0u;
+        }
         HIPCHK(c, hipMemsetAsync(A.spill_n, 0, 2 * sizeof(unsigned long long), c->stream));
         uint64_t items = est_items;
-        rc = level1(t, g, l1, A, p, m, items_per_start, &items);
+        rc = level1(t, g, l1, A, cap_items, p, m, items_per_start, &items);
         if (rc) return rc;
-        if (!l1.seg && items > A.round_items) {
+        if (!l1.seg && items > cap_items) {
             items_per_start = std::min(1.0, (double)items / (double)m * 1.02);
+            caps.exact_from_here();
             continue;
         }
         if (items) {
@@ -692,12 +712,14 @@
             RoundEnd end;
             rc = level2_and_apply(t, g, l1, A, items, &p2_fast_ok, &lists, &end);
             if (rc) return rc;
-            if (end == RoundEnd::RedoExactL1) { l1_fast_ok = false; continue; }
+            if (end == RoundEnd::RedoExactL1) { l1_fast_ok = false; caps.exact_from_here(); continue; }
             if (end == RoundEnd::DirectPath) break;
             bool lost = false;
             rc = insert_spilled(t, lists, &lost);
             if (rc) return rc;
             if (lost) { pos += m; break; }
+            rc = guards_check(c, A);
+            if (rc) return rc;
         }
         pos += m;
     }
diff --git a/kat_amd/csrc/kg_l2_blocks.hpp b/kat_amd/csrc/kg_l2_blocks.hpp
--- a/kat_amd/csrc/kg_l2_blocks.hpp
+++ b/kat_amd/csrc/kg_l2_blocks.hpp
@@ -35,8 +35,8 @@
     for (uint32_t b1 = g.b_lo + blockIdx.x; b1 < g.b_hi; b1 += gridDim.x) {
         uint64_t beg, n_items, n_real;
         const uint8_t* bucket = l1_buf + l1_bucket_range(g, l1_off, seg_slots, b1, beg, n_items, n_real);
-        const uint64_t cap = p2_region_cap(n_real, P, TILE_CAP, L2_BLOCK_ITEMS);
-        const uint64_t obase = p2_out_base(beg, b1, P, TILE_CAP, L2_BLOCK_ITEMS) - p2_out_base(beg0, g.b_lo, P, TILE_CAP, L2_BLOCK_ITEMS);
+        const uint64_t cap = p2_region_cap(n_real, P, TILE_CAP, L2_BLOCK_ITEMS, g.l2_trim != 0);
+        const uint64_t obase = p2_out_base(beg, b1, P, TILE_CAP, L2_BLOCK_ITEMS, g.l2_trim != 0) - p2_out_base(beg0, g.b_lo, P, TILE_CAP, L2_BLOCK_ITEMS, g.l2_trim != 0);
         uint8_t* const runs = l2_buf + l2_lo_at<1>(obase >> 2);
         const uint32_t capb = (uint32_t)(cap / L2_BLOCK_ITEMS);
         lds_barrier();
diff --git a/kat_amd/csrc/kg_partition.hpp b/kat_amd/csrc/kg_partition.hpp
--- a/kat_amd/csrc/kg_partition.hpp
+++ b/kat_amd/csrc/kg_partition.hpp
@@ -2,6 +2,7 @@
 #include "kg_kernels.hpp"
 #include "kg_l1_lean.hpp"
 #include "kg_apply_lean.hpp"
+#include "kg_arena_plan.hpp"
 
 #include <cstddef>
 #include <type_traits>
@@ -32,6 +33,7 @@
     uint64_t l1_real;
     uint64_t spill_cap;
     uint32_t cbits;
+    uint32_t l2_trim;
     Place pl;
 };
 __device__ __host__ __forceinline__ uint32_t l2_hi_bytes(uint32_t rb) { return rb <= 31 ? 0u : rb <= 39 ? 1u : rb <= 47 ? 2u : 4u; }
@@ -42,9 +44,6 @@
     static constexpr uint32_t GS = 16 + 4 * HB;
     static constexpr uint64_t NONE = HB == 4 ? ~0ULL : (1ULL << (32 + 8 * HB)) - 1;
 };
-__device__ __host__ __forceinline__ uint32_t l2_tile_items(uint32_t hb) { return hb == 4 ? 12 * 1024 : 16 * 1024; }
-__device__ __host__ __forceinline__ constexpr bool l2_blocked(uint32_t hb) { return hb == 1; }
-constexpr uint32_t L2_BLOCK_ITEMS = 12, L2_BLOCK_BYTES = 64;
 template <int HB> __device__ __host__ __forceinline__ uint64_t l2_lo_at(uint64_t grp) {
     if (l2_blocked(HB)) { const uint64_t b = grp / 3; return b * L2_BLOCK_BYTES + (grp - 3 * b) * 16; }
     return grp * L2Fmt<HB>::GS;
@@ -53,9 +52,6 @@
     if (l2_blocked(HB)) { const uint64_t b = grp / 3; return b * L2_BLOCK_BYTES + 48 + (grp - 3 * b) * 4; }
     return grp * L2Fmt<HB>::GS + 16;
 }
-__device__ __host__ __forceinline__ uint64_t l2_buffer_bytes(uint32_t hb, uint64_t items) { return l2_blocked(hb) ? (items / L2_BLOCK_ITEMS + 2) * L2_BLOCK_BYTES : items / 4 * (16 + 4 * hb); }
-__device__ __host__ __forceinline__ double l2_bytes_per_item(uint32_t hb) { return l2_blocked(hb) ? (double)L2_BLOCK_BYTES / L2_BLOCK_ITEMS : 4.0 + hb; }
-__device__ __host__ __forceinline__ uint32_t l2_run_align(uint32_t hb) { return l2_blocked(hb) ? L2_BLOCK_ITEMS : 4u; }
 template <int HB> struct HiWord { typedef uint32_t type; };
 template <> struct HiWord<1> { typedef uint8_t type; };
 template <> struct HiWord<2> { typedef uint16_t type; };
@@ -178,7 +174,6 @@
 constexpr int P1_TILE_STARTS = P1_TILE_BYTES - CHUNK_OVERLAP;
 constexpr int P1_LANES_WITH_STARTS = P1_TILE_STARTS / PART_ITEMS;
 
-__device__ __host__ __forceinline__ uint64_t l1_bucket_base(uint64_t first_item, uint32_t b) { return 8 * first_item + 32ULL * b; }
 template <uint32_t HB1>
 __device__ __forceinline__ void l1_put(uint8_t* __restrict__ bucket, uint64_t group_byte, uint32_t q, uint32_t lo, uint32_t hi) {
     uint8_t* grp = bucket + group_byte;
@@ -1017,7 +1012,6 @@
     return blocks;
 }
 
-__device__ __host__ __forceinline__ uint64_t p2_exact_base(uint64_t beg, uint32_t b1, uint32_t P2) { return (beg + 4 * ((uint64_t)P2 + 1) * b1 + 3) & ~3ULL; }
 
 template <int HB, bool W1 , bool L1B = false >
 __global__ void __launch_bounds__(PART_BLOCK)
@@ -1064,15 +1058,6 @@
     }
 }
 
-constexpr uint32_t P2_RUN_SLACK = 48;
-__device__ __host__ __forceinline__ uint64_t p2_region_cap(uint64_t n_b, uint32_t P2, uint32_t tile, uint32_t al = 4) {
-    const uint64_t c = ((n_b + (n_b >> 4)) >> (31 - __builtin_clz(P2))) + 2 * (n_b / tile + 1) + 16;
-    return (c + al - 1) / al * al;
-}
-__device__ __host__ __forceinline__ uint64_t p2_out_base(uint64_t beg, uint32_t b1, uint32_t P2, uint32_t tile, uint32_t al = 4) {
-    const uint64_t o = beg + (beg >> 4) + 2 * (uint64_t)P2 * (beg / tile) + (uint64_t)b1 * P2 * P2_RUN_SLACK;
-    return (o + al - 1) / al * al;
-}
 
 template <int HB, bool W1, bool STAMP = false, bool L1B = false >
 __global__ void __launch_bounds__(PART_BLOCK)
@@ -1092,8 +1077,8 @@
     for (uint32_t b1 = g.b_lo + blockIdx.x; b1 < g.b_hi; b1 += gridDim.x) {
         uint64_t beg, n_items, n_real;
         const uint8_t* bucket = l1_buf + l1_bucket_range(g, l1_off, seg_slots, b1, beg, n_items, n_real);
-        const uint64_t cap = p2_region_cap(n_real, g.P2, L2Fmt<HB>::TILE, AL);
-        const uint64_t obase = p2_out_base(beg, b1, g.P2, L2Fmt<HB>::TILE, AL) - p2_out_base(beg0, g.b_lo, g.P2, L2Fmt<HB>::TILE, AL);
+        const uint64_t cap = p2_region_cap(n_real, g.P2, L2Fmt<HB>::TILE, AL, g.l2_trim != 0);
+        const uint64_t obase = p2_out_base(beg, b1, g.P2, L2Fmt<HB>::TILE, AL, g.l2_trim != 0) - p2_out_base(beg0, g.b_lo, g.P2, L2Fmt<HB>::TILE, AL, g.l2_trim != 0);
         uint8_t* runs = l2_buf + l2_lo_at<HB>(obase >> 2);
         const uint32_t capg = (uint32_t)(cap / AL);
         lds_barrier();
```
